# quokka-astro/quokka

Hardware: AMD Instinct MI355X
Metric: Mcell-updates/s on 3D Sedov unigrid (higher is better)
Workload: dtype f64; 1 GPU; 3D Sedov blast 256x256x256 unigrid (tests/blast_unigrid_256.in scaled to 256^3 cells per GPU), 128^3 boxes, PPM+HLLC RK2, gamma=1.4, CFL 0.3, reflecting octant; cells_per_gpu=16777216, boxes_per_gpu=8, parallelism=box-decomposition x1, rk2_mode=carry, fofc_stages=0, retries=0, x_sweep_in_y_march=True

## Files before the change

### include/quokka_amd.h

```cpp
#ifndef QUOKKA_AMD_H_
#define QUOKKA_AMD_H_

#include <stdint.h>

#ifdef __cplusplus
extern "C" {
#endif

typedef struct qk_ctx qk_ctx;
typedef struct qk_level qk_level;
typedef void *qk_stream;

typedef enum qk_status {
	QK_OK = 0,
	QK_ERR_INVALID = -1,
	QK_ERR_HIP = -2,
	QK_ERR_UNSUPPORTED = -3,
	QK_ERR_STATE = -4,
	QK_ERR_NOT_CONVERGED = -5
} qk_status;

typedef struct qk_array4 {
	double *p;
	int64_t jstride, kstride, nstride;
// ... 12 lines not shown

typedef struct qk_box {
	int lo[3];
	int hi[3];
} qk_box;

#define QK_MAX_SCALARS 8
#define QK_HOOK_COMPILED 100
typedef struct qk_hydro_traits {
	double gamma;
	double cs_isothermal;
	double mean_molecular_weight;
	double boltzmann_constant;
	int reconstruct_eint;
	int nscalars;
	int nmscalars;
	int ndim;
	int eos_temperature_model;
	double eos_alpha;
} qk_hydro_traits;

enum { QK_DIR_X1 = 0, QK_DIR_X2 = 1, QK_DIR_X3 = 2 };
enum { QK_RIEMANN_HLLC = 0, QK_RIEMANN_LLF = 1, QK_RIEMANN_HLLD = 2  };
enum { QK_LIMITER_MINMOD = 0, QK_LIMITER_MC = 1 };
enum { QK_BC_REFLECT_ODD = -1, QK_BC_INT_DIR = 0, QK_BC_REFLECT_EVEN = 1, QK_BC_FOEXTRAP = 2, QK_BC_EXT_DIR = 3 };

#define QK_DEVICE_HOST_PLANNING (-1)
int qk_ctx_create(qk_ctx **ctx, int device);
int qk_ctx_destroy(qk_ctx *ctx);
const char *qk_last_error(qk_ctx *ctx);
const char *qk_version(void);

int qk_profile_enable(qk_ctx *ctx, int on);
int qk_profile_only(qk_ctx *ctx, const char *kernel_name);
int qk_profile_reset(qk_ctx *ctx);
int qk_profile_num_kernels(qk_ctx *ctx);
int qk_profile_get(qk_ctx *ctx, int k, const char **name, long *count, double *total_ms);

int qk_clear_bytes(qk_ctx *ctx, qk_stream s, void *device_ptr, int64_t nbytes);

int qk_level_create(qk_ctx *ctx, qk_level **lev, int ndim, int nboxes, const qk_box *valid_boxes);
int qk_level_destroy(qk_level *lev);

int qk_upload_array4_table(qk_ctx *ctx, int n, const qk_array4 *host_table, qk_array4 **device_table);
int qk_upload_iarray4_table(qk_ctx *ctx, int n, const qk_iarray4 *host_table, qk_iarray4 **device_table);

int qk_ReconstructStatesConstant(qk_level *lev, qk_stream s, int dir, const qk_array4 *q, qk_array4 *leftState, qk_array4 *rightState, int nghost,
				 int nvars);
int qk_ReconstructStatesPLM(qk_level *lev, qk_stream s, int dir, int limiter, const qk_array4 *q, qk_array4 *leftState, qk_array4 *rightState,
			    int nghost, int nvars);
int qk_ReconstructStatesPPM(qk_level *lev, qk_stream s, int dir, const qk_array4 *q, qk_array4 *leftState, qk_array4 *rightState, int nghost,
			    int nvars, int iReadFrom, int iWriteFrom);

int qk_hydro_ConservedToPrimitive(qk_level *lev, qk_stream s, const qk_hydro_traits *t, const qk_array4 *cons, qk_array4 *primVar, int nghost);
int qk_hydro_ComputeFlatteningCoefficients(qk_level *lev, qk_stream s, const qk_hydro_traits *t, int dir, const qk_array4 *primVar, qk_array4 *x1Chi,
					   int nghost);
int qk_hydro_FlattenShocks(qk_level *lev, qk_stream s, const qk_hydro_traits *t, int dir, const qk_array4 *q, const qk_array4 *x1Chi,
			   const qk_array4 *x2Chi, const qk_array4 *x3Chi, qk_array4 *x1LeftState, qk_array4 *x1RightState, int nghost, int nvars);
int qk_hydro_ComputeFluxes(qk_level *lev, qk_stream s, const qk_hydro_traits *t, int riemann, int dir, qk_array4 *x1Flux, qk_array4 *x1FaceVel,
			   const qk_array4 *x1LeftState, const qk_array4 *x1RightState, const qk_array4 *primVar, double K_visc);
int qk_hydro_ComputeRhsFromFluxes(qk_level *lev, qk_stream s, const qk_hydro_traits *t, qk_array4 *rhs, const qk_array4 *const fluxArray[3],
				  const double dx[3], int nvars);
int qk_hydro_AddInternalEnergyPdV(qk_level *lev, qk_stream s, const qk_hydro_traits *t, qk_array4 *rhs, const qk_array4 *consVar, const double dx[3],
				  const qk_array4 *const faceVelArray[3], const qk_iarray4 *redoFlag);
int qk_hydro_PredictStep(qk_level *lev, qk_stream s, const qk_hydro_traits *t, const qk_array4 *consVarOld, qk_array4 *consVarNew,
			 const qk_array4 *rhs, double dt, int nvars, qk_iarray4 *redoFlag, int64_t *d_redo_count);
int qk_hydro_EnforceLimits(qk_level *lev, qk_stream s, const qk_hydro_traits *t, double densityFloor, double tempFloor, qk_array4 *state);
int qk_hydro_SyncDualEnergy(qk_level *lev, qk_stream s, const qk_hydro_traits *t, qk_array4 *consVar, int *d_error_flag);
int qk_hydro_ComputeMaxSignalSpeed(qk_level *lev, qk_stream s, const qk_hydro_traits *t, const qk_array4 *cons, qk_array4 *maxSignal);
int qk_hydro_maxSignalSpeedLocal(qk_level *lev, qk_stream s, const qk_hydro_traits *t, int which, const qk_array4 *cons, double *d_result);

int qk_replaceFluxes(qk_level *lev, qk_stream s, int dir, qk_array4 *flux, const qk_array4 *FOflux, const qk_iarray4 *redoFlag, int face_ncomp);
int qk_Saxpy(qk_level *lev, qk_stream s, int dir, qk_array4 *dst, double a, const qk_array4 *src, int ncomp);
int qk_hydro_FixupState(qk_level *lev, qk_stream s, const qk_hydro_traits *t, double densityFloor, double tempFloor, int use_dual_energy, qk_array4 *state,
			int *d_error_flag, double *d_max_signal);


int qk_advect_ComputeFluxes(qk_level *lev, qk_stream s, int dir, qk_array4 *flux, const qk_array4 *left, const qk_array4 *right, double advectionVx, int nvars);
int qk_advect_PredictStep(qk_level *lev, qk_stream s, const qk_array4 *consVarOld, qk_array4 *consVarNew, const qk_array4 *const fluxArray[3], double dt,
			  const double dx[3], int nvars);
int qk_advect_AddFluxesRK2(qk_level *lev, qk_stream s, qk_array4 *U_new, const qk_array4 *U0, const qk_array4 *U1, const qk_array4 *const fluxArray[3], double dt,
			   const double dx[3], int nvars);

typedef struct qk_hydro_stage_args {
	const qk_array4 *U_in;
	const qk_array4 *U_old;
	qk_array4 *U_out;
	qk_array4 *halfFlux[3];
	qk_array4 *halfVel[3];
	qk_iarray4 *redoFlag;
	int64_t *d_redo_count;
	int *d_error_flag;
	double *d_max_signal;
	void *scratch;
	int64_t scratch_bytes;
	double dx[3];
	double dt;
	int stage;
	int reconstruction_order;
	double densityFloor, tempFloor;
	int use_dual_energy;
	double K_visc;
	int store_flux_rk2;
	qk_array4 *fluxRk2[3];
	int rk2_carry_rhs;
	qk_array4 *rhs1;
	const struct qk_carray4 *flux_mask;
	int fofc_pass;
	int prim_out;
	int prim_in;
	int store_vel_rk2;
	qk_array4 *velRk2[3];
} qk_hydro_stage_args;

int64_t qk_hydro_stage_scratch_bytes(qk_level *lev, const qk_hydro_traits *t);
int qk_hydro_stage_fused(qk_level *lev, qk_stream s, const qk_hydro_traits *t, const qk_hydro_stage_args *a);

#define QK_MAX_GROUPS 8
typedef struct qk_rad_traits {
	double c_light, c_hat, radiation_constant, Erad_floor;
	int beta_order;
	int opacity_model;
	double kappaP, kappaE, kappaF;
	int pow_mode;
	int eddington_model;
	double opacity_T_ref, opacity_T_exponent, opacity_pow_floor;
	int ngroups;
	int mg_opacity_model;
	double energy_unit;
	double rad_boundaries[QK_MAX_GROUPS + 1];
	double mg_kappa_exponent[QK_MAX_GROUPS + 1], mg_kappa_lower[QK_MAX_GROUPS + 1];
	double mg_kappa_rho_exponent, mg_kappa_T_ref, mg_kappa_T_exponent;
	int enable_dust_gas_thermal_coupling_model;
	double dust_gas_interaction_coeff;
	int thermal_model;
	double gas_dust_coupling_threshold;
	double cooling_linear_coeff[QK_MAX_GROUPS];
	double cr_heating_rate;
	int enable_photoelectric_heating;
	double pe_heating_E1_derivative;
} qk_rad_traits;

int qk_rad_ConservedToPrimitive(qk_level *lev, qk_stream s, const qk_rad_traits *rt, const qk_array4 *cons, qk_array4 *primVar, int nghost);
int qk_rad_ComputeWavespeedCorrection(qk_level *lev, qk_stream s, const qk_rad_traits *rt, const qk_hydro_traits *t, int ndim, const qk_array4 *consVar,
				      const double dx[3], qk_array4 *const eps[3]);
int qk_rad_ComputeFluxes(qk_level *lev, qk_stream s, const qk_rad_traits *rt, int dir, qk_array4 *x1Flux, const qk_array4 *x1LeftState,
			 const qk_array4 *x1RightState, const qk_array4 *consVar, const qk_array4 *wavespeed_eps);
int qk_rad_computeRadiationFluxes(qk_level *lev, qk_stream s, const qk_rad_traits *rt, int ndim, int reconstruction_order, const qk_array4 *consVar,
				  qk_array4 *const flux[3], const qk_array4 *const wavespeed_eps[3] );
int qk_rad_stage_fused(qk_level *lev, qk_stream s, const qk_rad_traits *rt, int reconstruction_order, int stage, const qk_array4 *U_in, const qk_array4 *U0,
		       qk_array4 *U_new, qk_array4 *acc, qk_array4 *const flux_out[3], double dt, const double dx[3],
		       const qk_array4 *const wavespeed_eps[3] );
int qk_rad_PredictStep(qk_level *lev, qk_stream s, const qk_rad_traits *rt, int ndim, const qk_array4 *consVarOld, qk_array4 *consVarNew,
		       const qk_array4 *const fluxArray[3], double dt, const double dx[3]);
int qk_rad_AddFluxesRK2(qk_level *lev, qk_stream s, const qk_rad_traits *rt, int ndim, qk_array4 *U_new, const qk_array4 *U0, const qk_array4 *U1,
			const qk_array4 *const fluxArrayOld[3], const qk_array4 *const fluxArray[3], double dt, const double dx[3]);
int qk_rad_AddSourceTermsSingleGroup(qk_level *lev, qk_stream s, const qk_rad_traits *rt, const qk_hydro_traits *t, qk_array4 *consVar,
				     const qk_array4 *radEnergySource, double dt, int stage, int *d_iteration_counter, int *d_failure_counter);
int qk_rad_AddSourceTermsSingleGroupMirror(qk_level *lev, qk_stream s, const qk_rad_traits *rt, const qk_hydro_traits *t, qk_array4 *consVar,
					   const qk_array4 *radEnergySource, double dt, int stage, int *d_iteration_counter, int *d_failure_counter,
					   qk_array4 *mirror);
int qk_rad_AddSourceTermsMultiGroup(qk_level *lev, qk_stream s, const qk_rad_traits *rt, const qk_hydro_traits *t, qk_array4 *consVar,
				    const qk_array4 *radEnergySource, double dt, int stage, int *d_iteration_counter, int *d_failure_counter);
int qk_rad_mg_planck_fractions(qk_ctx *ctx, const qk_rad_traits *rt, double kB, int n, const double *T, double *fractions, double *Erad_g);

typedef struct qk_geometry {
	qk_box domain;
	int periodic[3];
	int ndim;
} qk_geometry;

typedef struct qk_bcrec {
	int lo[3];
	int hi[3];
} qk_bcrec;

#define QK_MAX_STATE_COMPS 48
typedef struct qk_dirichlet_face {
	int enabled;
	double values[QK_MAX_STATE_COMPS];
	int marshak;
	int marshak_energy_comp;
	int marshak_flux_comp;
	double marshak_c;
	uint64_t interior_mask;
	int kinetic_from_interior;
} qk_dirichlet_face;

typedef struct qk_ghost_plan qk_ghost_plan;
int qk_ghost_plan_create(qk_level *lev, qk_ghost_plan **plan, const qk_geometry *geom, int nghost, int ncomp, int n_all_boxes,
			 const qk_box *all_boxes, const int *owner_rank, int my_rank);
int qk_ghost_plan_destroy(qk_ghost_plan *plan);
int qk_ghost_plan_num_peers(qk_ghost_plan *plan);
int qk_ghost_plan_peer(qk_ghost_plan *plan, int k, int *rank, int64_t *send_count, int64_t *recv_count);
int qk_ghost_plan_num_items(qk_ghost_plan *plan, int kind, int k);
int qk_ghost_plan_item(qk_ghost_plan *plan, int kind, int k, int idx, int *dst_box, int *src_box, int lo[3], int hi[3], int shift[3], int64_t *offset);
int qk_FillBoundary_local(qk_ghost_plan *plan, qk_stream s, qk_array4 *state);
int qk_FillBoundary_local_int(qk_ghost_plan *plan, qk_stream s, qk_iarray4 *state);
int qk_FillBoundary_pack(qk_ghost_plan *plan, qk_stream s, int k, const qk_array4 *state, double *sendbuf);
int qk_FillBoundary_unpack(qk_ghost_plan *plan, qk_stream s, int k, qk_array4 *state, const double *recvbuf);
int qk_FillBoundary_pack_int(qk_ghost_plan *plan, qk_stream s, int k, const qk_iarray4 *state, int *sendbuf);
int qk_FillBoundary_unpack_int(qk_ghost_plan *plan, qk_stream s, int k, qk_iarray4 *state, const int *recvbuf);
int qk_SumBoundary_local(qk_ghost_plan *plan, qk_stream s, qk_array4 *state);
int qk_SumBoundary_pack(qk_ghost_plan *plan, qk_stream s, int k, const qk_array4 *state, double *buf);
int qk_SumBoundary_unpack(qk_ghost_plan *plan, qk_stream s, int k, qk_array4 *state, const double *buf);
int qk_FillPhysicalBoundary(qk_ghost_plan *plan, qk_stream s, qk_array4 *state, const qk_bcrec *bcs, const qk_dirichlet_face *dirichlet);
int qk_ghost_plan_set_components(qk_ghost_plan *plan, int scomp, int ncomp);
#define QK_BOXES_ALL 0
#define QK_BOXES_LOCAL_ONLY 1
#define QK_BOXES_REMOTE_DEPENDENT 2
int qk_ghost_plan_box_is_remote(qk_ghost_plan *plan, int local_box);
int qk_ghost_plan_set_box_remote(qk_ghost_plan *plan, int local_box, int flag);
int qk_FillPhysicalBoundary_subset(qk_ghost_plan *plan, qk_stream s, qk_array4 *state, const qk_bcrec *bcs, const qk_dirichlet_face *dirichlet,
				   int which);

typedef struct qk_carray4 {
	char *p;
	int64_t jstride, kstride, nstride;
	int begin[3];
	int end[3];
	int ncomp;
} qk_carray4;
enum { QK_TAG_CLEAR = 0, QK_TAG_BUF = 1, QK_TAG_SET = 2 };
#define QK_TAGFIELD_PRESSURE (-1)
int qk_tag_relative_gradient(qk_level *lev, qk_stream s, const qk_hydro_traits *t, const qk_array4 *state, qk_carray4 *tags, int field,
			     double eta_threshold, double q_min, int min_inclusive);
int qk_tag_centered_gradient(qk_level *lev, qk_stream s, const qk_array4 *state, qk_carray4 *tags, int comp, int dir, double dx, double eta_threshold,
			     double q_min, int min_inclusive);
int qk_PreInterpState(qk_level *lev, qk_stream s, qk_array4 *mf);
int qk_PostInterpState(qk_level *lev, qk_stream s, qk_array4 *mf);
typedef struct qk_avgdown_plan qk_avgdown_plan;
int qk_avgdown_plan_create(qk_level *crse, qk_level *fine, const int ratio[3], qk_avgdown_plan **plan);
int qk_avgdown_plan_destroy(qk_avgdown_plan *plan);
int qk_avgdown_plan_num_items(qk_avgdown_plan *plan);
int qk_average_down(qk_avgdown_plan *plan, qk_stream s, const qk_array4 *fine, qk_array4 *crse, int scomp, int ncomp);

typedef struct qk_interp_plan qk_interp_plan;
int qk_interp_plan_create(qk_level *crse, qk_level *fine, const qk_geometry *fine_geom, int nghost, const int ratio[3], int whole_fab, int n_all_fine,
			  const qk_box *all_fine, qk_interp_plan **plan);
int qk_interp_plan_destroy(qk_interp_plan *plan);
int qk_interp_plan_num_items(qk_interp_plan *plan);
int qk_interp_plan_item(qk_interp_plan *plan, int idx, int *fine_box, int *crse_box, int lo[3], int hi[3]);
int qk_InterpFromCoarse(qk_interp_plan *plan, qk_stream s, qk_array4 *fine, const qk_array4 *crse_old, const qk_array4 *crse_new, double w_old,
			double w_new, int ncomp, int method, int energy_hooks);

typedef struct qk_fluxreg qk_fluxreg;
int qk_fluxreg_create(qk_level *crse, qk_level *fine, const qk_geometry *crse_geom, const int ratio[3], int ncomp, int n_all_fine, const qk_box *all_fine,
		      int reg_nghost, qk_fluxreg **fr);
int qk_fluxreg_destroy(qk_fluxreg *fr);
int qk_fluxreg_num_items(qk_fluxreg *fr);
int qk_fluxreg_item(qk_fluxreg *fr, int idx, int *dir, int *side, int *fine_box, int *crse_box, int lo[3], int hi[3], int shift[3]);
int qk_fluxreg_reset(qk_fluxreg *fr, qk_stream s);
int qk_fluxreg_save(qk_fluxreg *fr, qk_stream s);
int qk_fluxreg_restore(qk_fluxreg *fr, qk_stream s);
int qk_fluxreg_CrseAdd(qk_fluxreg *fr, qk_stream s, const qk_array4 *const flux[3], const double dx[3], double dt);
int qk_fluxreg_FineAdd(qk_fluxreg *fr, qk_stream s, const qk_array4 *const flux[3], const double dx_fine[3], double dt);
int qk_fluxreg_Reflux(qk_fluxreg *fr, qk_stream s, qk_array4 *crse_state);
int qk_fluxreg_set_state_component(qk_fluxreg *fr, int comp0);

int qk_fluxreg_create_crse_part(qk_level *crse, qk_level *all_fine_level, const qk_geometry *crse_geom, const int ratio[3], int ncomp, qk_fluxreg **fr);

typedef struct qk_pcopy_plan qk_pcopy_plan;
int qk_pcopy_plan_create(qk_ctx *ctx, const qk_geometry *geom, int n_src, const qk_box *src_boxes, const int *src_owner, int src_nghost, int src_ring_only,
			 int n_dst, const qk_box *dst_boxes, const int *dst_owner, int dst_nghost, const qk_box *dst_holes, int ncomp, int my_rank,
			 qk_pcopy_plan **plan);
int qk_pcopy_plan_destroy(qk_pcopy_plan *plan);
int qk_pcopy_plan_num_peers(qk_pcopy_plan *plan);
int qk_pcopy_plan_peer(qk_pcopy_plan *plan, int k, int *rank, int64_t *send_count, int64_t *recv_count);
int qk_pcopy_plan_num_items(qk_pcopy_plan *plan, int kind, int k);
int qk_pcopy_plan_item(qk_pcopy_plan *plan, int kind, int k, int idx, int *dst_box, int *src_box, int lo[3], int hi[3], int shift[3], int64_t *offset);
int qk_ParallelCopy_local(qk_pcopy_plan *plan, qk_stream s, const qk_array4 *src, qk_array4 *dst, int scomp_src, int scomp_dst, int add);
int qk_ParallelCopy_pack(qk_pcopy_plan *plan, qk_stream s, int k, const qk_array4 *src, int scomp_src, double *sendbuf);
int qk_ParallelCopy_unpack(qk_pcopy_plan *plan, qk_stream s, int k, qk_array4 *dst, int scomp_dst, const double *recvbuf, int add);

int qk_copy_box(qk_ctx *ctx, qk_stream s, const qk_array4 *src, const qk_array4 *dst, const int lo[3], const int hi[3], int scomp, int dcomp, int ncomp);
int qk_amr_tile_flags(qk_level *lev, qk_stream s, const qk_carray4 *tags, const qk_box *domain, int n_error_buf, int tile, int *tile_flags_host);
int qk_amr_tile_flags_periodic(qk_level *lev, qk_stream s, const qk_carray4 *tags, const qk_box *domain, const int periodic[3], int n_error_buf, int tile,
			       int *tile_flags_host);
int qk_amr_cluster_tiles(const int *tiles, const int ntiles[3], int ndim, int blocking_factor, int max_grid_size, int parent_align, qk_box *boxes,
			 int max_boxes);
int qk_amr_cluster_berger_rigoutsos(const int *tiles, const int *allowed, const int ntiles[3], int ndim, int blocking_factor, int max_grid_size, double grid_eff,
				    qk_box *boxes, int max_boxes);

typedef struct qk_cloudy_tables {
	const double *log_nH;
	const double *log_Tgas;
	const double *cooling;
	const double *heating;
	const double *mean_mol_weight;
	int n_nH, n_Tgas;
	double T_min, T_max;
	double mmw_min, mmw_max;
} qk_cloudy_tables;
int qk_cloudy_tables_read(qk_ctx *ctx, const char *path, qk_cloudy_tables *host_tables);
int qk_cloudy_tables_free(qk_cloudy_tables *host_tables);
int qk_cooling_tabulated(qk_level *lev, qk_stream s, const qk_hydro_traits *t, qk_array4 *state, const qk_cloudy_tables *device_tables, double dt, double T_floor,
			 long long *d_counters);
// ... 52 lines not shown
```

### quokka_amd/capi.py

```python
from __future__ import annotations

import ctypes as C
import os

_HERE = os.path.dirname(os.path.abspath(__file__))
LIB_PATH = os.environ.get("QK_LIB_PATH", os.path.join(_HERE, "lib", "libquokka_amd.so"))

QK_OK, QK_ERR_INVALID, QK_ERR_HIP, QK_ERR_UNSUPPORTED, QK_ERR_STATE, QK_ERR_NOT_CONVERGED = 0, -1, -2, -3, -4, -5
ERR_UNSUPPORTED = QK_ERR_UNSUPPORTED
QK_TRACER_PREV, QK_TRACER_CUR, QK_TRACER_MAX_DEPTH = 0, 1, 3
HOOK_COMPILED = 100
DIR_X1, DIR_X2, DIR_X3 = 0, 1, 2
ARITH_DIVBY_RECIPOF, ARITH_DIVN, ARITH_RECIPEXACT, ARITH_SQRTN = 0, 1, 2, 3
COOLING_LIBM_DEVICE, COOLING_LIBM_PORTABLE = 0, 1
RIEMANN_HLLC, RIEMANN_LLF, RIEMANN_HLLD = 0, 1, 2
LIMITER_MINMOD, LIMITER_MC = 0, 1
BC_REFLECT_ODD, BC_INT_DIR, BC_REFLECT_EVEN, BC_FOEXTRAP, BC_EXT_DIR = -1, 0, 1, 2, 3

K_B = 1.380649e-16
M_U = 1.6605390666e-24


class Array4(C.Structure):
    _fields_ = [("p", C.c_void_p), ("jstride", C.c_int64), ("kstride", C.c_int64), ("nstride", C.c_int64),
                ("begin", C.c_int * 3), ("end", C.c_int * 3), ("ncomp", C.c_int)]


class Box(C.Structure):
    _fields_ = [("lo", C.c_int * 3), ("hi", C.c_int * 3)]


class HydroTraits(C.Structure):
    _fields_ = [("gamma", C.c_double), ("cs_isothermal", C.c_double), ("mean_molecular_weight", C.c_double),
                ("boltzmann_constant", C.c_double), ("reconstruct_eint", C.c_int), ("nscalars", C.c_int),
                ("nmscalars", C.c_int), ("ndim", C.c_int), ("eos_temperature_model", C.c_int), ("eos_alpha", C.c_double)]


class Geometry(C.Structure):
    _fields_ = [("domain", Box), ("periodic", C.c_int * 3), ("ndim", C.c_int)]


class BCRec(C.Structure):
    _fields_ = [("lo", C.c_int * 3), ("hi", C.c_int * 3)]


MAX_GROUPS = 8
MAX_STATE_COMPS = 48


class DirichletFace(C.Structure):
    _fields_ = [("enabled", C.c_int), ("values", C.c_double * MAX_STATE_COMPS),
                ("marshak", C.c_int), ("marshak_energy_comp", C.c_int), ("marshak_flux_comp", C.c_int), ("marshak_c", C.c_double),
                ("interior_mask", C.c_uint64), ("kinetic_from_interior", C.c_int)]


class RadTraits(C.Structure):
    _fields_ = [("c_light", C.c_double), ("c_hat", C.c_double), ("radiation_constant", C.c_double), ("Erad_floor", C.c_double),
                ("beta_order", C.c_int), ("opacity_model", C.c_int), ("kappaP", C.c_double), ("kappaE", C.c_double), ("kappaF", C.c_double),
                ("pow_mode", C.c_int), ("eddington_model", C.c_int),
                ("opacity_T_ref", C.c_double), ("opacity_T_exponent", C.c_double), ("opacity_pow_floor", C.c_double),
                ("ngroups", C.c_int), ("mg_opacity_model", C.c_int), ("energy_unit", C.c_double), ("rad_boundaries", C.c_double * (MAX_GROUPS + 1)),
                ("mg_kappa_exponent", C.c_double * (MAX_GROUPS + 1)), ("mg_kappa_lower", C.c_double * (MAX_GROUPS + 1)),
                ("mg_kappa_rho_exponent", C.c_double), ("mg_kappa_T_ref", C.c_double), ("mg_kappa_T_exponent", C.c_double),
                ("enable_dust_gas_thermal_coupling_model", C.c_int), ("dust_gas_interaction_coeff", C.c_double), ("thermal_model", C.c_int),
                ("gas_dust_coupling_threshold", C.c_double),
                ("cooling_linear_coeff", C.c_double * MAX_GROUPS), ("cr_heating_rate", C.c_double), ("enable_photoelectric_heating", C.c_int),
                ("pe_heating_E1_derivative", C.c_double)]

    def set_groups(self, boundaries, energy_unit, opacity_model, kappa_exponent, kappa_lower, rho_exponent=0.0, T_ref=0.0, T_exponent=0.0):
        ng = len(boundaries) - 1
        assert 2 <= ng <= MAX_GROUPS and len(kappa_exponent) == len(kappa_lower) == ng + 1
        self.ngroups, self.mg_opacity_model, self.energy_unit = ng, int(opacity_model), float(energy_unit)
        for g in range(ng + 1):
            self.rad_boundaries[g] = float(boundaries[g])
            self.mg_kappa_exponent[g] = float(kappa_exponent[g])
            self.mg_kappa_lower[g] = float(kappa_lower[g])
        self.mg_kappa_rho_exponent, self.mg_kappa_T_ref, self.mg_kappa_T_exponent = float(rho_exponent), float(T_ref), float(T_exponent)
        return self


class CloudyTables(C.Structure):
    _fields_ = [("log_nH", C.c_void_p), ("log_Tgas", C.c_void_p), ("cooling", C.c_void_p), ("heating", C.c_void_p), ("mean_mol_weight", C.c_void_p),
                ("n_nH", C.c_int), ("n_Tgas", C.c_int), ("T_min", C.c_double), ("T_max", C.c_double), ("mmw_min", C.c_double), ("mmw_max", C.c_double)]


class StageArgs(C.Structure):
    _fields_ = [("U_in", C.c_void_p), ("U_old", C.c_void_p), ("U_out", C.c_void_p),
                ("halfFlux", C.c_void_p * 3), ("halfVel", C.c_void_p * 3),
                ("redoFlag", C.c_void_p), ("d_redo_count", C.c_void_p), ("d_error_flag", C.c_void_p), ("d_max_signal", C.c_void_p),
                ("scratch", C.c_void_p), ("scratch_bytes", C.c_int64),
                ("dx", C.c_double * 3), ("dt", C.c_double), ("stage", C.c_int), ("reconstruction_order", C.c_int),
                ("densityFloor", C.c_double), ("tempFloor", C.c_double), ("use_dual_energy", C.c_int), ("K_visc", C.c_double),
                ("store_flux_rk2", C.c_int), ("fluxRk2", C.c_void_p * 3), ("rk2_carry_rhs", C.c_int), ("rhs1", C.c_void_p), ("flux_mask", C.c_void_p), ("fofc_pass", C.c_int),
                ("prim_out", C.c_int), ("prim_in", C.c_int),
                ("store_vel_rk2", C.c_int), ("velRk2", C.c_void_p * 3)]


def traits(gamma=1.4, reconstruct_eint=True, ndim=3, mean_molecular_weight=M_U, boltzmann_constant=K_B,
           cs_isothermal=float("nan"), nscalars=0, nmscalars=0, eos_temperature_model=0, eos_alpha=0.0) -> HydroTraits:
    return HydroTraits(gamma, cs_isothermal, mean_molecular_weight, boltzmann_constant, int(reconstruct_eint), nscalars, nmscalars, ndim,
                       int(eos_temperature_model), float(eos_alpha))


class QkError(RuntimeError):
    pass


_lib = None


def lib() -> C.CDLL:
    global _lib
    if _lib is not None:
        return _lib
    if not os.path.exists(LIB_PATH):
        raise QkError(f"{LIB_PATH} is missing: run `python -c 'import __graft_entry__ as g; g.build()'` "
                      "(hipcc --offload-arch=gfx950). The hot path has no CPU fallback.")
    L = C.CDLL(LIB_PATH)
    vp, ci, cd = C.c_void_p, C.c_int, C.c_double
    P = C.POINTER
    L.qk_version.restype = C.c_char_p
    L.qk_last_error.restype = C.c_char_p
    L.qk_last_error.argtypes = [vp]
    L.qk_ctx_create.argtypes = [P(vp), ci]
    L.qk_ctx_destroy.argtypes = [vp]
    L.qk_level_create.argtypes = [vp, P(vp), ci, ci, P(Box)]
    L.qk_level_destroy.argtypes = [vp]
    L.qk_upload_array4_table.argtypes = [vp, ci, P(Array4), P(vp)]
    L.qk_upload_iarray4_table.argtypes = [vp, ci, P(Array4), P(vp)]
    L.qk_profile_enable.argtypes = [vp, ci]
    L.qk_profile_only.argtypes = [vp, C.c_char_p]
    L.qk_clear_bytes.argtypes = [vp, vp, vp, C.c_int64]
    L.qk_profile_reset.argtypes = [vp]
    L.qk_cloudy_tables_read.argtypes = [vp, C.c_char_p, P(CloudyTables)]
    L.qk_cloudy_tables_free.argtypes = [P(CloudyTables)]
    L.qk_cooling_tabulated.argtypes = [vp, vp, P(HydroTraits), vp, P(CloudyTables), cd, cd, vp]
    L.qk_cooling_evaluate.argtypes = [vp, vp, P(CloudyTables), cd, ci, C.c_int64, vp, vp, vp]
    L.qk_cooling_set_libm.argtypes = [vp, ci]
    L.qk_arith_evaluate.argtypes = [vp, vp, ci, C.c_int64, vp, vp, vp]
    L.qk_profile_num_kernels.argtypes = [vp]
    L.qk_profile_get.argtypes = [vp, ci, P(C.c_char_p), P(C.c_long), P(cd)]
    T = P(HydroTraits)
    L.qk_ReconstructStatesConstant.argtypes = [vp, vp, ci, vp, vp, vp, ci, ci]
    L.qk_ReconstructStatesPLM.argtypes = [vp, vp, ci, ci, vp, vp, vp, ci, ci]
    L.qk_ReconstructStatesPPM.argtypes = [vp, vp, ci, vp, vp, vp, ci, ci, ci, ci]
    L.qk_hydro_ConservedToPrimitive.argtypes = [vp, vp, T, vp, vp, ci]
    L.qk_hydro_ComputeFlatteningCoefficients.argtypes = [vp, vp, T, ci, vp, vp, ci]
    L.qk_hydro_FlattenShocks.argtypes = [vp, vp, T, ci, vp, vp, vp, vp, vp, vp, ci, ci]
    L.qk_hydro_ComputeFluxes.argtypes = [vp, vp, T, ci, ci, vp, vp, vp, vp, vp, cd]
    L.qk_hydro_ComputeRhsFromFluxes.argtypes = [vp, vp, T, vp, P(vp), P(cd), ci]
    L.qk_hydro_AddInternalEnergyPdV.argtypes = [vp, vp, T, vp, vp, P(cd), P(vp), vp]
    L.qk_hydro_PredictStep.argtypes = [vp, vp, T, vp, vp, vp, cd, ci, vp, vp]
    L.qk_hydro_EnforceLimits.argtypes = [vp, vp, T, cd, cd, vp]
    L.qk_hydro_SyncDualEnergy.argtypes = [vp, vp, T, vp, vp]
    L.qk_hydro_ComputeMaxSignalSpeed.argtypes = [vp, vp, T, vp, vp]
    L.qk_hydro_maxSignalSpeedLocal.argtypes = [vp, vp, T, ci, vp, vp]
    L.qk_replaceFluxes.argtypes = [vp, vp, ci, vp, vp, vp, ci]
    L.qk_Saxpy.argtypes = [vp, vp, ci, vp, cd, vp, ci]
    R = P(RadTraits)
    L.qk_rad_ConservedToPrimitive.argtypes = [vp, vp, R, vp, vp, ci]
    L.qk_rad_ComputeFluxes.argtypes = [vp, vp, R, ci, vp, vp, vp, vp, vp]
    L.qk_rad_computeRadiationFluxes.argtypes = [vp, vp, R, ci, ci, vp, P(vp), P(vp)]
    L.qk_rad_ComputeWavespeedCorrection.argtypes = [vp, vp, R, T, ci, vp, P(cd), P(vp)]
    L.qk_rad_PredictStep.argtypes = [vp, vp, R, ci, vp, vp, P(vp), cd, P(cd)]
    L.qk_rad_AddFluxesRK2.argtypes = [vp, vp, R, ci, vp, vp, vp, P(vp), P(vp), cd, P(cd)]
    L.qk_hydro_FixupState.argtypes = [vp, vp, T, cd, cd, ci, vp, vp, vp]
    L.qk_rad_stage_fused.argtypes = [vp, vp, R, ci, ci, vp, vp, vp, vp, P(vp), cd, P(cd), P(vp)]
    L.qk_rad_AddSourceTermsSingleGroup.argtypes = [vp, vp, R, T, vp, vp, cd, ci, vp, vp]
    L.qk_rad_AddSourceTermsSingleGroupMirror.argtypes = [vp, vp, R, T, vp, vp, cd, ci, vp, vp, vp]
    L.qk_rad_AddSourceTermsMultiGroup.argtypes = [vp, vp, R, T, vp, vp, cd, ci, vp, vp]
    L.qk_rad_mg_planck_fractions.argtypes = [vp, R, cd, ci, P(cd), P(cd), P(cd)]
    if hasattr(L, "qk_hydro_stage_fused"):
        L.qk_hydro_stage_scratch_bytes.argtypes = [vp, T]
        L.qk_hydro_stage_scratch_bytes.restype = C.c_int64
        L.qk_hydro_stage_fused.argtypes = [vp, vp, T, P(StageArgs)]
    if hasattr(L, "qk_ghost_plan_create"):
        L.qk_ghost_plan_create.argtypes = [vp, P(vp), P(Geometry), ci, ci, ci, P(Box), P(ci), ci]
        L.qk_ghost_plan_destroy.argtypes = [vp]
        L.qk_ghost_plan_num_peers.argtypes = [vp]
        L.qk_ghost_plan_peer.argtypes = [vp, ci, P(ci), P(C.c_int64), P(C.c_int64)]
        L.qk_ghost_plan_num_items.argtypes = [vp, ci, ci]
        L.qk_ghost_plan_item.argtypes = [vp, ci, ci, ci, P(ci), P(ci), ci * 3, ci * 3, ci * 3, P(C.c_int64)]
        L.qk_FillBoundary_local.argtypes = [vp, vp, vp]
        L.qk_FillBoundary_local_int.argtypes = [vp, vp, vp]
        L.qk_FillBoundary_pack.argtypes = [vp, vp, ci, vp, vp]
        L.qk_FillBoundary_unpack.argtypes = [vp, vp, ci, vp, vp]
        L.qk_SumBoundary_local.argtypes = [vp, vp, vp]
        L.qk_SumBoundary_pack.argtypes = [vp, vp, ci, vp, vp]
        L.qk_SumBoundary_unpack.argtypes = [vp, vp, ci, vp, vp]
        L.qk_FillBoundary_pack_int.argtypes = [vp, vp, ci, vp, vp]
        L.qk_FillBoundary_unpack_int.argtypes = [vp, vp, ci, vp, vp]
        L.qk_FillPhysicalBoundary.argtypes = [vp, vp, vp, P(BCRec), P(DirichletFace)]
        L.qk_FillPhysicalBoundary_subset.argtypes = [vp, vp, vp, P(BCRec), P(DirichletFace), C.c_int]
        L.qk_ghost_plan_set_components.argtypes = [vp, C.c_int, C.c_int]
        L.qk_ghost_plan_box_is_remote.argtypes = [vp, C.c_int]
        L.qk_ghost_plan_set_box_remote.argtypes = [vp, C.c_int, C.c_int]
    if hasattr(L, "qk_tag_relative_gradient"):
        L.qk_tag_relative_gradient.argtypes = [vp, vp, T, vp, vp, ci, C.c_double, C.c_double, ci]
        L.qk_tag_centered_gradient.argtypes = [vp, vp, vp, vp, ci, ci, C.c_double, C.c_double, C.c_double, ci]
        L.qk_avgdown_plan_create.argtypes = [vp, vp, ci * 3, P(vp)]
        L.qk_avgdown_plan_destroy.argtypes = [vp]
        L.qk_avgdown_plan_num_items.argtypes = [vp]
        L.qk_average_down.argtypes = [vp, vp, vp, vp, ci, ci]
        L.qk_interp_plan_create.argtypes = [vp, vp, P(Geometry), ci, ci * 3, ci, ci, vp, P(vp)]
        L.qk_interp_plan_destroy.argtypes = [vp]
        L.qk_interp_plan_num_items.argtypes = [vp]
        L.qk_interp_plan_item.argtypes = [vp, ci, P(ci), P(ci), ci * 3, ci * 3]
        L.qk_InterpFromCoarse.argtypes = [vp, vp, vp, vp, vp, C.c_double, C.c_double, ci, ci, ci]
        L.qk_fluxreg_create.argtypes = [vp, vp, P(Geometry), ci * 3, ci, ci, vp, ci, P(vp)]
        L.qk_fluxreg_destroy.argtypes = [vp]
        L.qk_fluxreg_num_items.argtypes = [vp]
        L.qk_fluxreg_item.argtypes = [vp, ci, P(ci), P(ci), P(ci), P(ci), ci * 3, ci * 3, ci * 3]
        L.qk_fluxreg_reset.argtypes = [vp, vp]
        L.qk_fluxreg_save.argtypes = [vp, vp]
        L.qk_fluxreg_restore.argtypes = [vp, vp]
        L.qk_fluxreg_CrseAdd.argtypes = [vp, vp, vp * 3, C.c_double * 3, C.c_double]
        L.qk_fluxreg_FineAdd.argtypes = [vp, vp, vp * 3, C.c_double * 3, C.c_double]
        L.qk_fluxreg_Reflux.argtypes = [vp, vp, vp]
        L.qk_fluxreg_set_state_component.argtypes = [vp, C.c_int]
        L.qk_copy_box.argtypes = [vp, vp, vp, vp, ci * 3, ci * 3, ci, ci, ci]
        L.qk_amr_tile_flags.argtypes = [vp, vp, vp, P(Box), ci, ci, vp]
        L.qk_amr_tile_flags_periodic.argtypes = [vp, vp, vp, P(Box), P(ci), ci, ci, vp]
        L.qk_amr_cluster_tiles.argtypes = [vp, ci * 3, ci, ci, ci, ci, P(Box), ci]
        L.qk_amr_cluster_berger_rigoutsos.argtypes = [vp, vp, ci * 3, ci, ci, ci, C.c_double, P(Box), ci]
        L.qk_PreInterpState.argtypes = [vp, vp, vp]
        L.qk_PostInterpState.argtypes = [vp, vp, vp]
        L.qk_fluxreg_create_crse_part.argtypes = [vp, vp, P(Geometry), ci * 3, ci, P(vp)]
        L.qk_pcopy_plan_create.argtypes = [vp, P(Geometry), ci, P(Box), P(ci), ci, ci, ci, P(Box), P(ci), ci, vp, ci, ci, P(vp)]
        L.qk_pcopy_plan_destroy.argtypes = [vp]
        L.qk_pcopy_plan_num_peers.argtypes = [vp]
        L.qk_pcopy_plan_peer.argtypes = [vp, ci, P(ci), P(C.c_int64), P(C.c_int64)]
        L.qk_pcopy_plan_num_items.argtypes = [vp, ci, ci]
        L.qk_pcopy_plan_item.argtypes = [vp, ci, ci, ci, P(ci), P(ci), ci * 3, ci * 3, ci * 3, P(C.c_int64)]
        L.qk_ParallelCopy_local.argtypes = [vp, vp, vp, vp, ci, ci, ci]
        L.qk_ParallelCopy_pack.argtypes = [vp, vp, ci, vp, ci, vp]
        L.qk_ParallelCopy_unpack.argtypes = [vp, vp, ci, vp, ci, vp, ci]
    L.qk_tracer_plan_create.argtypes = [vp, P(vp), P(Geometry), cd * 3, cd * 3, cd * 3]
    L.qk_tracer_plan_destroy.argtypes = [vp]
    L.qk_tracer_plan_lattice.argtypes = [vp, ci * 3, P(C.c_int64)]
    L.qk_tracer_InitOnePerCell.argtypes = [vp, vp, cd * 3, vp * 3, vp * 3, vp, vp, C.c_int64, ci]
    L.qk_tracer_AdvectWithUmac.argtypes = [vp, vp, vp * 3, cd, C.c_int64, vp * 3, vp * 3]
    L.qk_tracer_Redistribute.argtypes = [vp, vp, C.c_int64, vp * 3, vp]
    L.qk_tracer_plan_create_refined.argtypes = [vp, P(vp), P(Geometry), cd * 3, cd * 3, cd * 3]
    L.qk_tracer_plan_set_parent.argtypes = [vp, ci, vp, vp * 3]
    L.qk_tracer_plan_set_time_weights.argtypes = [vp, cd, cd]
    L.qk_tracer_plan_clear_parent.argtypes = [vp]
    L.qk_tracer_Where.argtypes = [P(vp), ci, vp, ci, ci, C.c_int64, vp * 3, vp, vp, vp]
    i3 = ci * 3
    L.qk_gravity_scratch_bytes.argtypes = [i3]
    L.qk_gravity_scratch_bytes.restype = C.c_int64
    L.qk_gravity_num_ghosts.argtypes = [i3]
    L.qk_gravity_num_ghosts.restype = C.c_int64
    L.qk_gravity_fill_rhs.argtypes = [vp, vp, cd, vp, ci, i3, vp]
    L.qk_gravity_dirichlet_solve.argtypes = [vp, vp, i3, cd, vp, vp, cd, cd, ci, vp, C.c_int64, P(ci), P(cd)]
    L.qk_gravity_surface_gather.argtypes = [vp, vp, i3, vp, vp]
    L.qk_gravity_surface_potential.argtypes = [vp, vp, i3, vp, vp, vp, C.c_int64]
    L.qk_gravity_surface_scatter.argtypes = [vp, vp, i3, vp, vp]
    L.qk_gravity_kick.argtypes = [vp, vp, i3, vp, cd * 3, cd, vp]
    _lib = L
    return L


BOXES_ALL, BOXES_LOCAL_ONLY, BOXES_REMOTE_DEPENDENT = 0, 1, 2
TAG_CLEAR, TAG_BUF, TAG_SET = 0, 1, 2
TAGFIELD_PRESSURE = -1

DECLARED_SYMBOLS = [
    "qk_ctx_create", "qk_ctx_destroy", "qk_last_error", "qk_version", "qk_level_create", "qk_level_destroy",
    "qk_upload_array4_table", "qk_upload_iarray4_table", "qk_clear_bytes", "qk_profile_enable", "qk_profile_only", "qk_profile_reset", "qk_profile_num_kernels", "qk_profile_get",
    "qk_ReconstructStatesConstant", "qk_ReconstructStatesPLM", "qk_ReconstructStatesPPM",
    "qk_hydro_ConservedToPrimitive", "qk_hydro_ComputeFlatteningCoefficients", "qk_hydro_FlattenShocks",
    "qk_hydro_ComputeFluxes", "qk_hydro_ComputeRhsFromFluxes", "qk_hydro_AddInternalEnergyPdV", "qk_hydro_PredictStep",
    "qk_hydro_EnforceLimits", "qk_hydro_SyncDualEnergy", "qk_hydro_ComputeMaxSignalSpeed", "qk_hydro_maxSignalSpeedLocal",
    "qk_replaceFluxes", "qk_Saxpy", "qk_hydro_FixupState", "qk_hydro_stage_scratch_bytes", "qk_hydro_stage_fused",
    "qk_rad_ConservedToPrimitive", "qk_rad_ComputeWavespeedCorrection", "qk_rad_ComputeFluxes", "qk_rad_computeRadiationFluxes", "qk_rad_PredictStep", "qk_rad_AddFluxesRK2", "qk_rad_stage_fused",
    "qk_rad_AddSourceTermsSingleGroup", "qk_rad_AddSourceTermsSingleGroupMirror", "qk_rad_AddSourceTermsMultiGroup", "qk_rad_mg_planck_fractions",
    "qk_ghost_plan_create", "qk_ghost_plan_destroy", "qk_ghost_plan_num_peers", "qk_ghost_plan_peer", "qk_ghost_plan_num_items", "qk_ghost_plan_item",
    "qk_FillBoundary_local", "qk_FillBoundary_local_int", "qk_FillBoundary_pack", "qk_FillBoundary_unpack", "qk_FillBoundary_pack_int", "qk_FillBoundary_unpack_int", "qk_SumBoundary_local", "qk_SumBoundary_pack", "qk_SumBoundary_unpack", "qk_FillPhysicalBoundary",
    "qk_FillPhysicalBoundary_subset", "qk_ghost_plan_set_components", "qk_ghost_plan_box_is_remote", "qk_ghost_plan_set_box_remote",
    "qk_tag_relative_gradient", "qk_tag_centered_gradient", "qk_avgdown_plan_create", "qk_avgdown_plan_destroy", "qk_avgdown_plan_num_items", "qk_average_down", "qk_PreInterpState", "qk_PostInterpState",
    "qk_interp_plan_create", "qk_interp_plan_destroy", "qk_interp_plan_num_items", "qk_interp_plan_item", "qk_InterpFromCoarse",
    "qk_fluxreg_create", "qk_fluxreg_destroy", "qk_fluxreg_num_items", "qk_fluxreg_item", "qk_fluxreg_reset", "qk_fluxreg_save", "qk_fluxreg_restore", "qk_fluxreg_CrseAdd", "qk_fluxreg_FineAdd",
    "qk_fluxreg_Reflux", "qk_fluxreg_set_state_component", "qk_amr_tile_flags", "qk_amr_tile_flags_periodic", "qk_amr_cluster_tiles", "qk_amr_cluster_berger_rigoutsos", "qk_copy_box",
    "qk_cloudy_tables_read", "qk_cloudy_tables_free", "qk_cooling_tabulated", "qk_cooling_evaluate", "qk_cooling_set_libm", "qk_arith_evaluate",
    "qk_fluxreg_create_crse_part", "qk_pcopy_plan_create", "qk_pcopy_plan_destroy", "qk_pcopy_plan_num_peers", "qk_pcopy_plan_peer", "qk_pcopy_plan_num_items",
    "qk_pcopy_plan_item", "qk_ParallelCopy_local", "qk_ParallelCopy_pack", "qk_ParallelCopy_unpack",
    "qk_tracer_plan_create", "qk_tracer_plan_destroy", "qk_tracer_plan_lattice", "qk_tracer_InitOnePerCell", "qk_tracer_AdvectWithUmac", "qk_tracer_Redistribute",
    "qk_tracer_plan_create_refined", "qk_tracer_plan_set_parent", "qk_tracer_plan_set_time_weights", "qk_tracer_plan_clear_parent", "qk_tracer_Where",
    "qk_gravity_scratch_bytes", "qk_gravity_num_ghosts", "qk_gravity_fill_rhs", "qk_gravity_dirichlet_solve", "qk_gravity_surface_gather",
    "qk_gravity_surface_potential", "qk_gravity_surface_scatter", "qk_gravity_kick",
]


def check(ctx, rc: int, what: str = "") -> None:
    if rc != QK_OK:
        msg = lib().qk_last_error(ctx).decode() if ctx else ""
        raise QkError(f"{what} failed with status {rc}: {msg}")
```

### quokka_amd/csrc/qk_boundary.hip

```cpp
#include <algorithm>
#include <cstdlib>
#include <array>
#include <map>
#include <cstring>
#include <vector>

#include "qk_device.hpp"
#include "qk_internal.hpp"

using namespace qk;

namespace
{

struct CopyItem {
	int dst_box;
	int src_box;
	int lo[3], hi[3];
	int shift[3];
	int64_t offset;
};

struct PeerPlan {
	int rank = -1;
// ... 333 lines not shown
					it.offset = pp.recv_count;
					pp.recv_count += regionCells(it) * ncomp;
					pp.max_recv_cells = std::max<int64_t>(pp.max_recv_cells, regionCells(it));
					pp.recv.push_back(it);
				} else {
					PeerPlan &pp = peers[owner[gd]];
					pp.rank = owner[gd];
					it.offset = pp.send_count;
					pp.send_count += regionCells(it) * ncomp;
					pp.max_send_cells = std::max<int64_t>(pp.max_send_cells, regionCells(it));
					pp.send.push_back(it);
				}
			}
		}
	}
	for (int b = 0; b < lev->nboxes; ++b) {
		qk_box grown = lev->boxes[b];
		for (int d = 0; d < geom->ndim; ++d) {
			grown.lo[d] -= nghost;
			grown.hi[d] += nghost;
		}
		for (int d = 0; d < geom->ndim; ++d) {
			if (geom->periodic[d] != 0) {
				continue;
			}
			for (int side = 0; side < 2; ++side) {
				CopyItem it{};
				it.dst_box = b;
				it.src_box = b;
				for (int e = 0; e < 3; ++e) {
					it.lo[e] = grown.lo[e];
					it.hi[e] = grown.hi[e];
				}
				if (side == 0) {
					it.hi[d] = std::min(grown.hi[d], geom->domain.lo[d] - 1);
				} else {
					it.lo[d] = std::max(grown.lo[d], geom->domain.hi[d] + 1);
				}
				if (it.hi[d] >= it.lo[d]) {
					P->shells.push_back(it);
					P->max_shell_cells = std::max<int64_t>(P->max_shell_cells, regionCells(it));
				}
			}
		}
	}
	P->box_remote.assign(lev->nboxes, 0);
	for (auto &kv : peers) {
		for (auto const &it : kv.second.recv) {
			P->box_remote[it.dst_box] = 1;
		}
	}
	partitionShells(P);
	{
		int64_t biggest = std::max<int64_t>(P->max_local_cells, P->max_shell_cells);
		for (auto &kv : peers) {
			biggest = std::max<int64_t>(biggest, std::max<int64_t>(kv.second.max_recv_cells, kv.second.max_send_cells));
		}
		if (biggest * ncomp >= (int64_t{1} << 31)) {
			delete P;
			return setError(ctx, QK_ERR_UNSUPPORTED, "qk_ghost_plan_create: a ghost region holds 2^31 or more values");
		}
	}
	int rc = uploadItems(ctx, P->local, &P->d_local);
	if (rc == QK_OK) {
		rc = uploadItems(ctx, P->shells, &P->d_shells);
	}
	for (auto &kv : peers) {
		if (rc == QK_OK) {
			rc = uploadItems(ctx, kv.second.send, &kv.second.d_send);
		}
		if (rc == QK_OK) {
			rc = uploadItems(ctx, kv.second.recv, &kv.second.d_recv);
		}
		P->peers.push_back(kv.second);
	}
	if (rc != QK_OK) {
		qk_ghost_plan_destroy(P);
		return rc;
	}
	*plan_out = P;
	return QK_OK;
}

int qk_ghost_plan_destroy(qk_ghost_plan *plan)
{
	if (plan == nullptr) {
		return QK_ERR_INVALID;
	}
	(void)hipFree(plan->d_local);
	(void)hipFree(plan->d_shells);
	for (auto &p : plan->peers) {
		(void)hipFree(p.d_send);
		(void)hipFree(p.d_recv);
	}
	(void)hipFree(plan->d_bcs);
	(void)hipFree(plan->d_dir);
	(void)hipFree(plan->d_physbc);
	delete plan;
	return QK_OK;
}

int qk_ghost_plan_num_peers(qk_ghost_plan *plan) { return plan == nullptr ? QK_ERR_INVALID : static_cast<int>(plan->peers.size()); }

int qk_ghost_plan_peer(qk_ghost_plan *plan, int k, int *rank, int64_t *send_count, int64_t *recv_count)
{
	if (plan == nullptr) {
		return QK_ERR_INVALID;
	}
	QK_REQUIRE(plan->lev->ctx, k >= 0 && k < static_cast<int>(plan->peers.size()) && rank && send_count && recv_count, "qk_ghost_plan_peer: bad index");
	*rank = plan->peers[k].rank;
	*send_count = plan->peers[k].send_count;
	*recv_count = plan->peers[k].recv_count;
	return QK_OK;
}

static auto planItems(qk_ghost_plan *plan, int kind, int k) -> std::vector<CopyItem> const *
{
	if (kind == 0) {
		return &plan->local;
	}
	if (kind == 3) {
		return &plan->shells;
	}
	if (k < 0 || k >= static_cast<int>(plan->peers.size())) {
		return nullptr;
	}
	return (kind == 1) ? &plan->peers[k].send : (kind == 2) ? &plan->peers[k].recv : nullptr;
}

int qk_ghost_plan_num_items(qk_ghost_plan *plan, int kind, int k)
{
	if (plan == nullptr) {
		return QK_ERR_INVALID;
	}
	auto const *v = planItems(plan, kind, k);
	return v == nullptr ? QK_ERR_INVALID : static_cast<int>(v->size());
}

int qk_ghost_plan_item(qk_ghost_plan *plan, int kind, int k, int idx, int *dst_box, int *src_box, int lo[3], int hi[3], int shift[3], int64_t *offset)
{
	if (plan == nullptr) {
		return QK_ERR_INVALID;
	}
	auto const *v = planItems(plan, kind, k);
	QK_REQUIRE(plan->lev->ctx, v != nullptr && idx >= 0 && idx < static_cast<int>(v->size()) && dst_box && src_box && lo && hi && shift && offset,
		   "qk_ghost_plan_item: bad argument");
	CopyItem const &it = (*v)[idx];
	*dst_box = it.dst_box;
	*src_box = it.src_box;
	for (int d = 0; d < 3; ++d) {
		lo[d] = it.lo[d];
		hi[d] = it.hi[d];
		shift[d] = it.shift[d];
	}
	*offset = it.offset;
	return QK_OK;
}

int qk_FillBoundary_local(qk_ghost_plan *plan, qk_stream s, qk_array4 *state_t)
{
	if (plan == nullptr) {
		return QK_ERR_INVALID;
	}
	qk_ctx *ctx = plan->lev->ctx;
	QK_REQUIRE(ctx, state_t, "FillBoundary_local: NULL state");
	if (plan->local.empty()) {
// ... 268 lines not shown
```

### quokka_amd/csrc/qk_core.hip

```cpp
#include <algorithm>
#include <cstring>

#include "qk_device.hpp"
#include "qk_internal.hpp"

namespace
{

__global__ void __launch_bounds__(256) k_arith_evaluate(int what, int64_t n, const double *a, const double *b, double *out)
{
	const int64_t i = static_cast<int64_t>(blockIdx.x) * blockDim.x + threadIdx.x;
	if (i >= n) {
		return;
	}
	double r;
	switch (what) {
	case QK_ARITH_DIVBY_RECIPOF:
		r = qk::divBy(a[i], qk::recipOf(b[i]));
		break;
	case QK_ARITH_DIVN:
		r = qk::divN(a[i], b[i]);
		break;
	case QK_ARITH_RECIPEXACT:
		r = qk::recipExact(b[i]);
// ... 20 lines not shown
		auto *c = new qk_ctx;
		c->device = -1;
		*ctx = c;
		return QK_OK;
	}
	int ndev = 0;
	if (hipGetDeviceCount(&ndev) != hipSuccess || ndev == 0) {
		std::fprintf(stderr, "quokka_amd: no HIP device visible; the hot path has no CPU fallback\n");
		return QK_ERR_HIP;
	}
	if (device < 0 || device >= ndev) {
		return QK_ERR_INVALID;
	}
	if (hipSetDevice(device) != hipSuccess) {
		return QK_ERR_HIP;
	}
	auto *c = new qk_ctx;
	c->device = device;
	*ctx = c;
	return QK_OK;
}

int qk_ctx_destroy(qk_ctx *ctx)
{
	if (ctx == nullptr) {
		return QK_ERR_INVALID;
	}
	for (void *p : ctx->owned) {
		(void)hipFree(p);
	}
	delete ctx;
	return QK_OK;
}

const char *qk_last_error(qk_ctx *ctx)
{
	if (ctx == nullptr) {
		return "null context";
	}
	return ctx->last_error.c_str();
}

int qk_level_create(qk_ctx *ctx, qk_level **lev, int ndim, int nboxes, const qk_box *valid_boxes)
{
	if (ctx == nullptr || lev == nullptr) {
		return QK_ERR_INVALID;
	}
	QK_REQUIRE(ctx, nboxes >= 0 && (valid_boxes != nullptr || nboxes == 0), "qk_level_create: bad box list");
	QK_REQUIRE(ctx, ndim >= 1 && ndim <= 3, "qk_level_create: ndim must be 1, 2 or 3");
	auto *L = new qk_level;
	L->ctx = ctx;
	L->ndim = ndim;
	L->nboxes = nboxes;
	L->boxes.assign(valid_boxes, valid_boxes + nboxes);
	for (int b = 0; b < nboxes; ++b) {
		for (int d = 0; d < 3; ++d) {
			L->maxlen[d] = std::max(L->maxlen[d], valid_boxes[b].hi[d] - valid_boxes[b].lo[d] + 1);
		}
	}
	if (ctx->device < 0) {
		*lev = L;
		return QK_OK;
	}
	hipError_t e = hipMalloc(reinterpret_cast<void **>(&L->d_boxes), sizeof(qk_box) * (nboxes > 0 ? nboxes : 1));
	if (e == hipSuccess) {
		e = (nboxes > 0) ? hipMemcpy(L->d_boxes, valid_boxes, sizeof(qk_box) * nboxes, hipMemcpyHostToDevice) : hipSuccess;
	}
	if (e != hipSuccess) {
		delete L;
		return qk::setError(ctx, QK_ERR_HIP, "qk_level_create", hipGetErrorString(e));
	}
	*lev = L;
	return QK_OK;
}

int qk_level_destroy(qk_level *lev)
{
	if (lev == nullptr) {
		return QK_ERR_INVALID;
	}
	(void)hipFree(lev->d_boxes);
	(void)hipFree(lev->d_sgeom);
	(void)hipFree(lev->d_tile_flags);
	(void)hipFree(lev->d_cooling_queue);
	delete lev;
	return QK_OK;
}

int qk_clear_bytes(qk_ctx *ctx, qk_stream s, void *device_ptr, int64_t nbytes)
{
	if (ctx == nullptr) {
		return QK_ERR_INVALID;
	}
	QK_REQUIRE(ctx, device_ptr != nullptr && nbytes >= 0, "qk_clear_bytes: NULL pointer or negative size");
	QK_HIP_CHECK(ctx, hipMemsetAsync(device_ptr, 0, static_cast<size_t>(nbytes), static_cast<hipStream_t>(s)));
	return QK_OK;
}

int qk_profile_enable(qk_ctx *ctx, int on)
{
	if (ctx == nullptr) {
		return QK_ERR_INVALID;
	}
	ctx->profiling = (on != 0);
	return QK_OK;
}

int qk_profile_only(qk_ctx *ctx, const char *kernel_name)
{
	if (ctx == nullptr) {
		return QK_ERR_INVALID;
	}
	ctx->prof_only = (kernel_name != nullptr) ? kernel_name : "";
	return QK_OK;
}

static void profCollect(qk_ctx *ctx)
{
	for (auto &p : ctx->prof_pending) {
		float ms = 0.f;
		if (hipEventSynchronize(p.stop) == hipSuccess && hipEventElapsedTime(&ms, p.start, p.stop) == hipSuccess) {
			ctx->prof_slots[p.slot].count += 1;
			ctx->prof_slots[p.slot].total_ms += ms;
		}
		ctx->prof_free_events.push_back(p.start);
		ctx->prof_free_events.push_back(p.stop);
	}
	ctx->prof_pending.clear();
}

int qk_profile_reset(qk_ctx *ctx)
{
	if (ctx == nullptr) {
		return QK_ERR_INVALID;
	}
	profCollect(ctx);
	ctx->prof_slots.clear();
	return QK_OK;
}

int qk_profile_num_kernels(qk_ctx *ctx)
{
	if (ctx == nullptr) {
		return QK_ERR_INVALID;
	}
	profCollect(ctx);
	return static_cast<int>(ctx->prof_slots.size());
}

int qk_profile_get(qk_ctx *ctx, int k, const char **name, long *count, double *total_ms)
{
	if (ctx == nullptr) {
		return QK_ERR_INVALID;
	}
	QK_REQUIRE(ctx, k >= 0 && k < static_cast<int>(ctx->prof_slots.size()) && name && count && total_ms, "qk_profile_get: bad index");
	*name = ctx->prof_slots[k].name.c_str();
	*count = ctx->prof_slots[k].count;
	*total_ms = ctx->prof_slots[k].total_ms;
	return QK_OK;
}

static int uploadTable(qk_ctx *ctx, int n, const void *host, size_t elem, void **dev)
{
	if (ctx == nullptr) {
		return QK_ERR_INVALID;
	}
// ... 40 lines not shown
```

### quokka_amd/csrc/qk_hydro_fused.hip

```cpp
#include "qk_device.hpp"
#include <algorithm>
#include <cmath>
#include <cstdlib>
#include <type_traits>
#include <vector>

#include "qk_internal.hpp"

using namespace qk;

namespace
{

constexpr int NG = 4;

template <class P> QK_DEV void streamStore(P *p, double v) { __builtin_nontemporal_store(v, p); }
template <class P> QK_DEV auto streamLoad(P *p) -> double { return __builtin_nontemporal_load(p); }

struct SGeom {
	int64_t off;
	int glo[3];
	int n[3];
	int pitch;
	int64_t ncell;
};

enum { S_AUX = 0, S_RHS = 4 };
constexpr auto scratchComps(int nscalars) -> int { return S_RHS + NVAR + nscalars + 1; }
constexpr int QK_FUSED_MAX_SCALARS = 3;

struct SweepArgs {
	const qk_box *boxes;
	const SGeom *geom;
	double *scratch;
	int64_t total_cells;
	const qk_array4 *U_in;
	const qk_array4 *U_old;
	qk_array4 *U_out;
	qk_array4 *halfFlux;
	qk_array4 *halfVel;
	qk_iarray4 *redoFlag;
	unsigned long long *redo_count;
	int *error_flag;
	double *max_signal;
	double inv_dx;
	double dx;
	double inv_dx0, dx0;
	double dx3[3];
	double dt;
	double densityFloor, tempFloor;
	double K_visc;
	int use_dual_energy;
	bool reconstruct_eint;
	bool same_old;
	bool store_rk2;
	qk_array4 *rk2Flux;
	qk_array4 *rhs1;
	const qk_carray4 *fluxMask;
	int nseg;
	bool prim_in, prim_out;
	bool store_vel;
	qk_array4 *rk2Vel;
};

QK_DEV auto sarr(SweepArgs const &a, int comp) -> double * { return a.scratch + static_cast<int64_t>(comp) * a.total_cells; }

#ifndef QK_PT_Y
#define QK_PT_Y 7
#define QK_PT_THREADS 512
#endif
constexpr int PT_X = 66, PT_Y = QK_PT_Y, PT_THREADS = QK_PT_THREADS;
constexpr int PT_OWN = PT_X * PT_Y;
constexpr int PT_HALO_Y = 6 * PT_X;
constexpr int PT_HALO = PT_HALO_Y + 6 * PT_Y;
static_assert(PT_HALO <= PT_THREADS && PT_OWN <= PT_THREADS, "one halo cell per thread");

struct PlaneCell {
	double rho, vx, vy, vz, P;
};

struct PlaneRaw {
	double rho, mx, my, mz, E;
};
QK_DEV auto planeLoad(RA4 const &U, int64_t u) -> PlaneRaw
{
	PlaneRaw r;
	r.rho = U.p[u + U.ns * RHO];
	r.mx = U.p[u + U.ns * MX];
	r.my = U.p[u + U.ns * MY];
	r.mz = U.p[u + U.ns * MZ];
	r.E = U.p[u + U.ns * ENE];
	return r;
}
QK_DEV auto planeCell(Eos const &eos, bool re, PlaneRaw const &r) -> PlaneCell
{
	PlaneCell c;
	c.rho = r.rho;
	const Recip R = recipOf(c.rho);
	c.vx = divBy(r.mx, R);
	c.vy = divBy(r.my, R);
	c.vz = divBy(r.mz, R);
	if (eos.isothermal) {
		c.P = c.rho * (eos.cs_iso * eos.cs_iso);
		return c;
	}
	const double kinetic_energy = 0.5 * c.rho * (c.vx * c.vx + c.vy * c.vy + c.vz * c.vz);
	const double Eint_cons = r.E - kinetic_energy;
	if (re) {
		const double e = divBy(Eint_cons, R);
		const double e2 = (c.rho == 0.0) ? 0.0 : divBy(c.rho * e, R);
		c.P = eos.gm1 * c.rho * e2;
	} else {
		const double e = (c.rho == 0.0) ? 0.0 : divBy(Eint_cons, R);
		c.P = eos.gm1 * c.rho * e;
	}
	return c;
}

QK_DEV auto chiCompressive(double Pm2, double Pm1, double Pp1, double Pp2, Recip const &RKS, Recip const &Rbeta) -> double
{
	constexpr double beta_max = 0.85;
	constexpr double Zmax = 0.75;
	constexpr double Zmin = 0.25;
	const double dP1 = fabs(Pp1 - Pm1);
	const double beta_denom = fabs(Pp2 - Pm2);
	const double beta = (beta_denom != 0) ? divBy(dP1, recipOf(beta_denom)) : 0;
	const double chi_min = smax0(smin1(divBy(beta_max - beta, Rbeta)));
	const double Z = divBy(dP1, RKS);
	return smax(chi_min, smin1((Zmax - Z) / (Zmax - Zmin)));
}

template <bool PRIM>
__global__ void __launch_bounds__(PT_THREADS, 4) k_pre3(const qk_box *boxes, const SGeom *geom, const qk_array4 *U_t, double *scratch, int64_t T, Eos eos, bool re, int nseg,
							    int xt, int yt, int ndim)
{
	constexpr bool prim_in = PRIM;
	const unsigned nblk = gridDim.x, lin = blockIdx.x;
	const unsigned q8 = nblk / 8, r8 = nblk % 8, xcd = lin % 8, slot = lin / 8;
	const unsigned logical = (xcd < r8) ? xcd * (q8 + 1) + slot : r8 * (q8 + 1) + (xcd - r8) * q8 + slot;
	const int bix = static_cast<int>(logical % xt), biy = static_cast<int>((logical / xt) % yt), biz = static_cast<int>(logical / (xt * yt));
	__shared__ double s_P[PT_Y + 6][PT_X + 6];
	__shared__ double s_vx[PT_Y][PT_X + 4], s_vy[PT_Y + 4][PT_X];
	__shared__ double s_cx[PT_Y][PT_X + 2], s_cy[PT_Y + 2][PT_X];

	const int b = biz / nseg;
	const int seg = biz - b * nseg;
	const qk_box bx = boxes[b];
	const SGeom g = geom[b];
	RA4 U(U_t[b]);
	const int t = threadIdx.x;
	const int x0 = bx.lo[0] - 1 + bix * PT_X;
	const int y0 = bx.lo[1] - 1 + biy * PT_Y;
	if (x0 > bx.hi[0] + 1 || y0 > bx.hi[1] + 1) {
		return;
	}
	const int nall = bx.hi[2] - bx.lo[2] + 3;
	const int seglen = (nall + nseg - 1) / nseg;
	const int zfirst = bx.lo[2] - 1 + seg * seglen;
	const int zlast = min(zfirst + seglen - 1, bx.hi[2] + 1);
	if (zlast < zfirst) {
		return;
	}
	const int ngy = (ndim >= 2) ? NG : 0, ngz = (ndim == 3) ? NG : 0;
	const int flo[2] = {bx.lo[0] - NG, bx.lo[1] - ngy}, fhi[2] = {bx.hi[0] + NG, bx.hi[1] + ngy};
	const int fzlo = bx.lo[2] - ngz, fzhi = bx.hi[2] + ngz;

	const bool own = t < PT_OWN;
	const int ty = own ? t / PT_X : 0;
	const int tx = own ? t - ty * PT_X : 0;
	const int oi = x0 + tx, oj = y0 + ty;
	const bool ownIn = own && oi <= fhi[0] && oj >= flo[1] && oj <= fhi[1];
	const bool ownOut = own && oi <= bx.hi[0] + 1 && oj <= bx.hi[1] + 1;
	const int h = t - (PT_THREADS - PT_HALO);
	int hx = 0, hy = 0;
	if (h >= 0) {
		if (h < PT_HALO_Y) {
			const int r = h / PT_X;
			hx = h - r * PT_X;
			hy = (r < 3) ? r - 3 : PT_Y + r - 3;
		} else {
			const int r = (h - PT_HALO_Y) / 6, c = (h - PT_HALO_Y) - r * 6;
			hy = r;
			hx = (c < 3) ? c - 3 : PT_X + c - 3;
		}
	}
	const int hi_ = x0 + hx, hj = y0 + hy;
	const bool haloIn = (h >= 0) && hi_ >= flo[0] && hi_ <= fhi[0] && hj >= flo[1] && hj <= fhi[1];
	const bool rimX = (h >= 0) && (hx == -1 || hx == PT_X);
	const bool rimY = (h >= 0) && (hy == -1 || hy == PT_Y);
	const int rx = hx, ry = hy;

	double Pz[5] = {1., 1., 1., 1., 1.}, vzw[5] = {0., 0., 0., 0., 0.}, rhoz[3] = {1., 1., 1.}, chz[3] = {1., 1., 1.};
	const Recip Rbeta = recipOf(0.85 - 0.75);
	double fm[4] = {1., 1., 1., 1.}, fdx[4] = {0., 0., 0., 0.}, fdy[4] = {0., 0., 0., 0.};
	double *Sout = scratch + g.off;
	const PlaneRaw neutral{1., 0., 0., 0., prim_in ? 1. : 1. / eos.gm1};
	auto cellOf = [&](PlaneRaw const &r) -> PlaneCell { return prim_in ? PlaneCell{r.rho, r.mx, r.my, r.mz, r.E} : planeCell(eos, re, r); };
	int64_t uo = ownIn ? U.idx(oi, oj, zfirst - 3) : 0;
	int64_t uh = haloIn ? U.idx(hi_, hj, zfirst - 3) : 0;

	for (int k = zfirst - 3; k <= zlast + 3; ++k, uo += U.ks, uh += U.ks) {
		const bool inPlane = (k >= zfirst) && (k <= zlast);
		const bool kIn = (k >= fzlo) && (k <= fzhi);
		const PlaneCell c = cellOf((ownIn && kIn) ? planeLoad(U, uo) : neutral);
#pragma unroll
		for (int m = 0; m < 4; ++m) {
			Pz[m] = Pz[m + 1];
			vzw[m] = vzw[m + 1];
		}
		Pz[4] = c.P;
		vzw[4] = c.vz;
		rhoz[0] = rhoz[1];
		rhoz[1] = rhoz[2];
		rhoz[2] = c.rho;
#pragma unroll
		for (int m = 0; m < 3; ++m) {
			fm[m] = fm[m + 1];
			fdx[m] = fdx[m + 1];
			fdy[m] = fdy[m + 1];
		}
		if (inPlane) {
			PlaneCell hc{1., 0., 0., 0., 1.};
			if (own) {
				s_P[ty + 3][tx + 3] = c.P;
				s_vx[ty][tx + 2] = c.vx;
				s_vy[ty + 2][tx] = c.vy;
			}
			if (h >= 0) {
				if constexpr (PRIM) {
					if (haloIn && kIn) {
						hc.P = U.p[uh + U.ns * ENE];
						if (hy >= 0 && hy < PT_Y && hx >= -2 && hx < PT_X + 2) {
							hc.vx = U.p[uh + U.ns * MX];
						}
						if (hx >= 0 && hx < PT_X && hy >= -2 && hy < PT_Y + 2) {
							hc.vy = U.p[uh + U.ns * MY];
						}
						if (rimX || rimY) {
							hc.rho = U.p[uh + U.ns * RHO];
						}
					}
				} else {
					hc = cellOf((haloIn && kIn) ? planeLoad(U, uh) : neutral);
				}
				s_P[hy + 3][hx + 3] = hc.P;
				if (hy >= 0 && hy < PT_Y && hx >= -2 && hx < PT_X + 2) {
					s_vx[hy][hx + 2] = hc.vx;
				}
				if (hx >= 0 && hx < PT_X && hy >= -2 && hy < PT_Y + 2) {
					s_vy[hy + 2][hx] = hc.vy;
				}
			}
			__syncthreads();
			if (own) {
				const bool cx = s_vx[ty][tx + 3] < s_vx[ty][tx + 1];
				const bool cy = (ndim >= 2) && (s_vy[ty + 3][tx] < s_vy[ty + 1][tx]);
				double chx = 1.0, chy = 1.0;
				if (cx || cy) {
					const Recip RKS = recipOf(flatteningKS(eos, c.rho, c.P));
					if (cx) {
						const double *Pr = &s_P[ty + 3][tx + 3];
						chx = chiCompressive(Pr[-2], Pr[-1], Pr[1], Pr[2], RKS, Rbeta);
					}
					if (cy) {
						chy = chiCompressive(s_P[ty + 1][tx + 3], s_P[ty + 2][tx + 3], s_P[ty + 4][tx + 3], s_P[ty + 5][tx + 3], RKS, Rbeta);
					}
				}
				s_cx[ty][tx + 1] = chx;
				s_cy[ty + 1][tx] = chy;
			}
			if (rimX) {
				double chx = 1.0;
				if (s_vx[ry][rx + 3] < s_vx[ry][rx + 1]) {
					const double *Pr = &s_P[ry + 3][rx + 3];
					chx = chiCompressive(Pr[-2], Pr[-1], Pr[1], Pr[2], recipOf(flatteningKS(eos, hc.rho, hc.P)), Rbeta);
				}
				s_cx[ry][rx + 1] = chx;
			} else if (rimY) {
				double chy = 1.0;
				if ((ndim >= 2) && (s_vy[ry + 3][rx] < s_vy[ry + 1][rx])) {
					chy = chiCompressive(s_P[ry + 1][rx + 3], s_P[ry + 2][rx + 3], s_P[ry + 4][rx + 3], s_P[ry + 5][rx + 3],
							     recipOf(flatteningKS(eos, hc.rho, hc.P)), Rbeta);
				}
				s_cy[ry + 1][rx] = chy;
			}
			__syncthreads();
			if (own) {
				const double mx = smin(smin(s_cx[ty][tx], s_cx[ty][tx + 1]), s_cx[ty][tx + 2]);
				const double my = smin(smin(s_cy[ty][tx], s_cy[ty + 1][tx]), s_cy[ty + 2][tx]);
				fm[3] = smin(mx, my);
				fdx[3] = smin(s_vx[ty][tx + 3] - c.vx, c.vx - s_vx[ty][tx + 1]);
				fdy[3] = smin(s_vy[ty + 3][tx] - c.vy, c.vy - s_vy[ty + 1][tx]);
			}
			__syncthreads();
		}
		chz[0] = chz[1];
		chz[1] = chz[2];
		chz[2] = 1.0;
		if ((ndim == 3) && (vzw[3] < vzw[1])) {
			chz[2] = chiCompressive(Pz[0], Pz[1], Pz[3], Pz[4], recipOf(flatteningKS(eos, rhoz[0], Pz[2])), Rbeta);
		}
		const int ko = k - 3;
		if (ko >= zfirst && ko <= zlast && ownOut) {
			const int64_t cc = (oi - g.glo[0]) + static_cast<int64_t>(g.pitch) * ((oj - g.glo[1]) + static_cast<int64_t>(g.n[1]) * (ko - g.glo[2]));
			Sout[(S_AUX + 0) * T + cc] = smin(fm[0], smin(smin(chz[0], chz[1]), chz[2]));
			Sout[(S_AUX + 1) * T + cc] = fdx[0];
			Sout[(S_AUX + 2) * T + cc] = fdy[0];
			Sout[(S_AUX + 3) * T + cc] = smin(vzw[2] - vzw[1], vzw[1] - vzw[0]);
		}
	}
}

template <int ORDER> QK_DEV void cellEdges(const double qm2, const double qm1, const double q0, const double qp1, const double qp2, double &am, double &ap)
{
	if (ORDER == 3) {
		ppmEdges(qm2, qm1, q0, qp1, qp2, am, ap);
	} else if (ORDER == 2) {
		plmEdges<QK_LIMITER_MINMOD>(qm1, q0, qp1, am, ap);
	} else {
		am = q0;
		ap = q0;
	}
}

// ... 446 lines not shown
			marked = (maskByte(md, i - 1, j, k) | maskByte(md, i, j, k)) != 0;
		}
		double qLo[NV];
		if (FOFC && STAGE == 1) {
			getColumn(s_q, tm1, qLo);
		}
		settleFace<STAGE, CARRY, FOFC, 0, NS, false>(a, eos, NDIM, b, fi, true, marked, F1, qLo, q0, F, vf);
	}
	__syncthreads();
	putColumn(s_q, t, F);
	s_d[2][t] = vf;
	__syncthreads();

	const bool isCell = validRow && (i >= bx.lo[0]) && (i <= bx.hi[0]) && (t >= 3) && (t < 3 + XOUT);
	if constexpr (NDIM == 1) {
		double sig0 = 0., sig1 = 0.;
		if (isCell) {
			double rhs[NV], r1[NV + 1];
#pragma unroll
			for (int n = 0; n < NV; ++n) {
				rhs[n] = a.inv_dx * (F[n] - s_q[n][tp1]);
				r1[n] = 0.;
			}
			r1[NV] = 0.;
			const double div_v = (s_d[2][tp1] - vf) / a.dx;
			RA4 Uold(a.U_old[b]);
			const int64_t co = Uold.idx(i, j, k);
			double Uo[NV];
#pragma unroll
			for (int n = 0; n < NV; ++n) {
				Uo[n] = Uold.p[co + Uold.ns * n];
			}
			if (CARRY && STAGE == 2) {
				RA4 R1(a.rhs1[b]);
				const int64_t c1 = R1.idx(i, j, k);
#pragma unroll
				for (int n = 0; n < NV + 1; ++n) {
					r1[n] = R1.p[c1 + R1.ns * n];
				}
			}
			const EpiConst ec = epiConst(eos);
			updateCellFrom<NS, CARRY ? STAGE : 0, FOFC, 1>(a, eos, ec, b, i, j, k, Uo, rhs, div_v, r1, sig0, sig1);
		}
		if (a.max_signal != nullptr) {
			reduceSignal(a.max_signal, sig0, sig1);
		}
	} else if (isCell) {
		double *R = a.scratch + g.off + c;
#pragma unroll
		for (int n = 0; n < NV; ++n) {
			streamStore(&R[(S_RHS + n) * T], a.inv_dx * (F[n] - s_q[n][tp1]));
		}
		R[RHS_DIVV * T] = (s_d[2][tp1] - vf) / a.dx;
	}
}

#ifndef QK_MARCH_BY
#define QK_MARCH_BY 4
#endif
constexpr int MARCH_BY = QK_MARCH_BY;
constexpr int XW = 64 + 8;
#ifndef QK_XROWS
#define QK_XROWS 16
#endif
constexpr int XROWS = QK_XROWS;
static_assert(XROWS == 8 || XROWS == 16 || XROWS == 32, "the batch maps rows and sides onto the lanes of one wave");
QK_DEV void waveFence()
{
	__builtin_amdgcn_fence(__ATOMIC_SEQ_CST, "wavefront");
	__builtin_amdgcn_wave_barrier();
}
template <int NV> using EdgeRow = double[6][NV + 1];
template <int NV> QK_DEV void stageEdgeRow(double (*sx)[XW], const EdgeRow<NV> &row)
{
	const int t6 = static_cast<int>(threadIdx.x);
	if (t6 < 6) {
		const int slot = (t6 < 2) ? t6 : 64 + t6;
#pragma unroll
		for (int n = 0; n < NV + 1; ++n) {
			sx[n][slot] = row[t6][n];
		}
	}
}
template <int ORDER, int NS>
QK_DEV void fusexEdgeBatch(SweepArgs const &a, Eos const &eos, RA4 const &Uin, SGeom const &g, const int64_t (&st)[3], const double *S, int x0, int row0, int hi, int ot, EdgeRow<NVAR + NS> *edge)
{
	constexpr int NV = NVAR + NS;
	const int64_t T = a.total_cells;
	const int tx = static_cast<int>(threadIdx.x);
	const int side = (tx / XROWS) & 1;
	const int brow = tx & (XROWS - 1);
	const int mrow = min(row0 + brow, hi);
	const int f = x0 + 64 * side;
	int64_t ub = Uin.idx(f - 3, mrow, ot);
	double qb[6][NV], Uc[NVAR];
#pragma unroll
	for (int m = 0; m < 6; ++m, ++ub) {
		loadPrims<NS>(Uin, ub, eos, a.reconstruct_eint, a.prim_in, qb[m], Uc);
	}
	const int64_t cb = (f - 1 - g.glo[0]) + (mrow - g.glo[1]) * st[1] + (ot - g.glo[2]) * st[2];
	const double chiL = S[cb], chiR = S[cb + 1];
	const double DyL = S[(S_AUX + 2) * T + cb], DyR = S[(S_AUX + 2) * T + cb + 1];
	const double DzL = S[(S_AUX + 3) * T + cb], DzR = S[(S_AUX + 3) * T + cb + 1];
	double qLb[NV], qRb[NV], Fb[NV], vfb;
#pragma unroll
	for (int n = 0; n < NV; ++n) {
		double unused;
		reconstructVar<ORDER>(chiL, qb[0][n], qb[1][n], qb[2][n], qb[3][n], qb[4][n], unused, qLb[n]);
		reconstructVar<ORDER>(chiR, qb[1][n], qb[2][n], qb[3][n], qb[4][n], qb[5][n], qRb[n], unused);
	}
	faceFluxAll<0, QK_RIEMANN_HLLC, false, NS>(eos, a.reconstruct_eint, 3, qLb, qRb, qb[3][PVX] - qb[2][PVX], DyL, DyR, DzL, DzR, a.K_visc, Fb, vfb);
	double(*ed)[NV + 1] = edge[brow];
	double *ef = ed[5 - side];
#pragma unroll
	for (int n = 0; n < NV; ++n) {
		ef[n] = Fb[n];
	}
	ef[NV] = vfb;
#pragma unroll
	for (int n = 0; n < NV; ++n) {
		ed[2 * side][n] = (side != 0) ? qb[3][n] : qb[1][n];
		ed[2 * side + 1][n] = (side != 0) ? qb[4][n] : qb[2][n];
	}
}
template <int DIR, int ORDER, int STAGE, bool LAST, int NS, bool CARRY, bool TWOD = false, bool FOFC = false, bool FUSEX = false>
__global__ void __launch_bounds__(64 * MARCH_BY) k_sweep_march(SweepArgs a, Eos eos)
{
	static_assert(!FUSEX || (DIR == 1 && !LAST && !TWOD && !FOFC && CARRY), "the X sweep rides on the Y sweep of a 3-D level in the carried form");
	static_assert(!(FOFC && CARRY), "the first-order flux correction pass exists for the reference's form of the RK2 average");
	static_assert(!TWOD || (DIR == 1 && LAST), "the 2-D build has one marching sweep: y, carrying the epilogue");
	constexpr int NV = NVAR + NS;
	constexpr int RHS_DIVV = S_RHS + NV;
	static_assert(DIR == 1 || DIR == 2, "marching sweeps are the strided directions");
	const BlockId blk = xcdContiguousBlock();
	const int bix = blk.x, biy = blk.y, biz = blk.z;
	const int b = biz / a.nseg;
	const int seg = biz - b * a.nseg;
	const qk_box bx = a.boxes[b];
	const SGeom g = a.geom[b];
	constexpr int OT = (DIR == 1) ? 2 : 1;
	const int i_raw = bx.lo[0] + bix * 64 + threadIdx.x;
	const int ot_raw = bx.lo[OT] + biy * MARCH_BY + threadIdx.y;
	const bool live = (i_raw <= bx.hi[0]) && (ot_raw <= bx.hi[OT]);
	const int i = min(i_raw, bx.hi[0]);
	const int ot = min(ot_raw, bx.hi[OT]);
	double sig0 = 0., sig1 = 0.;
	const int64_t T = a.total_cells;
	const int64_t st[3] = {1, g.pitch, static_cast<int64_t>(g.pitch) * g.n[1]};
	const int64_t ms = st[DIR];
	const int seglen = (bx.hi[DIR] - bx.lo[DIR] + 1 + a.nseg - 1) / a.nseg;
	const int lo = bx.lo[DIR] + seg * seglen, hi = min(lo + seglen - 1, bx.hi[DIR]);
	const int nvalid = hi - lo + 1;
	if (nvalid <= 0) {
		return;
	}
	if constexpr (FUSEX) {
		if (bx.lo[0] + bix * 64 > bx.hi[0]) {
			return;
		}
	}
	int pos[3];
	pos[0] = i;
	pos[OT] = ot;
	pos[DIR] = lo - 3;
	int64_t c = (pos[0] - g.glo[0]) * st[0] + (pos[1] - g.glo[1]) * st[1] + (pos[2] - g.glo[2]) * st[2];
	const double *S = a.scratch + g.off;
	double *Sw = a.scratch + g.off;
	RA4 Uin(a.U_in[b]);
	RA4 Uold(a.U_old[b]);
	const EpiConst ec = epiConst(eos);
	int64_t u = Uin.idx(pos[0], pos[1], pos[2]);
	const int64_t ums = (DIR == 1) ? Uin.js : Uin.ks;

	constexpr int AV = Axes<DIR, TWOD>::v, AW = Axes<DIR, TWOD>::w;
	double q[5][NV];
	double apPrev[NV], Fprev[NV];
	double vfPrev = 0., dVprev = 0., dWprev = 0.;
	bool maskCol = false;
	int maskLo = 0, maskHi = -1;
	if (CARRY && a.fluxMask != nullptr) {
		const qk_carray4 md = a.fluxMask[b];
		maskCol = live && i >= md.begin[0] && i < md.end[0] && ot >= md.begin[OT] && ot < md.end[OT];
		maskLo = md.begin[DIR];
		maskHi = md.end[DIR] - 1;
	}
	constexpr bool RING = LAST && (STAGE == 1);
	__shared__ double s_ring[RING ? 3 : 1][RING ? NV : 1][RING ? 64 * MARCH_BY : 1];
	__shared__ double s_fx[FUSEX ? MARCH_BY : 1][FUSEX ? NV + 2 : 1][FUSEX ? XW : 1];
	__shared__ double s_edge[FUSEX ? MARCH_BY : 1][FUSEX ? XROWS : 1][6][FUSEX ? NV + 1 : 1];
	double chiPrev = 1.;
	const int lself = (FUSEX && threadIdx.x == 0) ? 69 : static_cast<int>(threadIdx.x) + 2;
	const int lnext = (FUSEX && threadIdx.x == 63) ? 68 : static_cast<int>(threadIdx.x) + 3;
	const int tid = threadIdx.y * 64 + threadIdx.x;
	const bool ring = RING && a.same_old;
	int slot = 0;
	double Uo[NV];
#pragma unroll
	for (int n = 0; n < NV; ++n) {
		apPrev[n] = 0.;
		Fprev[n] = 0.;
#pragma unroll
		for (int m = 0; m < 5; ++m) {
			q[m][n] = 0.;
		}
	}

	constexpr bool PFQ = !FUSEX && NS == 0;
	double Un[NVAR];
	if constexpr (PFQ) {
#pragma unroll
		for (int n = 0; n < NVAR; ++n) {
			Un[n] = Uin.p[u + Uin.ns * n];
		}
	}
	for (int step = 0; step < nvalid + 6; ++step, c += ms, u += ums) {
#pragma unroll
		for (int n = 0; n < NV; ++n) {
			q[0][n] = q[1][n];
			q[1][n] = q[2][n];
			q[2][n] = q[3][n];
			q[3][n] = q[4][n];
		}
		{
			double Uc[NVAR];
			if constexpr (PFQ) {
#pragma unroll
				for (int n = 0; n < NVAR; ++n) {
					Uc[n] = Un[n];
					Un[n] = Uin.p[u + ums + Uin.ns * n];
				}
				primsOf<NS>(Uin, u, eos, a.reconstruct_eint, a.prim_in, Uc, q[4]);
			} else {
				loadPrims<NS>(Uin, u, eos, a.reconstruct_eint, a.prim_in, q[4], Uc);
			}
			if constexpr (RING) {
				if (ring) {
#pragma unroll
					for (int n = 0; n < NV; ++n) {
						Uo[n] = s_ring[slot][n][tid];
						s_ring[slot][n][tid] = (n < NVAR) ? Uc[n] : q[4][n];
					}
					slot = (slot == 2) ? 0 : slot + 1;
				}
			}
		}
		if (step < 4) {
			continue;
		}
		const int64_t cc = c - 2 * ms;
		const double chi = S[(S_AUX + 0) * T + cc];
		const double dV = S[(S_AUX + 1 + AV) * T + cc];
		const double dW = S[(S_AUX + 1 + AW) * T + cc];
		int fidx[3], cidx[3];
		fidx[0] = cidx[0] = i;
		fidx[OT] = cidx[OT] = ot;
		fidx[DIR] = lo + (step - 5);
		cidx[DIR] = lo + (step - 6);
		const int64_t cu = cc - ms;
		double rhs_in[NV + 1], F1[NV + 1];
		if (step >= 6) {
			if constexpr (FUSEX) {
				double(*sx)[XW] = s_fx[threadIdx.y];
				EdgeRow<NV> *edge = s_edge[threadIdx.y];
				const int rr = (step - 6) & (XROWS - 1);
				if (rr == 0) {
					fusexEdgeBatch<ORDER, NS>(a, eos, Uin, g, st, S, bx.lo[0] + bix * 64, cidx[DIR], hi, ot, edge);
					waveFence();
					stageEdgeRow<NV>(sx, edge[0]);
				}
				const double Dy = S[(S_AUX + 2) * T + cu];
				const int l = static_cast<int>(threadIdx.x) + 2;
				putColumn(sx, l, q[1]);
				waveFence();
				double amx[NV], apx[NV];
				reconstructCell<ORDER>(chiPrev, q[1], [&](int m, int n) { return sx[n][l + m]; }, amx, apx);
				const double uLeft = sx[PVX][l - 1];
				waveFence();
				putColumn(sx, l, apx);
				sx[NV][l] = Dy;
				sx[NV + 1][l] = dVprev;
				waveFence();
				double qLx[NV], Fx[NV], vfx;
				getColumn(sx, l - 1, qLx);
				const double dvl = sx[NV][l - 1], dwl = sx[NV + 1][l - 1];
				faceFluxAll<0, QK_RIEMANN_HLLC, false, NS>(eos, a.reconstruct_eint, 3, qLx, amx, q[1][PVX] - uLeft, dvl, Dy, dwl, dVprev, a.K_visc, Fx, vfx);
				waveFence();
				putColumn(sx, l, Fx);
				sx[NV][l] = vfx;
				waveFence();
#pragma unroll
				for (int n = 0; n < NV; ++n) {
					rhs_in[n] = a.inv_dx0 * (sx[n][lself] - sx[n][lnext]);
				}
				rhs_in[NV] = (sx[NV][lnext] - sx[NV][lself]) / a.dx0;
				waveFence();
				if (rr + 1 < XROWS) {
					stageEdgeRow<NV>(sx, edge[rr + 1]);
				}
			} else {
#pragma unroll
				for (int n = 0; n < NV + 1; ++n) {
					rhs_in[n] = streamLoad(&S[(S_RHS + n) * T + cu]);
				}
			}
			if (LAST && !ring && !(CARRY && STAGE == 2)) {
				const int64_t co = Uold.idx(cidx[0], cidx[1], cidx[2]);
#pragma unroll
				for (int n = 0; n < NV; ++n) {
					Uo[n] = Uold.p[co + Uold.ns * n];
				}
			}
			if (CARRY && LAST && STAGE == 2) {
				RA4 R1(a.rhs1[b]);
				const int64_t c1 = R1.idx(cidx[0], cidx[1], cidx[2]);
#pragma unroll
				for (int n = 0; n < NV + 1; ++n) {
					F1[n] = R1.p[c1 + R1.ns * n];
				}
			}
		}
		if (!CARRY && STAGE == 2 && step >= 5) {
			loadF1<NV>(a, b, fidx, F1);
		}
		double am[NV], ap[NV];
		reconstructCell<ORDER>(chi, q[2], [&](int m, int n) { return q[2 + m][n]; }, am, ap);
		if (step >= 5) {
			const double du = q[2][PVX + DIR] - q[1][PVX + DIR];
			double F[NV], vf;
			faceFluxAll<DIR, QK_RIEMANN_HLLC, TWOD, NS>(eos, a.reconstruct_eint, TWOD ? 2 : 3, apPrev, am, du, dVprev, dV, dWprev, dW, a.K_visc, F, vf);
			bool marked = false;
			if (maskCol && fidx[DIR] >= maskLo && cidx[DIR] <= maskHi) {
				CA4 M(a.fluxMask[b]);
				const int m0 = (cidx[DIR] >= maskLo) ? M(cidx[0], cidx[1], cidx[2]) : 0;
				const int m1 = (fidx[DIR] <= maskHi) ? M(fidx[0], fidx[1], fidx[2]) : 0;
				marked = (m0 | m1) != 0;
			}
			settleFace<STAGE, CARRY, FOFC, DIR, NS, TWOD>(a, eos, TWOD ? 2 : 3, b, fidx, live, marked, F1, q[1], q[2], F, vf);
			if (step >= 6) {
				double rhs[NV];
#pragma unroll
				for (int n = 0; n < NV; ++n) {
					rhs[n] = rhs_in[n] + a.inv_dx * (Fprev[n] - F[n]);
				}
				const double div_v = rhs_in[NV] + (vf - vfPrev) / a.dx;
				if (LAST) {
					if (live) {
						updateCellFrom<NS, CARRY ? STAGE : 0, FOFC, TWOD ? 2 : 3>(a, eos, ec, b, cidx[0], cidx[1], cidx[2], Uo, rhs, div_v, F1, sig0, sig1,
													    (STAGE == 1) && a.same_old && !a.reconstruct_eint && !a.prim_in, q[1][PPRES]);
					}
// ... 109 lines not shown
	const int nplanes = lev->maxlen[2] + 2;
	if (small) {
		return static_cast<int>(std::min<int64_t>((1024 + tiles - 1) / tiles, std::max(1, nplanes / smallMinLen())));
	}
	const int base = std::max(1, std::min(8, (nplanes + 15) / 30));
	int nseg = base;
	const double slots = 512.0;
	if (static_cast<double>(tiles) * base / slots < 6.0) {
		double best = 1e300;
		for (int c = std::max(1, base - 1); c <= base + 1; ++c) {
			const double rounds = static_cast<double>(tiles) * c / slots;
			const int seglen = (nplanes + c - 1) / c;
			const double cost = (std::ceil(rounds) / rounds) * (static_cast<double>(seglen + 6) / seglen);
			if (cost < best) {
				best = cost;
				nseg = c;
			}
		}
	}
	return nseg;
}

auto sweepArgsFor(SweepArgs a, const qk_hydro_stage_args *args, int d) -> SweepArgs
{
	a.halfFlux = args->halfFlux[d];
	a.halfVel = args->halfVel[d];
	a.rk2Flux = args->fluxRk2[d];
	a.rk2Vel = args->velRk2[d];
	a.inv_dx = 1.0 / args->dx[d];
	a.dx = args->dx[d];
	return a;
}

auto fusexApplies(const qk_level *lev, SweepArgs const &a, bool carry, int nscalars) -> bool
{
	const char *e = std::getenv("QK_FUSEX");
	if (!carry || nscalars != 0 || lev->ndim != 3 || a.fluxMask != nullptr || (e != nullptr && std::atoi(e) == 0)) {
		return false;
	}
	for (int b = 0; b < lev->nboxes; ++b) {
		if ((lev->boxes[b].hi[0] - lev->boxes[b].lo[0] + 1) % 64 != 0) {
			return false;
		}
	}
	return true;
}

template <int ORDER, int STAGE, int NS, bool CARRY, bool FOFC = false> void launchSweeps(qk_level *lev, hipStream_t s, SweepArgs a, Eos eos, const qk_hydro_stage_args *args)
{
	const bool fusex = fusexApplies(lev, a, CARRY, NS);
	if (!fusex) {
		const SweepArgs ax = sweepArgsFor(a, args, 0);
		const int64_t slab = static_cast<int64_t>(lev->maxlen[0] + 2 * NG) * lev->maxlen[1];
		const dim3 grid(static_cast<unsigned>((slab + XOUT - 1) / XOUT), static_cast<unsigned>(lev->maxlen[2]), static_cast<unsigned>(lev->nboxes));
		ProfScope ps(lev->ctx, s, "k_sweep_x");
		if (lev->ndim == 3) {
			hipLaunchKernelGGL((k_sweep_x<ORDER, STAGE, NS, CARRY, 3, FOFC>), grid, dim3(XB), 0, s, ax, eos);
		} else if constexpr (!CARRY) {
			if (lev->ndim == 2) {
				hipLaunchKernelGGL((k_sweep_x<ORDER, STAGE, NS, false, 2, FOFC>), grid, dim3(XB), 0, s, ax, eos);
			} else {
				hipLaunchKernelGGL((k_sweep_x<ORDER, STAGE, NS, false, 1, FOFC>), grid, dim3(XB), 0, s, ax, eos);
			}
		}
	}
	if (lev->ndim == 1) {
		return;
	}
	{
		SweepArgs ay = sweepArgsFor(a, args, 1);
		ay.same_old = (lev->ndim == 2) && (args->U_in == args->U_old);
		ay.nseg = marchSegments(lev, 1, 2);
		ay.inv_dx0 = 1.0 / args->dx[0];
		ay.dx0 = args->dx[0];
		const dim3 grid((lev->maxlen[0] + 63) / 64, (lev->maxlen[2] + MARCH_BY - 1) / MARCH_BY, lev->nboxes * ay.nseg);
		ProfScope ps(lev->ctx, s, fusex ? "k_sweep_xy" : "k_sweep_y");
		if (lev->ndim == 2) {
			if constexpr (!CARRY) {
				hipLaunchKernelGGL((k_sweep_march<1, ORDER, STAGE, true, NS, false, true, FOFC>), grid, dim3(64, MARCH_BY), 0, s, ay, eos);
			}
			return;
		}
		if constexpr (CARRY && !FOFC && NS == 0) {
			if (fusex) {
				hipLaunchKernelGGL((k_sweep_march<1, ORDER, STAGE, false, NS, CARRY, false, FOFC, true>), grid, dim3(64, MARCH_BY), 0, s, ay, eos);
			}
		}
		if (!fusex) {
			hipLaunchKernelGGL((k_sweep_march<1, ORDER, STAGE, false, NS, CARRY, false, FOFC>), grid, dim3(64, MARCH_BY), 0, s, ay, eos);
		}
	}
	{
		SweepArgs az = sweepArgsFor(a, args, 2);
		az.same_old = (args->U_in == args->U_old);
		az.nseg = marchSegments(lev, 2, 1);
		const dim3 grid((lev->maxlen[0] + 63) / 64, (lev->maxlen[1] + MARCH_BY - 1) / MARCH_BY, lev->nboxes * az.nseg);
		ProfScope ps(lev->ctx, s, "k_sweep_z");
		hipLaunchKernelGGL((k_sweep_march<2, ORDER, STAGE, true, NS, CARRY, false, FOFC>), grid, dim3(64, MARCH_BY), 0, s, az, eos);
	}
}

template <int ORDER, int NS> void launchStage(qk_level *lev, hipStream_t s, SweepArgs const &a, Eos const &eos, const qk_hydro_stage_args *args)
{
	auto form = [&](auto stage) {
		constexpr int STAGE = decltype(stage)::value;
		if (args->fofc_pass != 0) {
			launchSweeps<ORDER, STAGE, NS, false, true>(lev, s, a, eos, args);
		} else if (args->rk2_carry_rhs != 0) {
			launchSweeps<ORDER, STAGE, NS, true>(lev, s, a, eos, args);
		} else {
			launchSweeps<ORDER, STAGE, NS, false>(lev, s, a, eos, args);
		}
	};
	if (args->stage == 1) {
		form(std::integral_constant<int, 1>{});
	} else {
		form(std::integral_constant<int, 2>{});
	}
}
template <int ORDER> void launchOrder(int nscalars, qk_level *lev, hipStream_t s, SweepArgs const &a, Eos const &eos, const qk_hydro_stage_args *args)
{
	switch (nscalars) {
	case 0: return launchStage<ORDER, 0>(lev, s, a, eos, args);
	case 1: return launchStage<ORDER, 1>(lev, s, a, eos, args);
	case 2: return launchStage<ORDER, 2>(lev, s, a, eos, args);
	default: return launchStage<ORDER, 3>(lev, s, a, eos, args);
	}
}

}

extern "C" {

int64_t qk_hydro_stage_scratch_bytes(qk_level *lev, const qk_hydro_traits *t)
{
	if (lev == nullptr) {
		return QK_ERR_INVALID;
	}
	if (int rc = checkTraits(lev->ctx, t); rc != QK_OK) {
		return rc;
	}
	std::vector<SGeom> g;
	const int64_t cells = scratchGeom(lev, g);
	return cells * scratchComps(t->nscalars) * static_cast<int64_t>(sizeof(double));
}

int qk_hydro_stage_fused(qk_level *lev, qk_stream stream, const qk_hydro_traits *t, const qk_hydro_stage_args *args)
{
	if (lev == nullptr) {
		return QK_ERR_INVALID;
	}
	qk_ctx *ctx = lev->ctx;
	if (int rc = checkTraits(ctx, t); rc != QK_OK) {
		return rc;
	}
	if (int rc = needsLibraryEos(ctx, t, "qk_hydro_stage_fused (EnforceLimits)"); rc != QK_OK) {
		return rc;
	}
	QK_REQUIRE(ctx, args != nullptr, "qk_hydro_stage_fused: NULL args");
	if (lev->nboxes == 0) {
		return QK_OK;
	}
	if (t->nscalars > QK_FUSED_MAX_SCALARS || t->nmscalars != 0) {
		return setError(ctx, QK_ERR_UNSUPPORTED, "qk_hydro_stage_fused: up to 3 passive scalars, no mass scalars (use the reference-shaped operators)");
	}
	if (t->ndim != lev->ndim) {
		return setError(ctx, QK_ERR_INVALID, "qk_hydro_stage_fused: traits.ndim differs from the level's dimension");
	}
	if (t->ndim != 3 && args->rk2_carry_rhs != 0) {
		return setError(ctx, QK_ERR_UNSUPPORTED, "qk_hydro_stage_fused: rk2_carry_rhs is instantiated for 3-D builds");
	}
	QK_REQUIRE(ctx, args->K_visc >= 0.0, "qk_hydro_stage_fused: negative artificial-viscosity coefficient");
	QK_REQUIRE(ctx, args->stage == 1 || args->stage == 2, "qk_hydro_stage_fused: stage must be 1 or 2");
	QK_REQUIRE(ctx, args->reconstruction_order >= 1 && args->reconstruction_order <= 3, "qk_hydro_stage_fused: reconstruction_order must be 1..3");
	QK_REQUIRE(ctx, args->U_in && args->U_old && args->U_out && args->redoFlag && args->d_redo_count && args->d_error_flag && args->scratch,
		   "qk_hydro_stage_fused: NULL array");
	QK_REQUIRE(ctx, args->fofc_pass == 0 || (args->K_visc == 0.0 && (args->rk2_carry_rhs == 0 || args->stage == 1)),
		   "qk_hydro_stage_fused: the fused first-order flux correction pass needs K_visc == 0 and, in the carried-rhs form, stage 1 (use the reference-shaped operators otherwise)");
	QK_REQUIRE(ctx, args->rk2_carry_rhs == 0 || (args->rhs1 != nullptr && args->store_flux_rk2 == 0),
		   "qk_hydro_stage_fused: rk2_carry_rhs needs rhs1 and excludes store_flux_rk2 (flux_rk2 is formed on the faces flux_mask marks, nowhere else)");
	if (args->rk2_carry_rhs != 0 && args->flux_mask != nullptr) {
		for (int d = 0; d < t->ndim; ++d) {
			QK_REQUIRE(ctx, args->halfFlux[d] != nullptr && args->fluxRk2[d] != nullptr && args->fluxRk2[d] != args->halfFlux[d],
				   "qk_hydro_stage_fused: flux_mask needs halfFlux[d] and a distinct fluxRk2[d]");
		}
	}
	for (int d = 0; d < t->ndim; ++d) {
		QK_REQUIRE(ctx, args->rk2_carry_rhs != 0 || (args->halfFlux[d] && args->halfVel[d]), "qk_hydro_stage_fused: NULL halfFlux/halfVel");
		QK_REQUIRE(ctx, args->store_flux_rk2 == 0 || args->stage != 2 || (args->fluxRk2[d] != nullptr && args->fluxRk2[d] != args->halfFlux[d]),
			   "qk_hydro_stage_fused: store_flux_rk2 needs fluxRk2[d], distinct from halfFlux[d]");
		QK_REQUIRE(ctx, lev->maxlen[d] >= 1, "qk_hydro_stage_fused: empty box");
	}
	if (args->store_vel_rk2 != 0) {
		QK_REQUIRE(ctx, args->rk2_carry_rhs == 0, "qk_hydro_stage_fused: store_vel_rk2 excludes rk2_carry_rhs (the carried form has no halfVel to average with)");
		QK_REQUIRE(ctx, args->stage == 2, "qk_hydro_stage_fused: store_vel_rk2 belongs to stage 2 (stage 1 leaves its face velocity in halfVel)");
		for (int d = 0; d < t->ndim; ++d) {
			QK_REQUIRE(ctx, args->velRk2[d] != nullptr, "qk_hydro_stage_fused: store_vel_rk2 needs velRk2[d]");
			QK_REQUIRE(ctx, args->velRk2[d] != args->halfVel[d],
				   "qk_hydro_stage_fused: store_vel_rk2 needs velRk2[d] distinct from halfVel[d] (the x sweep evaluates a tile-boundary face in both tiles, and both need v1 intact)");
		}
	}
	QK_REQUIRE(ctx, args->scratch_bytes >= qk_hydro_stage_scratch_bytes(lev, t), "qk_hydro_stage_fused: scratch too small");
	if (args->prim_in != 0 || args->prim_out != 0) {
		QK_REQUIRE(ctx, t->reconstruct_eint == 0 && !Eos(*t).isothermal && t->eos_temperature_model == 0,
			   "qk_hydro_stage_fused: the primitive hand-off is the gamma-law, reconstruct_eint = 0 form");
		QK_REQUIRE(ctx, args->fofc_pass == 0, "qk_hydro_stage_fused: the primitive hand-off has no correction pass (redo the step without it)");
		QK_REQUIRE(ctx, (args->prim_out == 0 || args->stage == 1) && (args->prim_in == 0 || (args->stage == 2 && args->U_in != args->U_old)),
			   "qk_hydro_stage_fused: prim_out belongs to stage 1, prim_in to stage 2 (whose old state is a different array)");
	}

	if (int rc = buildGeom(lev); rc != QK_OK) {
		return rc;
	}
	auto s = static_cast<hipStream_t>(stream);
	const Eos eos(*t);
	const bool re = (t->reconstruct_eint != 0);
	auto *scratch = static_cast<double *>(args->scratch);
	const int64_t T = lev->sgeom_total_cells;
	const SGeom *geom = static_cast<const SGeom *>(lev->d_sgeom);
	const qk_box *boxes = lev->d_boxes;

	{
		ProfScope ps(ctx, s, "k_pre");
		const int xt = (lev->maxlen[0] + 2 + PT_X - 1) / PT_X, yt = (lev->maxlen[1] + 2 + PT_Y - 1) / PT_Y;
		const int nseg = prePassSegments(lev, xt, yt);
		const dim3 grid(static_cast<unsigned>(xt) * yt * lev->nboxes * nseg);
		if (args->prim_in != 0) {
			hipLaunchKernelGGL(k_pre3<true>, grid, dim3(PT_THREADS), 0, s, boxes, geom, args->U_in, scratch, T, eos, re, nseg, xt, yt, t->ndim);
		} else {
			hipLaunchKernelGGL(k_pre3<false>, grid, dim3(PT_THREADS), 0, s, boxes, geom, args->U_in, scratch, T, eos, re, nseg, xt, yt, t->ndim);
		}
	}

	SweepArgs a{};
	a.boxes = boxes;
	a.geom = geom;
	a.scratch = scratch;
	a.total_cells = T;
	a.U_in = args->U_in;
	a.U_old = args->U_old;
	a.U_out = args->U_out;
	a.redoFlag = args->redoFlag;
	a.redo_count = reinterpret_cast<unsigned long long *>(args->d_redo_count);
	a.error_flag = args->d_error_flag;
	a.max_signal = args->d_max_signal;
	a.dt = args->dt;
	a.densityFloor = args->densityFloor;
	a.tempFloor = args->tempFloor;
	a.K_visc = args->K_visc;
	a.use_dual_energy = args->use_dual_energy;
	a.reconstruct_eint = re;
	a.store_rk2 = (args->store_flux_rk2 != 0);
	a.store_vel = (args->store_vel_rk2 != 0);
	a.rhs1 = args->rhs1;
	a.fluxMask = (args->rk2_carry_rhs != 0) ? args->flux_mask : nullptr;
	a.prim_in = (args->prim_in != 0);
	a.prim_out = (args->prim_out != 0);
	for (int d = 0; d < 3; ++d) {
		a.dx3[d] = args->dx[d];
	}

	if (args->reconstruction_order == 3) {
		launchOrder<3>(t->nscalars, lev, s, a, eos, args);
	} else if (args->reconstruction_order == 2) {
		launchOrder<2>(t->nscalars, lev, s, a, eos, args);
	} else {
		launchOrder<1>(t->nscalars, lev, s, a, eos, args);
	}
	QK_HIP_CHECK(ctx, hipGetLastError());
	return QK_OK;
}

}
```

### quokka_amd/csrc/qk_internal.hpp

```cpp
#ifndef QK_INTERNAL_HPP_
#define QK_INTERNAL_HPP_

#include <hip/hip_runtime.h>

#include <cstdio>
#include <mutex>
#include <string>
#include <vector>

#include "quokka_amd.h"

struct qk_prof_pending {
	int slot;
	hipEvent_t start, stop;
};
struct qk_prof_slot {
	std::string name;
	long count = 0;
	double total_ms = 0.0;
};

struct qk_ctx {
	int device = 0;
	std::string last_error;
	std::vector<void *> owned;
	std::mutex mtx;
	bool profiling = false;
	std::string prof_only;
	std::vector<qk_prof_slot> prof_slots;
	std::vector<qk_prof_pending> prof_pending;
	std::vector<hipEvent_t> prof_free_events;
	int *counter_slots = nullptr;
	int cooling_libm = 0;
};

struct qk_level {
	qk_ctx *ctx = nullptr;
	int ndim = 3;
	int nboxes = 0;
	std::vector<qk_box> boxes;
	qk_box *d_boxes = nullptr;
	int maxlen[3] = {0, 0, 0};
	void *d_sgeom = nullptr;
	int64_t sgeom_total_cells = 0;
	int *d_tile_flags = nullptr;
	size_t tile_flags_bytes = 0;
	unsigned long long *d_cooling_queue = nullptr;
};

namespace qk
{

inline auto setError(qk_ctx *ctx, int code, const char *what, const char *detail = "") -> int
{
	if (ctx != nullptr) {
		std::lock_guard<std::mutex> lock(ctx->mtx);
		ctx->last_error = std::string(what) + (detail[0] != 0 ? ": " : "") + detail;
	}
	return code;
}

#define QK_HIP_CHECK(ctx, expr)                                                                                                                      \
	do {                                                                                                                                         \
		hipError_t qk_e_ = (expr);                                                                                                           \
		if (qk_e_ != hipSuccess) {                                                                                                           \
			return qk::setError((ctx), QK_ERR_HIP, #expr, hipGetErrorString(qk_e_));                                                     \
		}                                                                                                                                    \
	} while (0)

#define QK_REQUIRE(ctx, cond, msg)                                                                                                                   \
	do {                                                                                                                                         \
		if (!(cond)) {                                                                                                                       \
			return qk::setError((ctx), QK_ERR_INVALID, msg);                                                                             \
		}                                                                                                                                    \
	} while (0)

inline auto checkTraits(qk_ctx *ctx, const qk_hydro_traits *t) -> int
{
	if (t == nullptr) {
		return setError(ctx, QK_ERR_INVALID, "traits is NULL");
	}
	if (t->nscalars < 0 || t->nscalars > QK_MAX_SCALARS || t->nmscalars < 0 || t->nmscalars > t->nscalars) {
		return setError(ctx, QK_ERR_UNSUPPORTED, "0..QK_MAX_SCALARS passive scalars, of which the first nmscalars (0..nscalars) are mass scalars");
	}
	if (t->eos_temperature_model != QK_HOOK_COMPILED &&
	    (t->eos_temperature_model < 0 || t->eos_temperature_model > 1 || (t->eos_temperature_model == 1 && !(t->eos_alpha > 0.0)))) {
		return setError(ctx, QK_ERR_UNSUPPORTED, "eos_temperature_model must be 0 (gamma law), 1 (E = alpha / 4 T^4, alpha > 0) or QK_HOOK_COMPILED");
	}
	if (t->ndim < 1 || t->ndim > 3) {
		return setError(ctx, QK_ERR_UNSUPPORTED, "ndim must be 1, 2 or 3");
	}
	return QK_OK;
}

inline auto needsLibraryEos(qk_ctx *ctx, const qk_hydro_traits *t, const char *who) -> int
{
	if (t->eos_temperature_model == QK_HOOK_COMPILED) {
		return setError(ctx, QK_ERR_UNSUPPORTED, who,
				"the quokka::EOS temperature hooks of this problem are compiled device code: instantiate the kernel in the problem's translation unit "
				"(quokka_amd/host/qk_problem_kernels.hpp)");
	}
	return QK_OK;
}

struct CellLaunch {
	dim3 grid;
	dim3 block;
};

inline auto cellLaunch(const qk_level *lev, int ng, int facedir) -> CellLaunch
{
	int64_t n = 1;
	for (int d = 0; d < 3; ++d) {
		int len = lev->maxlen[d];
		if (d < lev->ndim) {
			len += 2 * ng;
		}
		if (d == facedir) {
			len += 1;
		}
		n *= len;
	}
	CellLaunch L;
	L.block = dim3(256, 1, 1);
	L.grid = dim3(static_cast<unsigned>((n + 255) / 256), static_cast<unsigned>(lev->nboxes), 1);
	return L;
}

struct ProfScope {
	qk_ctx *ctx;
// ... 44 lines not shown
```

### quokka_amd/host/quokka_host.hpp

```cpp
#ifndef QK_HOST_QUOKKA_HOST_HPP_
#define QK_HOST_QUOKKA_HOST_HPP_

#include "quokka_amr_simulation.hpp"
#include "compat/grackle_like_cooling.hpp"
#include "compat/tabulated_cooling.hpp"

template <typename problem_t> class QuokkaSimulation : public AMRSimulation<problem_t>
{
      public:
	using B = AMRSimulation<problem_t>;
	using B::BCs_cc_;
	using B::cflNumber_;
	using B::densityFloor_;
	using B::dt_;
	using B::geom;
	using B::grids_;
	using B::istep;
	using B::maxTimesteps_;
	using B::nghost_cc_;
	using B::state_new_cc_;
	using B::state_old_cc_;
	using B::stopTime_;
	using B::tempFloor_;
	using B::tNew_;
// ... 364 lines not shown
		} else {
			amrex::MultiFab::Copy(state_new_cc_[0], state_old_cc_[0], 0, 0, ncompHydro_, 0);
		}
		if constexpr (is_radiation_enabled_) {
			subcycleRadiationAtLevel(time, dt_lev);
		}
		callAfterLevelAdvance(time, dt_lev);
		return true;
	}

      private:
	void construct()
	{
		amrex::ParmParse hpp("hydro");
		hpp.query("rk_integrator_order", integratorOrder_);
		hpp.query("reconstruction_order", reconstructionOrder_);
		hpp.query("use_dual_energy", useDualEnergy_);
		hpp.query("abort_on_fofc_failure", abortOnFofcFailure_);
		hpp.query("artificial_viscosity_coefficient", artificialViscosityK_);
		{
			amrex::ParmParse qpp("qk");
			qpp.query("fused_fofc", fusedFofc_);
		}
		hpp.query("rk2_carry_rhs", rk2CarryRhs_);
		{
			amrex::ParmParse cpp("cooling");
			int alwaysReadTables = 0;
			cpp.query("enabled", enableCooling_);
			cpp.query("read_tables_even_if_disabled", alwaysReadTables);
			cpp.query("cooling_table_type", coolingTableType_);
			cpp.query("hdf5_data_file", coolingTableFilename_);
			if ((enableCooling_ == 1) || (alwaysReadTables == 1)) {
				if (coolingTableType_ == "cloudy_cooling_tools") {
					amrex::Print() << "Reading cloudy-cooling-tools tables...\n";
					quokka::TabulatedCooling::readCloudyData(coolingTableFilename_, cloudyTables_);
				} else if (coolingTableType_ == "grackle") {
					amrex::Print() << "Reading Grackle tables...\n";
					quokka::GrackleLikeCooling::readGrackleData(coolingTableFilename_, grackleTables_);
				} else {
					amrex::Abort("Invalid cooling table type!");
				}
			}
		}
		amrex::ParmParse rpp("radiation");
		rpp.query("reconstruction_order", radiationReconstructionOrder_);
		rpp.query("cfl", radiationCflNumber_);
		rpp.query("dust_gas_interaction_coeff", dustGasInteractionCoeff_);
		rpp.query("max_substeps", maxSubsteps_);
		{
			int ti = 0;
			rpp.query("source_is_time_independent", ti);
			radSourceTimeIndependent_ = (ti != 0);
		}
		std::string walltime;
		if (amrex::ParmParse().query("max_walltime", walltime)) {
			int h = 0, m = 0, sec = 0;
			if (std::sscanf(walltime.c_str(), "%d:%d:%d", &h, &m, &sec) == 3) {
				maxWalltime_ = 3600L * h + 60L * m + sec;
			}
		}
		defineComponentNames();
		allocate();
	}

      public:
	void defineComponentNames()
	{
		this->componentNames_cc_ = {"gasDensity", "x-GasMomentum", "y-GasMomentum", "z-GasMomentum", "gasEnergy", "gasInternalEnergy"};
		if constexpr (is_radiation_enabled_) {
			for (int i = 0; i < Physics_Traits<problem_t>::nGroups; ++i) {
				for (auto const *name : {"radEnergy-Group", "x-RadFlux-Group", "y-RadFlux-Group", "z-RadFlux-Group"}) {
					this->componentNames_cc_.push_back(name + std::to_string(i));
				}
			}
		}
	}

	void WritePlotFile();
	void WriteCheckpointFile();
	long maxWalltime_ = 0;
	int lastPlotFileStep_ = 0, lastChkFileStep_ = 0;
	void outputAfterInitialConditions()
	{
		if (this->restart_chkfile.empty() && this->checkpointInterval_ > 0) {
			WriteCheckpointFile();
		}
		if (this->plotfileInterval_ > 0) {
			WritePlotFile();
		}
		lastPlotFileStep_ = lastChkFileStep_ = istep[0];
	}
	void outputAfterStep(int step)
	{
		if (this->plotfileInterval_ > 0 && (step + 1) % this->plotfileInterval_ == 0) {
			lastPlotFileStep_ = step + 1;
			WritePlotFile();
		}
		if (this->checkpointInterval_ > 0 && (step + 1) % this->checkpointInterval_ == 0) {
			lastChkFileStep_ = step + 1;
			WriteCheckpointFile();
		}
	}
	void outputAfterEvolve()
	{
		if (this->plotfileInterval_ > 0 && istep[0] > lastPlotFileStep_) {
			WritePlotFile();
		}
		if (this->checkpointInterval_ > 0 && istep[0] > lastChkFileStep_) {
			WriteCheckpointFile();
		}
	}
	[[nodiscard]] auto walltimeExceeded(std::chrono::steady_clock::time_point t0) const -> bool
	{
		return maxWalltime_ > 0 && std::chrono::duration<double>(std::chrono::steady_clock::now() - t0).count() > 0.9 * static_cast<double>(maxWalltime_);
	}

	void setInitialConditionsOnGrid(quokka::grid const &grid_elem) override;
	void setInitialConditionsOnGridFaceVars(quokka::grid const &grid_elem) override;
	using AMRSimulation<problem_t>::componentNames_fc;
	void preCalculateInitialConditions() override;
	void computeAfterEvolve(amrex::Vector<amrex::Real> &initSumCons) override;
	void computeAfterTimestep();
	void ComputeDerivedVar(int lev, std::string const &dname, amrex::MultiFab &mf, int ncomp) const;
	[[nodiscard]] auto ComputeProjections(int dir) const -> std::unordered_map<std::string, amrex::BaseFab<amrex::Real>>;
	auto ComputeStatistics() -> std::map<std::string, amrex::Real>;
	template <typename F> auto computeAxisAlignedProfile(int axis, F const &user_f) -> amrex::Gpu::HostVector<amrex::Real>;
	void addStrangSplitSources(amrex::MultiFab &state, int lev, amrex::Real time, amrex::Real dt_lev);
	void createInitialParticles();
	void computeBeforeTimestep();
	void dropCachedSignal() { invalidateSignal(); }
	void callAfterTimestep()
	{
		computeAfterTimestep();
		if (!afterTimestepIsDefault_) {
			invalidateSignal();
		}
	}
	void computeAfterLevelAdvance(int lev, amrex::Real time, amrex::Real dt_lev, int ncycle);
	void callAfterLevelAdvance(double time, double dt_lev)
	{
		computeAfterLevelAdvance(this->amrLevel_, time, dt_lev, 1);
		if (!afterLevelAdvanceIsDefault_) {
			invalidateSignal();
		}
	}
	void callBeforeTimestep()
	{
		computeBeforeTimestep();
		if (!beforeTimestepIsDefault_) {
			invalidateSignal();
		}
	}
	void computeReferenceSolution(amrex::MultiFab & , amrex::GpuArray<amrex::Real, AMREX_SPACEDIM> const & ,
				      amrex::GpuArray<amrex::Real, AMREX_SPACEDIM> const & )
	{
	}

	void computeTimestep()
	{
		double m = 0.0;
		if constexpr (!Physics_Traits<problem_t>::is_hydro_enabled) {
			static_assert(is_radiation_enabled_, "At least one of hydro or radiation must be enabled! Cannot compute a time step.");
			m = RadSystem<problem_t>::c_hat_;
		} else {
			resolveSignal();
			m = (haveSignal_ ? signal_[1] : HydroSystem<problem_t>::maxSignalSpeedLocal(state_new_cc_[0], 1));
		}
		if constexpr (is_radiation_enabled_ && Physics_Traits<problem_t>::is_hydro_enabled) {
			m = std::max(RadSystem<problem_t>::c_hat_ / static_cast<double>(maxSubsteps_), m);
		}
		double dt_tmp = cflNumber_ * (minDx() / m);
		dt_tmp = std::min(dt_tmp, 1.1 * dt_[0]);
		double dt_0 = std::min(dt_tmp, 1.0 * dt_tmp);
		dt_0 = std::min(dt_0, this->maxDt_);
		if (tNew_[0] == 0.0) {
			dt_0 = std::min(dt_0, this->initDt_);
		}
		if (this->constantDt_ > 0.0) {
			dt_0 = this->constantDt_;
		}
		double const eps = 1.e-3 * dt_0;
		if (tNew_[0] + dt_0 > stopTime_ - eps) {
			dt_0 = stopTime_ - tNew_[0];
		}
		dt_[0] = dt_0;
	}

// ... 538 lines not shown
		QK_HOST_HIP(hipMemsetAsync(d_count_, 0, sizeof(int64_t), nullptr));
		HydroSystem<problem_t>::ComputeRhsFromFluxes(rhs_, fl, geom[0].CellSizeArray(), ncompHydro_);
		HydroSystem<problem_t>::AddInternalEnergyPdV(rhs_, stateOld, geom[0].CellSizeArray(), vl, redoFlag_);
		HydroSystem<problem_t>::PredictStep(stateOld, stateNew, rhs_, dt, ncompHydro_, redoFlag_, d_count_);
		return readCount();
	}

	void fillFlagGhosts()
	{
		for (size_t k = 0; k < flagPeers_.peer.size(); ++k) {
			qkhost::check(qk_FillBoundary_pack_int(flagPlan_, nullptr, static_cast<int>(k), qkhost::itab(redoFlag_), static_cast<int *>(flagPeers_.send[k])),
				      "redoFlag pack");
		}
		qkhost::Comm::get().exchangeBegin(flagPeers_.peer, flagPeers_.send, flagPeers_.nsend, flagPeers_.recv, flagPeers_.nrecv, sizeof(int), nullptr);
		qkhost::check(qk_FillBoundary_local_int(flagPlan_, nullptr, qkhost::itab(redoFlag_)), "redoFlag.FillBoundary");
		qkhost::Comm::get().exchangeEnd(nullptr);
		for (size_t k = 0; k < flagPeers_.peer.size(); ++k) {
			qkhost::check(qk_FillBoundary_unpack_int(flagPlan_, nullptr, static_cast<int>(k), qkhost::itab(redoFlag_), static_cast<const int *>(flagPeers_.recv[k])),
				      "redoFlag unpack");
		}
	}

	bool unfusedRan_ = false;
	auto stageUnfused(int stageNo, amrex::MultiFab const &U_in, amrex::MultiFab const &U_old, amrex::MultiFab &U_out, double dt) -> bool
	{
		unfusedRan_ = true;
		auto *lev = qkhost::Runtime::get().lev;
		computeHydroFluxes(U_in);
		auto *fl = &flux_;
		auto *vl = &vel_;
		if (stageNo == 1) {
			for (int d = 0; d < AMREX_SPACEDIM; ++d) {
				amrex::MultiFab::Copy(halfFlux_[d], flux_[d]);
				amrex::MultiFab::Copy(halfVel_[d], vel_[d]);
			}
		} else {
			for (int d = 0; d < AMREX_SPACEDIM; ++d) {
				rk2flux_[d].setVal(0);
				rk2vel_[d].setVal(0);
				qkhost::check(qk_Saxpy(lev, nullptr, d, qkhost::tab(rk2flux_[d]), 0.5, qkhost::tab(halfFlux_[d]), ncompHydro_), "Saxpy");
				qkhost::check(qk_Saxpy(lev, nullptr, d, qkhost::tab(rk2vel_[d]), 0.5, qkhost::tab(halfVel_[d]), 1), "Saxpy");
				qkhost::check(qk_Saxpy(lev, nullptr, d, qkhost::tab(rk2flux_[d]), 0.5, qkhost::tab(flux_[d]), ncompHydro_), "Saxpy");
				qkhost::check(qk_Saxpy(lev, nullptr, d, qkhost::tab(rk2vel_[d]), 0.5, qkhost::tab(vel_[d]), 1), "Saxpy");
			}
			fl = &rk2flux_;
			vl = &rk2vel_;
		}
		redoFlag_.setVal(0);
		int64_t nbad = rhsPdvPredict(*fl, *vl, U_old, U_out, dt);
		if (nbad > 0) {
			++fofcStages_;
			computeFOHydroFluxes(U_old);
			fillFlagGhosts();
			for (int d = 0; d < AMREX_SPACEDIM; ++d) {
				qkhost::check(qk_replaceFluxes(lev, nullptr, d, qkhost::tab((*fl)[d]), qkhost::tab(FOflux_[d]), qkhost::itab(redoFlag_), ncompHydro_),
					      "replaceFluxes");
				qkhost::check(qk_replaceFluxes(lev, nullptr, d, qkhost::tab((*vl)[d]), qkhost::tab(FOvel_[d]), qkhost::itab(redoFlag_), 1), "replaceFluxes");
			}
			nbad = rhsPdvPredict(*fl, *vl, U_old, U_out, dt);
			if (stageNo == 1 && integratorOrder_ == 1) {
				for (int d = 0; d < AMREX_SPACEDIM; ++d) {
					amrex::MultiFab::Copy(halfFlux_[d], flux_[d]);
				}
			}
			if (nbad > 0 && abortOnFofcFailure_ != 0) {
				return false;
			}
		}
		HydroSystem<problem_t>::EnforceLimits(densityFloor_, tempFloor_, U_out);
		if (useDualEnergy_ == 1) {
			HydroSystem<problem_t>::SyncDualEnergy(U_out, d_error_);
		}
		return true;
	}

	[[nodiscard]] static constexpr auto fusedEligible() -> bool
	{
		return HydroSystem<problem_t>::nscalars_ <= 3 && Physics_Traits<problem_t>::numMassScalars == 0;
	}
	[[nodiscard]] auto isFinalStage(int stageNo) const -> bool { return (stageNo == 2) || (integratorOrder_ == 1); }
	[[nodiscard]] auto carryActive() const -> bool { return AMREX_SPACEDIM == 3 && rk2CarryRhs_ != 0 && integratorOrder_ == 2 && !storeFluxRk2_ && !forceExactForm_; }
	bool forceExactForm_ = false;

	struct OverlapGroup {
		std::vector<int> idx;
		qk_level *lev = nullptr;
		std::map<const void *, void *> tables;
	};
	OverlapGroup groups_[2];
	OverlapGroup specNear_, specFar_;
	std::vector<OverlapGroup> specFarParts_;
	hipStream_t farStream_ = nullptr;
	hipEvent_t evInterReady_ = nullptr, evFarDone_ = nullptr;
	void *farScratch_ = nullptr;
	int64_t farScratchBytes_ = 0;
	double *d_fixFar_ = nullptr;
	bool fixFarPending_ = false;
	static void releaseGroup(OverlapGroup &G)
	{
		for (auto &kv : G.tables) {
			(void)hipFree(kv.second);
		}
		G.tables.clear();
		if (G.lev != nullptr) {
			qk_level_destroy(G.lev);
			G.lev = nullptr;
		}
		G.idx.clear();
	}
	int overlapState_ = 0;
	amrex::Long minOverlapCells_ = 8L * 128 * 128 * 128;

	auto overlapActive() -> bool
	{
		if (overlapState_ == 0) {
			overlapState_ = 2;
			amrex::ParmParse pq("qk");
			pq.query("min_overlap_cells", minOverlapCells_);
			if (!this->beforePhysBC_ && fusedEligible()) {
				amrex::Long cells[2] = {0, 0};
				for (int b = 0; b < static_cast<int>(grids_.size()); ++b) {
					int const g = (qk_ghost_plan_box_is_remote(this->plan_, b) == 1) ? 1 : 0;
					groups_[g].idx.push_back(b);
					cells[g] += grids_[b].numPts();
				}
				if (!groups_[0].idx.empty() && !groups_[1].idx.empty() && std::min(cells[0], cells[1]) >= minOverlapCells_) {
					for (auto &g : groups_) {
						std::vector<qk_box> qb;
						for (int b : g.idx) {
							qb.push_back({{grids_[b].lo[0], grids_[b].lo[1], grids_[b].lo[2]}, {grids_[b].hi[0], grids_[b].hi[1], grids_[b].hi[2]}});
						}
						qkhost::check(qk_level_create(qkhost::Runtime::get().ctx, &g.lev, AMREX_SPACEDIM, static_cast<int>(qb.size()), qb.data()), "qk_level_create");
					}
					overlapState_ = 1;
					std::cout << "rank " << qkhost::Comm::get().rank << ": overlapped ghost fill: " << groups_[0].idx.size() << " early / " << groups_[1].idx.size()
						  << " late boxes\n";
				}
			}
		}
		return overlapState_ == 1;
	}
	template <typename D> auto groupTable(int g, D *full) -> D * { return groupTableOf(groups_[g], full); }
	template <typename D> static auto groupTableOf(OverlapGroup &G, D *full) -> D *
	{
		if (full == nullptr) {
			return nullptr;
		}
		auto &m = G.tables;
		auto it = m.find(full);
		if (it == m.end()) {
			void *p = nullptr;
			QK_HOST_HIP(hipMalloc(&p, sizeof(D) * G.idx.size()));
			for (size_t n = 0; n < G.idx.size(); ++n) {
				QK_HOST_HIP(hipMemcpy(static_cast<D *>(p) + n, full + G.idx[n], sizeof(D), hipMemcpyDeviceToDevice));
			}
			it = m.emplace(full, p).first;
		}
		return static_cast<D *>(it->second);
	}

	void fusedBegin(int stageNo, bool bothSlots = false)
	{
		hipStream_t const cs = qkhost::Runtime::get().computeStream();
		(void)stageNo;
		QK_HOST_HIP(hipMemsetAsync(d_words_, 0, 3 * sizeof(int64_t), cs));
		if (bothSlots) {
			QK_HOST_HIP(hipMemsetAsync(d_words_ + 4, 0, 3 * sizeof(int64_t), cs));
		}
	}
	void readWords(StageWords w[2])
	{
		int64_t h[8];
		QK_HOST_HIP(hipMemcpy(h, d_words_, sizeof(h), hipMemcpyDeviceToHost));
		double v[8];
		for (int sl = 0; sl < 2; ++sl) {
			std::memcpy(&v[4 * sl], &h[4 * sl], 2 * sizeof(double));
			v[4 * sl + 2] = static_cast<double>(h[4 * sl + 2]);
			v[4 * sl + 3] = static_cast<double>(h[4 * sl + 3] & 0xFFFFFFFFLL);
		}
		if (qkhost::Comm::get().size > 1) {
			qkhost::Comm::get().allReduce(v, 8, qkhost::Comm::Op::max);
		}
		for (int sl = 0; sl < 2; ++sl) {
			w[sl].sig[0] = v[4 * sl];
			w[sl].sig[1] = v[4 * sl + 1];
			w[sl].count = static_cast<int64_t>(v[4 * sl + 2]);
			w[sl].err = static_cast<int64_t>(v[4 * sl + 3]);
		}
	}
	void fusedLaunch(int stageNo, amrex::MultiFab const &U_in, amrex::MultiFab const &U_old, amrex::MultiFab &U_out, double dt, int group = -1, bool fofc = false,
			 int slot = 0, OverlapGroup *grp = nullptr, void *scratch = nullptr, int64_t scratchBytes = 0, hipStream_t stream = nullptr)
	{
		auto t = qkhost::traits<problem_t>();
		if (grp == nullptr && group >= 0) {
			grp = &groups_[group];
		}
		auto sel = [&](qk_array4 *full) { return grp == nullptr ? full : groupTableOf(*grp, full); };
		qk_hydro_stage_args a{};
		a.U_in = sel(qkhost::tab(U_in));
		a.U_old = sel(qkhost::tab(U_old));
		a.U_out = sel(qkhost::tab(U_out));
		for (int d = 0; d < 3; ++d) {
			a.halfFlux[d] = (d < AMREX_SPACEDIM) ? sel(qkhost::tab(halfFlux_[d])) : nullptr;
			a.halfVel[d] = (d < AMREX_SPACEDIM) ? sel(qkhost::tab(halfVel_[d])) : nullptr;
			a.dx[d] = (d < AMREX_SPACEDIM) ? geom[0].dx[d] : 1.0;
		}
		a.redoFlag = grp == nullptr ? qkhost::itab(redoFlag_) : groupTableOf(*grp, qkhost::itab(redoFlag_));
		a.d_redo_count = d_words_ + 4 * slot + 2;
		a.d_error_flag = reinterpret_cast<int *>(d_words_ + 4 * slot + 3);
		if (isFinalStage(stageNo)) {
			a.d_max_signal = reinterpret_cast<double *>(d_words_ + 4 * slot);
		}
		a.scratch = (scratch != nullptr) ? scratch : scratch_;
		a.scratch_bytes = (scratch != nullptr) ? scratchBytes : scratchBytes_;
		a.dt = dt;
		a.stage = stageNo;
		a.reconstruction_order = reconstructionOrder_;
		a.densityFloor = densityFloor_;
		a.tempFloor = tempFloor_;
		a.use_dual_energy = useDualEnergy_;
		a.K_visc = artificialViscosityK_;
		bool const masked = carryActive() && fluxMask_.size() > 0;
		a.store_flux_rk2 = (!carryActive() && needsFluxRk2()) ? 1 : 0;
		for (int d = 0; d < 3; ++d) {
			a.fluxRk2[d] = ((a.store_flux_rk2 != 0 || masked) && d < AMREX_SPACEDIM) ? sel(qkhost::tab(rk2flux_[d])) : nullptr;
		}
		if (masked) {
			auto *full = reinterpret_cast<qk_carray4 *>(fluxMask_.arrays());
			a.flux_mask = grp == nullptr ? full : groupTableOf(*grp, full);
		}
		if (carryActive()) {
			if (rhs1_.size() == 0) {
				rhs1_.define(grids_, ncompHydro_ + 1, 0);
			}
			a.rk2_carry_rhs = 1;
			a.rhs1 = sel(qkhost::tab(rhs1_));
		}
		a.fofc_pass = fofc ? 1 : 0;
		if (primNow_ && !fofc) {
			a.prim_out = (stageNo == 1) ? 1 : 0;
			a.prim_in = (stageNo == 2) ? 1 : 0;
		}
		qkhost::check(qk_hydro_stage_fused(grp == nullptr ? qkhost::Runtime::get().lev : grp->lev, stream != nullptr ? stream : qkhost::Runtime::get().computeStream(), &t, &a),
			      "qk_hydro_stage_fused");
	}
	auto fusedEnd(int stageNo, StageWords const *given = nullptr) -> int64_t
	{
		StageWords w[2];
		if (given == nullptr) {
			readWords(w);
			given = &w[0];
		}
		if (given->err != 0) {
			amrex::Abort("density is negative in SyncDualEnergy! abort!!");
		}
		int64_t const nbad = given->count;
		if (nbad == 0) {
			stage1LeftF1_ = (stageNo == 1) ? !carryActive() : stage1LeftF1_;
			if (isFinalStage(stageNo)) {
				signal_[0] = given->sig[0];
				signal_[1] = given->sig[1];
				haveSignal_ = true;
			}
		}
		return nbad;
	}
	auto redoStageUnfused(int stageNo, amrex::MultiFab const &U_in, amrex::MultiFab const &U_old, amrex::MultiFab &U_out, double dt) -> bool
	{
		if (stageNo == 2 && !stage1LeftF1_) {
			computeHydroFluxes(U_old);
			for (int d = 0; d < AMREX_SPACEDIM; ++d) {
				amrex::MultiFab::Copy(halfFlux_[d], flux_[d]);
				amrex::MultiFab::Copy(halfVel_[d], vel_[d]);
			}
		}
		if (stageNo == 1) {
			stage1LeftF1_ = true;
		}
		return stageUnfused(stageNo, U_in, U_old, U_out, dt);
	}

	auto correctStage(int stageNo, amrex::MultiFab const &U_in, amrex::MultiFab const &U_old, amrex::MultiFab &U_out, double dt) -> bool
	{
		if (stageNo == 1) {
			stage1LeftF1_ = !carryActive();
		}
		bool const applies = fusedFofc_ != 0 && artificialViscosityK_ == 0.0 && !(integratorOrder_ == 1 && storeFluxRk2_);
		if (!applies) {
			return redoStageUnfused(stageNo, U_in, U_old, U_out, dt);
		}
		if (carryActive() && stageNo == 2) {
			++fofcStages_;
			forceExactForm_ = true;
			fusedBegin(1);
			fusedLaunch(1, U_old, U_old, U_out, dt);
			stage1LeftF1_ = true;
			fusedBegin(2);
			fusedLaunch(2, U_in, U_old, U_out, dt);
			int64_t nbad = fusedEnd(2);
			if (nbad > 0) {
				fillFlagGhosts();
				fusedBegin(2);
				fusedLaunch(2, U_in, U_old, U_out, dt, -1, true);
				nbad = fusedEnd(2);
			}
			forceExactForm_ = false;
			return !(nbad > 0 && abortOnFofcFailure_ != 0);
		}
		++fofcStages_;
		fillFlagGhosts();
		fusedBegin(stageNo);
		fusedLaunch(stageNo, U_in, U_old, U_out, dt, -1, true);
		return !(fusedEnd(stageNo) > 0 && abortOnFofcFailure_ != 0);
	}

	auto stage(int stageNo, amrex::MultiFab const &U_in, amrex::MultiFab const &U_old, amrex::MultiFab &U_out, double dt) -> bool
	{
		if constexpr (fusedEligible()) {
			fusedBegin(stageNo);
			fusedLaunch(stageNo, U_in, U_old, U_out, dt);
			if (fusedEnd(stageNo) == 0) {
				return true;
			}
			return correctStage(stageNo, U_in, U_old, U_out, dt);
		}
		return redoStageUnfused(stageNo, U_in, U_old, U_out, dt);
	}

	auto fillAndStage(int stageNo, amrex::MultiFab &U_in, amrex::MultiFab const &U_old, amrex::MultiFab &U_out, double dt) -> bool
	{
		if constexpr (fusedEligible()) {
			if (overlapActive()) {
				fusedBegin(stageNo);
				launchStage(stageNo, U_in, U_old, U_out, dt, 0);
				if (fusedEnd(stageNo) == 0) {
					return true;
				}
				return correctStage(stageNo, U_in, U_old, U_out, dt);
			}
		}
		this->fillBoundaryConditions(U_in);
		return stage(stageNo, U_in, U_old, U_out, dt);
	}
	void launchStage(int stageNo, amrex::MultiFab &U_in, amrex::MultiFab const &U_old, amrex::MultiFab &U_out, double dt, int slot)
	{
		if (overlapActive()) {
			this->fillBoundaryConditions(U_in, [&]() { fusedLaunch(stageNo, U_in, U_old, U_out, dt, 0, false, slot); });
			fusedLaunch(stageNo, U_in, U_old, U_out, dt, 1, false, slot);
			return;
		}
		this->fillBoundaryConditions(U_in);
		fusedLaunch(stageNo, U_in, U_old, U_out, dt, -1, false, slot);
	}
	auto stagePairSpeculative(amrex::MultiFab &U_old, double time, double dt) -> int
	{
		if (primBackoff_ > 0) {
			--primBackoff_;
		} else if (primHandoffApplies()) {
			primNow_ = true;
			fusedBegin(1, true);
			fillTime_ = time;
			launchStage(1, U_old, U_old, state_inter_cc_, dt, 0);
			fillTime_ = time + dt;
			launchStage(2, state_inter_cc_, U_old, state_new_cc_[0], dt, 1);
			primNow_ = false;
			StageWords w[2];
			readWords(w);
			if (w[0].count == 0 && w[1].count == 0) {
				fusedEnd(1, &w[0]);
				fusedEnd(2, &w[1]);
				primBackoffLen_ = 0;
				return 1;
			}
			++primHandoffDropped_;
			primBackoffLen_ = std::min(64, std::max(4, 2 * primBackoffLen_));
			primBackoff_ = primBackoffLen_;
			invalidateSignal();
		}
		fusedBegin(1, true);
		fillTime_ = time;
		launchStage(1, U_old, U_old, state_inter_cc_, dt, 0);
		fillTime_ = time + dt;
		launchStage(2, state_inter_cc_, U_old, state_new_cc_[0], dt, 1);
		StageWords w[2];
		readWords(w);
		if (fusedEnd(1, &w[0]) != 0) {
			return -1;
		}
		if (fusedEnd(2, &w[1]) == 0) {
			return 1;
		}
		return correctStage(2, state_inter_cc_, U_old, state_new_cc_[0], dt) ? 1 : 0;
	}
	[[nodiscard]] auto primHandoffApplies() -> bool
	{
		if (primHandoffChecked_) {
			return primHandoffOk_;
		}
		if (this->customBcIsDefault_ < 0) {
			return false;
		}
		primHandoffChecked_ = true;
		int on = 1;
		amrex::ParmParse("qk").query("prim_handoff", on);
		auto const t = qkhost::traits<problem_t>();
		bool ok = on != 0 && this->customBcIsDefault_ == 1 && this->amrLevel_ == 0 && !is_radiation_enabled_ && t.reconstruct_eint == 0 &&
			  t.eos_temperature_model == 0 && !(t.cs_isothermal == t.cs_isothermal) && t.gamma != 1.0 &&
			  Physics_Indices<problem_t>::nvarTotal_cc == ncompHydro_;
		for (auto const &bc : this->BCs_cc_) {
			for (int d = 0; d < AMREX_SPACEDIM; ++d) {
				ok = ok && bc.lo(d) != amrex::BCType::ext_dir && bc.hi(d) != amrex::BCType::ext_dir && bc.lo(d) != amrex::BCType::hoextrap &&
				     bc.hi(d) != amrex::BCType::hoextrap;
			}
		}
		primHandoffOk_ = ok;
		return ok;
	}
	bool primHandoffChecked_ = false, primHandoffOk_ = false, primNow_ = false;
	long primHandoffDropped_ = 0;
	int primBackoff_ = 0, primBackoffLen_ = 0;
	int rk2CarryRhs_ = 0;
	int fusedFofc_ = 1;
	bool stage1LeftF1_ = true;
	amrex::MultiFab rhs1_;
};

template <typename problem_t> void QuokkaSimulation<problem_t>::preCalculateInitialConditions() {}
template <typename problem_t> void QuokkaSimulation<problem_t>::setInitialConditionsOnGridFaceVars(quokka::grid const & ) {}

template <typename problem_t> void QuokkaSimulation<problem_t>::computeAfterTimestep() { afterTimestepIsDefault_ = true; }
template <typename problem_t> void QuokkaSimulation<problem_t>::computeBeforeTimestep() { beforeTimestepIsDefault_ = true; }
// ... 94 lines not shown
```

### quokka_amd/simulation.py

```python
from __future__ import annotations

import ctypes as C
import math
import os
from dataclasses import dataclass
from typing import Callable, List, Optional, Sequence, Tuple

import numpy as np
import torch

from . import capi
from .hydro_system import HydroSystem, HyperbolicSystem, Saxpy, replaceFluxes
from .multifab import Context, Level, MultiFab

NGHOST_CC = 4


def chop_domain(n_cell: Sequence[int], max_grid_size: Sequence[int]) -> List[Tuple[List[int], List[int]]]:
    nb = [(n_cell[d] + max_grid_size[d] - 1) // max_grid_size[d] for d in range(3)]
    boxes = []
    for kb in range(nb[2]):
        for jb in range(nb[1]):
            for ib in range(nb[0]):
                lo, hi = [], []
# ... 168 lines not shown
        L = self.lev.ctx.L
        return [b for b in range(self.lev.nboxes) if L.qk_ghost_plan_box_is_remote(self.h, b) == 1]

    def set_box_remote(self, b: int, flag: bool):
        self.lev.ctx.check(self.lev.ctx.L.qk_ghost_plan_set_box_remote(self.h, b, int(flag)), "qk_ghost_plan_set_box_remote")

    def items(self, kind: int, k: int = 0):
        L = self.lev.ctx.L
        out = []
        for idx in range(L.qk_ghost_plan_num_items(self.h, kind, k)):
            db, sb, off = C.c_int(), C.c_int(), C.c_int64()
            lo, hi, sh = (C.c_int * 3)(), (C.c_int * 3)(), (C.c_int * 3)()
            self.lev.ctx.check(L.qk_ghost_plan_item(self.h, kind, k, idx, C.byref(db), C.byref(sb), lo, hi, sh, C.byref(off)), "qk_ghost_plan_item")
            out.append((db.value, sb.value, list(lo), list(hi), list(sh), off.value))
        return out

    def __del__(self):
        try:
            self.lev.ctx.L.qk_ghost_plan_destroy(self.h)
        except Exception:
            pass


class HydroSimulation:

    def __init__(self, ctx: Context, geom: Geometry, traits: capi.HydroTraits, bcs, max_grid_size=None, dirichlet=None,
                 rank: int = 0, nranks: int = 1, use_fused: bool = True, ncomp_cc: int = 6, boxes=None, owner=None):
        self.ctx, self.geom, self.traits = ctx, geom, traits
        self.rank, self.nranks = rank, nranks
        self.hydro = HydroSystem(traits)
        self.ncomp_cc = ncomp_cc
        mgs = list(max_grid_size) if max_grid_size is not None else list(geom.n_cell)
        mgs = (mgs + [1, 1, 1])[:3]
        for d in range(geom.ndim, 3):
            mgs[d] = 1
        self.all_boxes = [(list(lo), list(hi)) for lo, hi in boxes] if boxes is not None else chop_domain(geom.n_cell, mgs)
        if owner is not None:
            self.owner = list(owner)
        else:
            self.owner = distribute_boxes(self.all_boxes, nranks, geom.n_cell, mgs) if nranks > 1 else [0] * len(self.all_boxes)
        self.my_boxes = [b for b, o in zip(self.all_boxes, self.owner) if o == rank]
        assert self.my_boxes or owner is not None, "rank owns no boxes"
        self.lev = Level(ctx, geom.ndim, self.my_boxes)
        self.stopTime_ = 1.0
        self.cflNumber_ = 0.3
        self.maxTimesteps_ = 10000
        self.maxDt_ = float("inf")
        self.initDt_ = float("inf")
        self.constantDt_ = 0.0
        self.densityFloor_ = 0.0
        self.tempFloor_ = 0.0
        self.integratorOrder_ = 2
        self.reconstructionOrder_ = 3
        self.useDualEnergy_ = 1
        self.abortOnFofcFailure_ = 1
        self.artificialViscosityK_ = 0.0
        self.do_tracers = 0
        self.tracers = None
        self.tracers_on_fused_stages = 0
        self.doPoissonSolve_ = 0
        self.Gconst_ = 6.67430e-8
        self.reltolPoisson_ = 1.0e-5
        self.abstolPoisson_ = 1.0e-5
        self.do_cic_particles = 0
        self.phi = None
        self.poisson = None
        self.on_gravity = None
        self._avg_face_vel = None
        self.min_overlap_cells = 8 * 128 ** 3
        self.use_fused = use_fused and traits.nscalars <= 3 and traits.nmscalars == 0
        lev = self.lev
        self.state_old_cc_ = MultiFab(lev, self.ncomp_cc, NGHOST_CC, fill=0.0)
        self.state_new_cc_ = MultiFab(lev, self.ncomp_cc, NGHOST_CC, fill=0.0)
        self.state_old_tmp = MultiFab(lev, self.ncomp_cc, NGHOST_CC, fill=0.0)
        self.state_inter_cc_ = MultiFab(lev, self.ncomp_cc, NGHOST_CC, fill=0.0)
        self.tNew_ = 0.0
        self.dt_ = 1.0e100
        self.istep = 0
        self.cellUpdates_ = 0
        self.counters = {"fofc1_stages": 0, "fofc2_stages": 0, "retries": 0}
        self.strang_sources = []
        self.ghost = GhostExchange(lev, geom, self.ncomp_cc, NGHOST_CC, self.all_boxes, self.owner, rank, bcs, dirichlet)
        self.flag_ghost = None
        nd = geom.ndim
        self.halfFlux = [MultiFab(lev, self.hydro.nvar_, 0, facedir=d) for d in range(nd)]
        self.halfVel = [MultiFab(lev, 1, 0, facedir=d) for d in range(nd)]
        self.redoFlag = MultiFab(lev, 1, 1, dtype=torch.int32, fill=0)
        self._dev_words = torch.zeros(8, dtype=torch.int64, device=ctx.device)
        self.speculate_stage2 = True
        self.prim_handoff = os.environ.get("QK_PRIM_HANDOFF", "1") == "1"
        self._prim_now = False
        self._has_dirichlet = dirichlet is not None
        self.dev_counters = self._dev_words[2:3]
        self.dev_error = self._dev_words[3:4].view(torch.int32)[0:1]
        self._err_latched = False
        self._unfused_ran = False
        self.dev_max = torch.zeros(1, dtype=torch.float64, device=ctx.device)
        self.dev_signal = self._dev_words[0:2].view(torch.float64)
        self._dev_fix = torch.zeros(8, dtype=torch.int64, device=ctx.device)
        self._fix_far_words = False
        self._fix_words_pending = False
        self._signal_of_state_new = None
        self.scratch = None
        if self.use_fused:
            nbytes = ctx.L.qk_hydro_stage_scratch_bytes(lev.h, C.byref(traits))
            assert nbytes > 0 or not self.my_boxes
            self.scratch = torch.empty(max(nbytes // 8, 1), dtype=torch.float64, device=ctx.device)
        self._unfused_tmp = None

    def CountCells(self) -> int:
        return sum(int(np.prod([hi[d] - lo[d] + 1 for d in range(3)])) for lo, hi in self.all_boxes)

    def fillBoundaryConditions(self, state: MultiFab):
        self.ghost.fill(state)

    def set_initial_conditions(self, fn: Callable[[np.ndarray, np.ndarray, np.ndarray], np.ndarray]):
        for b, (lo, hi) in enumerate(self.my_boxes):
            k, j, i = np.meshgrid(np.arange(lo[2], hi[2] + 1), np.arange(lo[1], hi[1] + 1), np.arange(lo[0], hi[0] + 1), indexing="ij")
            vals = fn(i, j, k)
            self.state_new_cc_.valid(b).copy_(torch.from_numpy(np.ascontiguousarray(vals)))
        self.fillBoundaryConditions(self.state_new_cc_)
        self.state_old_cc_.copy_from(self.state_new_cc_)
        if self.do_tracers:
            self.InitTracerParticles()
        if self.doPoissonSolve_:
            self.calculateGpotAllLevels()

    def calculateGpotAllLevels(self):
        if not self.doPoissonSolve_:
            return
        from . import gravity
        gravity.check_supported(self)
        if self.poisson is None:
            self.poisson = gravity.PoissonSolver(self.ctx, self.geom.n_cell, self.geom.dx[0])
        ps = self.poisson
        ps.zero_rhs()
        ps.fill_rhs(self.lev, self.state_new_cc_, self.Gconst_, 0)
        ps.solve_open(self.reltolPoisson_, self.abstolPoisson_)
        self.phi = ps.phi

    def gravAccelAllLevels(self, dt: float):
        if not self.doPoissonSolve_:
            return
        if self.phi is None:
            raise capi.QkError("gravAccelAllLevels: no potential (calculateGpotAllLevels has not run)")
        self.poisson.kick(self.lev, self.state_new_cc_, self.geom.dx, dt)
        self._signal_of_state_new = None

    def ellipticSolveAllLevels(self, dt: float):
        if not self.doPoissonSolve_:
            return
        self.calculateGpotAllLevels()
        if self.on_gravity is not None:
            self.on_gravity(self, dt)
        self.gravAccelAllLevels(dt)

    def InitTracerParticles(self):
        if not self.do_tracers:
            raise capi.QkError("InitTracerParticles: do_tracers is 0")
        self._check_tracers()
        from .tracers import TracerParticles
        self.tracers = TracerParticles(self)
        self.tracers.init_one_per_cell()

    def _check_tracers(self):
        from .amr_simulation import AmrLevelSim
        if type(self) is not HydroSimulation and type(self) is not AmrLevelSim:
            raise capi.QkError(f"do_tracers: tracer particles are built for HydroSimulation and the hydro levels of AmrSimulation, not for "
                               f"{type(self).__name__} (radiation)")
        if self.nranks > 1:
            raise capi.QkError("do_tracers: tracer particles are built for one rank (nranks > 1: no particle exchange between ranks)")
        if self.integratorOrder_ != 2:
            raise capi.QkError("do_tracers: tracer particles need integratorOrder_ = 2 (the RK2 average of the face velocities)")

    def _allreduce_max(self, x: float) -> float:
        if self.nranks > 1:
            import torch.distributed as dist
            from . import comm
            t = torch.tensor([x], dtype=torch.float64, device=self.ctx.device)
            comm.all_reduce(t, dist.ReduceOp.MAX)
            return float(t.item())
        return x

    def _allreduce_sum(self, x: int) -> int:
        if self.nranks > 1:
            import torch.distributed as dist
            from . import comm
            t = torch.tensor([x], dtype=torch.int64, device=self.ctx.device)
            comm.all_reduce(t, dist.ReduceOp.SUM)
            return int(t.item())
        return x

    def min_dx(self) -> float:
        return min(self.geom.dx[: self.geom.ndim])

    @property
    def _signal_of_state_new(self):
# ... 132 lines not shown
        self._unfused_ran = True
        self.counters["operator_stages"] = self.counters.get("operator_stages", 0) + 1
        t, lev, nd = self._tmp(), self.lev, self.geom.ndim
        self.computeHydroFluxes(U_in, t["flux"], t["vel"])
        if stage == 1:
            for d in range(nd):
                self.halfFlux[d].copy_from(t["flux"][d])
                self.halfVel[d].copy_from(t["vel"][d])
            fl, vl = t["flux"], t["vel"]
        else:
            for d in range(nd):
                t["rk2flux"][d].storage.zero_()
                t["rk2vel"][d].storage.zero_()
                Saxpy(lev, d, t["rk2flux"][d], 0.5, self.halfFlux[d], self.hydro.nvar_)
                Saxpy(lev, d, t["rk2vel"][d], 0.5, self.halfVel[d], 1)
                Saxpy(lev, d, t["rk2flux"][d], 0.5, t["flux"][d], self.hydro.nvar_)
                Saxpy(lev, d, t["rk2vel"][d], 0.5, t["vel"][d], 1)
            fl, vl = t["rk2flux"], t["rk2vel"]
        self.redoFlag.storage.zero_()
        nbad = self._rhs_pdv_predict(fl, vl, U_old, U_out, dt)
        if nbad > 0 and with_fofc:
            self.counters["fofc1_stages" if stage == 1 else "fofc2_stages"] += 1
            self.computeFOHydroFluxes(U_old, t["FOflux"], t["FOvel"])
            self._fill_flag_ghosts()
            for d in range(nd):
                replaceFluxes(lev, d, fl[d], t["FOflux"][d], self.redoFlag, self.hydro.nvar_)
                replaceFluxes(lev, d, vl[d], t["FOvel"][d], self.redoFlag, 1)
            nbad = self._rhs_pdv_predict(fl, vl, U_old, U_out, dt)
            if nbad > 0 and self.abortOnFofcFailure_ != 0:
                return False
        self._limits_and_sync(U_out)
        if stage == 2:
            self._avg_face_vel = vl
        if stage == 2 and self._needs_flux_rk2():
            for d in range(nd):
                self.fluxRk2()[d].copy_from(fl[d])
        elif stage == 1 and self.integratorOrder_ == 1 and getattr(self, "store_flux_rk2", False):
            for d in range(nd):
                self.halfFlux[d].copy_from(fl[d])
        return True

    def fluxRk2(self):
        if getattr(self, "_fluxRk2", None) is None:
            self._fluxRk2 = [MultiFab(self.lev, self.hydro.nvar_, 0, facedir=d, fill=0.0) for d in range(self.geom.ndim)]
        return self._fluxRk2

    def _needs_flux_rk2(self) -> bool:
        return bool(getattr(self, "store_flux_rk2", False)) or getattr(self, "flux_mask", None) is not None

    def _carry_active(self) -> bool:
        return (bool(getattr(self, "rk2_carry_rhs", False)) and self.integratorOrder_ == 2 and not getattr(self, "store_flux_rk2", False)
                and self.geom.ndim == 3 and not getattr(self, "_force_exact_form", False) and not self._tracers_on_fused())

    def _tracers_on_fused(self) -> bool:
        return bool(self.tracers_on_fused_stages) and self.use_fused and bool(self.do_tracers) and self.tracers is not None

    def velRk2(self):
        if getattr(self, "_velRk2", None) is None:
            self._velRk2 = [MultiFab(self.lev, 1, 0, facedir=d, fill=0.0) for d in range(self.geom.ndim)]
        return self._velRk2

    def rhs1(self):
        if getattr(self, "_rhs1", None) is None:
            self._rhs1 = MultiFab(self.lev, self.hydro.nvar_ + 1, 0, fill=0.0)
        return self._rhs1

    def _prim_handoff_applies(self) -> bool:
        return type(self) is HydroSimulation and self._prim_handoff_state_ok()

    def _prim_handoff_state_ok(self) -> bool:
        t = self.traits
        return (self.prim_handoff and not self._has_dirichlet and self.ncomp_cc == self.hydro.nvar_
                and t.reconstruct_eint == 0 and t.cs_isothermal != t.cs_isothermal and t.eos_temperature_model == 0 and t.gamma != 1.0)

    def _is_final(self, stage: int) -> bool:
        return (stage == 2) or (self.integratorOrder_ == 1)

    def _fused_begin(self, stage: int, slot: int = 0, both: bool = False):
        if self._unfused_ran and not self._err_latched:
            self._err_latched = int(self.dev_error.item()) != 0
        c = self.ctx
        c.check(c.L.qk_clear_bytes(c.h, c.stream(), C.c_void_p(self._dev_words.data_ptr() + (0 if both else 32 * slot)), 64 if both else 32), "qk_clear_bytes")

    def _fused_launch(self, stage: int, U_in, U_old, U_out, dt, group=None, fofc: bool = False, slot: int = 0, scratch=None):
        lev, idx = (self.lev, None) if group is None else group
        tab = (lambda mf: mf.ptr) if idx is None else (lambda mf: mf.subset_ptr(idx))
        a = capi.StageArgs()
        a.U_in, a.U_old, a.U_out = tab(U_in), tab(U_old), tab(U_out)
        nd = self.geom.ndim
        for d in range(3):
            a.halfFlux[d] = tab(self.halfFlux[d]) if d < nd else None
            a.halfVel[d] = tab(self.halfVel[d]) if d < nd else None
            a.dx[d] = self.geom.dx[d] if d < nd else 1.0
        a.redoFlag = tab(self.redoFlag)
        w = self._dev_words.data_ptr() + 32 * slot
        a.d_redo_count = C.c_void_p(w + 16)
        a.d_error_flag = C.c_void_p(w + 24)
        if self._is_final(stage):
            a.d_max_signal = C.c_void_p(w)
        sc = self.scratch if scratch is None else scratch
        a.scratch = C.c_void_p(sc.data_ptr())
        a.scratch_bytes = sc.numel() * 8
        a.dt, a.stage, a.reconstruction_order = dt, stage, self.reconstructionOrder_
        a.densityFloor, a.tempFloor, a.use_dual_energy, a.K_visc = self.densityFloor_, self.tempFloor_, self.useDualEnergy_, float(self.artificialViscosityK_)
        mask = getattr(self, "flux_mask", None)
        if self._carry_active():
            a.rk2_carry_rhs = 1
            a.rhs1 = tab(self.rhs1())
            if mask is not None:
                a.flux_mask = tab(mask)
        else:
            a.store_flux_rk2 = int(self._needs_flux_rk2())
        if a.store_flux_rk2 or a.flux_mask:
            for d in range(nd):
                a.fluxRk2[d] = tab(self.fluxRk2()[d])
        if stage == 2 and self._tracers_on_fused():
            a.store_vel_rk2 = 1
            for d in range(nd):
                a.velRk2[d] = tab(self.velRk2()[d])
        a.fofc_pass = int(fofc)
        if self._prim_now and not fofc:
            a.prim_out, a.prim_in = int(stage == 1), int(stage == 2)
        c = self.ctx
        c.check(c.L.qk_hydro_stage_fused(lev.h, c.stream(), C.byref(self.traits), C.byref(a)), "qk_hydro_stage_fused")

    def _read_words(self):
        if self.nranks > 1:
            import torch.distributed as dist
            from . import comm
            w = self._dev_words.view(2, 4)
            v = torch.cat([w[:, 0:2].reshape(-1).view(torch.float64).view(2, 2), w[:, 2:3].to(torch.float64),
                           (w[:, 3:4] & 0xFFFFFFFF).to(torch.float64)], dim=1).reshape(-1)
            comm.all_reduce(v, dist.ReduceOp.MAX)
            vals = v.tolist()
            return [vals[0:4], vals[4:8]]
        hw = self.__dict__.get("_host_words")
        if hw is None:
            hw = self.__dict__["_host_words"] = torch.zeros(8, dtype=torch.int64).pin_memory()
            self.__dict__["_host_words_np"] = hw.numpy()
        hw.copy_(self._dev_words, non_blocking=True)
        torch.cuda.current_stream(self.ctx.device).synchronize()
        a = self.__dict__["_host_words_np"]
        f = a.view(np.float64)
        return [[float(f[4 * s]), float(f[4 * s + 1]), float(a[4 * s + 2]), float(int(a[4 * s + 3]) & 0xFFFFFFFF)] for s in (0, 1)]

    def _fused_end(self, stage: int, slot: int = 0, vals=None) -> int:
        final = self._is_final(stage)
        vals = (self._read_words() if vals is None else vals)[slot]
        self._err_latched = self._err_latched or vals[3] != 0.0
        nbad = int(vals[2])
        if final and nbad == 0:
            self._signal_of_state_new = (vals[0], vals[1])
        return nbad

    def overlap_groups(self):
        late = self.ghost.remote_boxes()
        key = tuple(late)
        if getattr(self, "_groups_key", None) != key:
            early = [b for b in range(self.lev.nboxes) if b not in set(late)]
            self._groups = None
            cells = lambda idx: sum(int(np.prod([self.my_boxes[b][1][d] - self.my_boxes[b][0][d] + 1 for d in range(3)])) for b in idx)
            if early and late and min(cells(early), cells(late)) >= self.min_overlap_cells:
                mk = lambda idx: (Level(self.ctx, self.geom.ndim, [self.my_boxes[b] for b in idx]), idx)
                self._groups = (mk(early), mk(late))
            self._groups_key = key
        return self._groups

    def _before_fill(self, stage: int, dt: float):
        """hook: a refined level sets the time its coarse-fine ghost cells are interpolated to"""

    def _launch_stage(self, stage, U_in, U_old, U_out, dt, slot: int = 0):
        self._before_fill(stage, dt)
        groups = self.overlap_groups()
        if groups is None:
            self.fillBoundaryConditions(U_in)
            self._fused_launch(stage, U_in, U_old, U_out, dt, slot=slot)
            return
        early, late = groups
        self.ghost.fill(U_in, between=lambda: self._fused_launch(stage, U_in, U_old, U_out, dt, early, slot=slot))
        self._fused_launch(stage, U_in, U_old, U_out, dt, late, slot=slot)

    def _finish_stage(self, stage, U_in, U_old, U_out, dt, nbad: int) -> bool:
        if nbad == 0:
            self._stage1_left_F1 = (stage == 1 and not self._carry_active())
            self._fused_stage_stood(stage)
            return True
        return self._correct_stage(stage, U_in, U_old, U_out, dt)

    def _fused_stage_stood(self, stage: int):
        if stage == 2 and self._tracers_on_fused():
            self._avg_face_vel = self.velRk2()

    def _fill_and_stage(self, stage, U_in, U_old, U_out, dt, fused: Optional[bool] = None) -> bool:
        if not (self.use_fused if fused is None else fused):
            self._before_fill(stage, dt)
            self.fillBoundaryConditions(U_in)
            return self._redo_stage_unfused(stage, U_in, U_old, U_out, dt)
        self._fused_begin(stage)
        self._launch_stage(stage, U_in, U_old, U_out, dt)
        return self._finish_stage(stage, U_in, U_old, U_out, dt, self._fused_end(stage))

    def _stage(self, stage, U_in, U_old, U_out, dt) -> bool:
        if self.use_fused:
            self._fused_begin(stage)
            self._fused_launch(stage, U_in, U_old, U_out, dt)
            return self._finish_stage(stage, U_in, U_old, U_out, dt, self._fused_end(stage))
        return self._redo_stage_unfused(stage, U_in, U_old, U_out, dt)

    def _correct_stage(self, stage, U_in, U_old, U_out, dt) -> bool:
        if stage == 1:
            self._stage1_left_F1 = not self._carry_active()
        ok = self._fofc_fused(stage, U_in, U_old, U_out, dt)
        if ok is not None:
            return ok
        return self._redo_stage_unfused(stage, U_in, U_old, U_out, dt)

    def _fofc_fused(self, stage, U_in, U_old, U_out, dt):
        if (not getattr(self, "fused_fofc", True) or float(self.artificialViscosityK_) != 0.0
                or (self.integratorOrder_ == 1 and getattr(self, "store_flux_rk2", False))):
            return None
        if self._carry_active() and stage == 2:
            return self._fofc_stage2_of_carried_form(U_in, U_old, U_out, dt)
        self.counters["fofc1_stages" if stage == 1 else "fofc2_stages"] += 1
        self._fill_flag_ghosts()
        self._fused_begin(stage)
        self._fused_launch(stage, U_in, U_old, U_out, dt, fofc=True)
        nbad = self._fused_end(stage)
        self._fused_stage_stood(stage)
        return not (nbad > 0 and self.abortOnFofcFailure_ != 0)

    def _fofc_stage2_of_carried_form(self, U_in, U_old, U_out, dt) -> bool:
        self.counters["fofc2_stages"] += 1
        self._force_exact_form = True
        try:
            self._fused_begin(1)
            self._fused_launch(1, U_old, U_old, U_out, dt)
            self._stage1_left_F1 = True
            self._fused_begin(2)
            self._fused_launch(2, U_in, U_old, U_out, dt)
            nbad = self._fused_end(2)
            if nbad > 0:
                self._fill_flag_ghosts()
                self._fused_begin(2)
                self._fused_launch(2, U_in, U_old, U_out, dt, fofc=True)
                nbad = self._fused_end(2)
        finally:
            self._force_exact_form = False
        return not (nbad > 0 and self.abortOnFofcFailure_ != 0)

    def _redo_stage_unfused(self, stage, U_in, U_old, U_out, dt) -> bool:
        if stage == 2 and self.use_fused and not getattr(self, "_stage1_left_F1", True):
            self.computeHydroFluxes(U_old, self.halfFlux, self.halfVel)
        if stage == 1:
            self._stage1_left_F1 = True
        return self._stage_unfused(stage, U_in, U_old, U_out, dt, with_fofc=True)

    def add_strang_source(self, source) -> None:
        self.strang_sources.append(source)

    def _strang_sources(self, state: MultiFab, time: float, dt: float) -> bool:
        ok = True
        for src in self.strang_sources:
            ok = src(state, time, dt) and ok
        return ok

    def advanceHydroAtLevel(self, state_old_tmp: MultiFab, dt_lev: float, time: Optional[float] = None) -> bool:
        time = (self.tNew_ - self.dt_) if time is None else time
        if self.strang_sources and not self._strang_sources(state_old_tmp, time, 0.5 * dt_lev):
            return False
        self._signal_of_state_new = None
        self._err_latched, self._unfused_ran = False, False
        with_tracers = bool(self.do_tracers) and self.tracers is not None
        if with_tracers:
            self._check_tracers()
        fused = self.use_fused and (not with_tracers or self._tracers_on_fused())
        self._avg_face_vel = None
        pair_done = False
        self._prim_now = False
        if getattr(self, "_prim_backoff", 0) > 0:
            self._prim_backoff -= 1
        elif fused and self.integratorOrder_ == 2 and self.speculate_stage2 and self._prim_handoff_applies():
            inter, new = self.state_inter_cc_, self.state_new_cc_
            self._prim_now = True
            try:
                self._fused_begin(1, both=True)
                self._launch_stage(1, state_old_tmp, state_old_tmp, inter, dt_lev, slot=0)
                self._launch_stage(2, inter, state_old_tmp, new, dt_lev, slot=1)
            finally:
                self._prim_now = False
            vals = self._read_words()
            latched = self._err_latched
            if self._fused_end(1, 0, vals) == 0 and self._fused_end(2, 1, vals) == 0:
# ... 345 lines not shown
```

Baseline: 3299 Mcell-updates/s.

## Read ghost cells directly from neighbour boxes instead of filling ghost zones

Adds a per-level face map that gives, for each box face, the source box, index transform and reflection sign. The fused hydro kernels then read halo cells straight from neighbouring boxes' interiors, flipping momentum signs at reflecting walls. The separate FillBoundary/physical-boundary pass before each RK stage is skipped, and ghosts are marked stale and filled lazily only before output or a correction stage. This removes the ghost-exchange kernels and their memory traffic. In exchange, the stage kernels do more complex, less coalesced address computation at box edges and take on extra correctness risk.

```diff
diff --git a/include/quokka_amd.h b/include/quokka_amd.h
--- a/include/quokka_amd.h
+++ b/include/quokka_amd.h
@@ -118,6 +118,7 @@
 int qk_advect_AddFluxesRK2(qk_level *lev, qk_stream s, qk_array4 *U_new, const qk_array4 *U0, const qk_array4 *U1, const qk_array4 *const fluxArray[3], double dt,
 			   const double dx[3], int nvars);
 
+#define QK_GHOST_FROM_SOURCE_ON 0x51475331
 typedef struct qk_hydro_stage_args {
 	const qk_array4 *U_in;
 	const qk_array4 *U_old;
@@ -147,6 +148,7 @@
 	int prim_in;
 	int store_vel_rk2;
 	qk_array4 *velRk2[3];
+	int ghost_from_source;
 } qk_hydro_stage_args;
 
 int64_t qk_hydro_stage_scratch_bytes(qk_level *lev, const qk_hydro_traits *t);
@@ -249,6 +251,9 @@
 int qk_ghost_plan_set_box_remote(qk_ghost_plan *plan, int local_box, int flag);
 int qk_FillPhysicalBoundary_subset(qk_ghost_plan *plan, qk_stream s, qk_array4 *state, const qk_bcrec *bcs, const qk_dirichlet_face *dirichlet,
 				   int which);
+
+int qk_ghost_source_plan(qk_level *lev, const qk_geometry *geom, int nghost, int ncomp, const qk_bcrec *bcs, int n_all, int *qualifies);
+int qk_ghost_source_lookup(qk_level *lev, int box, const int idx[3], int *src_box, int src_idx[3], int flip[3]);
 
 typedef struct qk_carray4 {
 	char *p;
diff --git a/quokka_amd/capi.py b/quokka_amd/capi.py
--- a/quokka_amd/capi.py
+++ b/quokka_amd/capi.py
@@ -15,6 +15,7 @@
 COOLING_LIBM_DEVICE, COOLING_LIBM_PORTABLE = 0, 1
 RIEMANN_HLLC, RIEMANN_LLF, RIEMANN_HLLD = 0, 1, 2
 LIMITER_MINMOD, LIMITER_MC = 0, 1
+GHOST_FROM_SOURCE_ON = 0x51475331
 BC_REFLECT_ODD, BC_INT_DIR, BC_REFLECT_EVEN, BC_FOEXTRAP, BC_EXT_DIR = -1, 0, 1, 2, 3
 
 K_B = 1.380649e-16
@@ -93,7 +94,8 @@
                 ("densityFloor", C.c_double), ("tempFloor", C.c_double), ("use_dual_energy", C.c_int), ("K_visc", C.c_double),
                 ("store_flux_rk2", C.c_int), ("fluxRk2", C.c_void_p * 3), ("rk2_carry_rhs", C.c_int), ("rhs1", C.c_void_p), ("flux_mask", C.c_void_p), ("fofc_pass", C.c_int),
                 ("prim_out", C.c_int), ("prim_in", C.c_int),
-                ("store_vel_rk2", C.c_int), ("velRk2", C.c_void_p * 3)]
+                ("store_vel_rk2", C.c_int), ("velRk2", C.c_void_p * 3),
+                ("ghost_from_source", C.c_int)]
 
 
 def traits(gamma=1.4, reconstruct_eint=True, ndim=3, mean_molecular_weight=M_U, boltzmann_constant=K_B,
@@ -195,6 +197,9 @@
         L.qk_ghost_plan_set_components.argtypes = [vp, C.c_int, C.c_int]
         L.qk_ghost_plan_box_is_remote.argtypes = [vp, C.c_int]
         L.qk_ghost_plan_set_box_remote.argtypes = [vp, C.c_int, C.c_int]
+    if hasattr(L, "qk_ghost_source_plan"):
+        L.qk_ghost_source_plan.argtypes = [vp, P(Geometry), ci, ci, P(BCRec), ci, P(ci)]
+        L.qk_ghost_source_lookup.argtypes = [vp, ci, ci * 3, P(ci), ci * 3, ci * 3]
     if hasattr(L, "qk_tag_relative_gradient"):
         L.qk_tag_relative_gradient.argtypes = [vp, vp, T, vp, vp, ci, C.c_double, C.c_double, ci]
         L.qk_tag_centered_gradient.argtypes = [vp, vp, vp, vp, ci, ci, C.c_double, C.c_double, C.c_double, ci]
@@ -278,6 +283,7 @@
     "qk_ghost_plan_create", "qk_ghost_plan_destroy", "qk_ghost_plan_num_peers", "qk_ghost_plan_peer", "qk_ghost_plan_num_items", "qk_ghost_plan_item",
     "qk_FillBoundary_local", "qk_FillBoundary_local_int", "qk_FillBoundary_pack", "qk_FillBoundary_unpack", "qk_FillBoundary_pack_int", "qk_FillBoundary_unpack_int", "qk_SumBoundary_local", "qk_SumBoundary_pack", "qk_SumBoundary_unpack", "qk_FillPhysicalBoundary",
     "qk_FillPhysicalBoundary_subset", "qk_ghost_plan_set_components", "qk_ghost_plan_box_is_remote", "qk_ghost_plan_set_box_remote",
+    "qk_ghost_source_plan", "qk_ghost_source_lookup",
     "qk_tag_relative_gradient", "qk_tag_centered_gradient", "qk_avgdown_plan_create", "qk_avgdown_plan_destroy", "qk_avgdown_plan_num_items", "qk_average_down", "qk_PreInterpState", "qk_PostInterpState",
     "qk_interp_plan_create", "qk_interp_plan_destroy", "qk_interp_plan_num_items", "qk_interp_plan_item", "qk_InterpFromCoarse",
     "qk_fluxreg_create", "qk_fluxreg_destroy", "qk_fluxreg_num_items", "qk_fluxreg_item", "qk_fluxreg_reset", "qk_fluxreg_save", "qk_fluxreg_restore", "qk_fluxreg_CrseAdd", "qk_fluxreg_FineAdd",
diff --git a/quokka_amd/csrc/qk_boundary.hip b/quokka_amd/csrc/qk_boundary.hip
--- a/quokka_amd/csrc/qk_boundary.hip
+++ b/quokka_amd/csrc/qk_boundary.hip
@@ -439,6 +439,143 @@
 	return QK_OK;
 }
 
+int qk_ghost_source_plan(qk_level *lev, const qk_geometry *geom, int nghost, int ncomp, const qk_bcrec *bcs, int n_all, int *qualifies)
+{
+	if (lev == nullptr) {
+		return QK_ERR_INVALID;
+	}
+	qk_ctx *ctx = lev->ctx;
+	QK_REQUIRE(ctx, geom && bcs && qualifies && ncomp >= 1 && nghost >= 0, "qk_ghost_source_plan: bad argument");
+	*qualifies = 0;
+	lev->gs_qualifies = 0;
+	if (geom->ndim != 3 || lev->ndim != 3 || lev->nboxes == 0 || n_all != lev->nboxes || ncomp < NVAR) {
+		return QK_OK;
+	}
+	int dlo[3], dhi[3], blen[3], nlat[3];
+	int64_t nsites = 1;
+	for (int d = 0; d < 3; ++d) {
+		dlo[d] = geom->domain.lo[d];
+		dhi[d] = geom->domain.hi[d];
+		blen[d] = lev->boxes[0].hi[d] - lev->boxes[0].lo[d] + 1;
+		const int width = dhi[d] - dlo[d] + 1;
+		if (blen[d] < std::max(nghost, 1) || width % blen[d] != 0) {
+			return QK_OK;
+		}
+		nlat[d] = width / blen[d];
+		nsites *= nlat[d];
+	}
+	if (nsites != lev->nboxes || blen[0] % 64 != 0) {
+		return QK_OK;
+	}
+	auto site = [&](const int l[3]) { return static_cast<size_t>(l[0] + nlat[0] * (l[1] + nlat[1] * l[2])); };
+	std::vector<int> lat2box(static_cast<size_t>(nsites), -1);
+	std::vector<std::array<int, 3>> latOf(static_cast<size_t>(lev->nboxes));
+	for (int b = 0; b < lev->nboxes; ++b) {
+		int l[3];
+		for (int d = 0; d < 3; ++d) {
+			const int len = lev->boxes[b].hi[d] - lev->boxes[b].lo[d] + 1;
+			const int rel = lev->boxes[b].lo[d] - dlo[d];
+			if (len != blen[d] || rel < 0 || rel % blen[d] != 0 || rel / blen[d] >= nlat[d]) {
+				return QK_OK;
+			}
+			l[d] = rel / blen[d];
+		}
+		if (lat2box[site(l)] != -1) {
+			return QK_OK;
+		}
+		lat2box[site(l)] = b;
+		latOf[static_cast<size_t>(b)] = {l[0], l[1], l[2]};
+	}
+	enum { WRAP, REFLECT, CLAMP };
+	int rule[3][2];
+	for (int d = 0; d < 3; ++d) {
+		for (int side = 0; side < 2; ++side) {
+			rule[d][side] = -1;
+			for (int n = 0; n < ncomp; ++n) {
+				const int type = (side == 0) ? bcs[n].lo[d] : bcs[n].hi[d];
+				int r;
+				if (geom->periodic[d] != 0) {
+					r = WRAP;
+				} else if (type == QK_BC_REFLECT_EVEN || type == QK_BC_REFLECT_ODD) {
+					r = REFLECT;
+					if ((type == QK_BC_REFLECT_ODD) != (n == MX + d)) {
+						return QK_OK;
+					}
+				} else if (type == QK_BC_FOEXTRAP) {
+					r = CLAMP;
+				} else {
+					return QK_OK;
+				}
+				if (rule[d][side] != -1 && rule[d][side] != r) {
+					return QK_OK;
+				}
+				rule[d][side] = r;
+			}
+		}
+	}
+	std::vector<GhostFace> faces(static_cast<size_t>(lev->nboxes) * 6);
+	for (int b = 0; b < lev->nboxes; ++b) {
+		for (int d = 0; d < 3; ++d) {
+			for (int side = 0; side < 2; ++side) {
+				GhostFace f{b, 0, 1, 0};
+				int l[3] = {latOf[static_cast<size_t>(b)][0], latOf[static_cast<size_t>(b)][1], latOf[static_cast<size_t>(b)][2]};
+				const bool wall = (side == 0) ? (l[d] == 0) : (l[d] == nlat[d] - 1);
+				const int r = wall ? rule[d][side] : WRAP;
+				if (r == REFLECT) {
+					f.a = (side == 0) ? 2 * dlo[d] - 1 : 2 * dhi[d] + 1;
+					f.b = -1;
+					f.flip = 1;
+				} else if (r == CLAMP) {
+					f.a = (side == 0) ? dlo[d] : dhi[d];
+					f.b = 0;
+				} else {
+					const int width = dhi[d] - dlo[d] + 1;
+					f.a = wall ? ((side == 0) ? width : -width) : 0;
+					l[d] = wall ? ((side == 0) ? nlat[d] - 1 : 0) : l[d] + ((side == 0) ? -1 : 1);
+					f.box = lat2box[site(l)];
+				}
+				faces[static_cast<size_t>(ghostFaceSlot(b, d, side))] = f;
+			}
+		}
+	}
+	lev->gs_faces = faces;
+	lev->gs_ncomp = ncomp;
+	if (ctx->device >= 0) {
+		(void)hipFree(lev->d_gs_faces);
+		lev->d_gs_faces = nullptr;
+		QK_HIP_CHECK(ctx, hipMalloc(reinterpret_cast<void **>(&lev->d_gs_faces), sizeof(GhostFace) * faces.size()));
+		QK_HIP_CHECK(ctx, hipMemcpy(lev->d_gs_faces, faces.data(), sizeof(GhostFace) * faces.size(), hipMemcpyHostToDevice));
+	}
+	lev->gs_qualifies = 1;
+	*qualifies = 1;
+	return QK_OK;
+}
+
+int qk_ghost_source_lookup(qk_level *lev, int box, const int idx[3], int *src_box, int src_idx[3], int flip[3])
+{
+	if (lev == nullptr) {
+		return QK_ERR_INVALID;
+	}
+	qk_ctx *ctx = lev->ctx;
+	QK_REQUIRE(ctx, lev->gs_qualifies != 0, "qk_ghost_source_lookup: the level has no source map (qk_ghost_source_plan)");
+	QK_REQUIRE(ctx, box >= 0 && box < lev->nboxes && idx && src_box && src_idx && flip, "qk_ghost_source_lookup: bad argument");
+	int bb = box;
+	for (int d = 0; d < 3; ++d) {
+		const int lo = lev->boxes[box].lo[d], hi = lev->boxes[box].hi[d];
+		QK_REQUIRE(ctx, idx[d] >= lo - (hi - lo + 1) && idx[d] <= hi + (hi - lo + 1), "qk_ghost_source_lookup: more than a box length outside");
+		src_idx[d] = idx[d];
+		flip[d] = 0;
+		if (idx[d] < lo || idx[d] > hi) {
+			GhostFace const &f = lev->gs_faces[static_cast<size_t>(ghostFaceSlot(bb, d, idx[d] > hi ? 1 : 0))];
+			src_idx[d] = f.a + f.b * idx[d];
+			flip[d] = f.flip;
+			bb = f.box;
+		}
+	}
+	*src_box = bb;
+	return QK_OK;
+}
+
 int qk_ghost_plan_destroy(qk_ghost_plan *plan)
 {
 	if (plan == nullptr) {
diff --git a/quokka_amd/csrc/qk_core.hip b/quokka_amd/csrc/qk_core.hip
--- a/quokka_amd/csrc/qk_core.hip
+++ b/quokka_amd/csrc/qk_core.hip
@@ -126,6 +126,7 @@
 	(void)hipFree(lev->d_boxes);
 	(void)hipFree(lev->d_sgeom);
 	(void)hipFree(lev->d_tile_flags);
+	(void)hipFree(lev->d_gs_faces);
 	(void)hipFree(lev->d_cooling_queue);
 	delete lev;
 	return QK_OK;
diff --git a/quokka_amd/csrc/qk_ghost_source.hpp b/quokka_amd/csrc/qk_ghost_source.hpp
--- /dev/null
+++ b/quokka_amd/csrc/qk_ghost_source.hpp
@@ -0,0 +1,20 @@
+#ifndef QK_GHOST_SOURCE_HPP_
+#define QK_GHOST_SOURCE_HPP_
+
+#include <hip/hip_runtime.h>
+
+#include "quokka_amd.h"
+
+namespace qk
+{
+
+struct GhostFace {
+	int box;
+	int a, b;
+	int flip;
+};
+__host__ __device__ __forceinline__ auto ghostFaceSlot(int box, int d, int side) -> int { return 6 * box + 2 * d + side; }
+
+}
+
+#endif
diff --git a/quokka_amd/csrc/qk_hydro_fused.hip b/quokka_amd/csrc/qk_hydro_fused.hip
--- a/quokka_amd/csrc/qk_hydro_fused.hip
+++ b/quokka_amd/csrc/qk_hydro_fused.hip
@@ -61,6 +61,7 @@
 	bool prim_in, prim_out;
 	bool store_vel;
 	qk_array4 *rk2Vel;
+	const GhostFace *gface;
 };
 
 QK_DEV auto sarr(SweepArgs const &a, int comp) -> double * { return a.scratch + static_cast<int64_t>(comp) * a.total_cells; }
@@ -130,9 +131,9 @@
 	return smax(chi_min, smin1((Zmax - Z) / (Zmax - Zmin)));
 }
 
-template <bool PRIM>
+template <bool PRIM, bool GFS = false>
 __global__ void __launch_bounds__(PT_THREADS, 4) k_pre3(const qk_box *boxes, const SGeom *geom, const qk_array4 *U_t, double *scratch, int64_t T, Eos eos, bool re, int nseg,
-							    int xt, int yt, int ndim)
+							    int xt, int yt, int ndim, const GhostFace *gface = nullptr)
 {
 	constexpr bool prim_in = PRIM;
 	const unsigned nblk = gridDim.x, lin = blockIdx.x;
@@ -198,11 +199,69 @@
 	auto cellOf = [&](PlaneRaw const &r) -> PlaneCell { return prim_in ? PlaneCell{r.rho, r.mx, r.my, r.mz, r.E} : planeCell(eos, re, r); };
 	int64_t uo = ownIn ? U.idx(oi, oj, zfirst - 3) : 0;
 	int64_t uh = haloIn ? U.idx(hi_, hj, zfirst - 3) : 0;
+	RA4::GT *po = nullptr, *ph = nullptr;
+	unsigned flips = 0;
+	int64_t kstep = 0;
+	bool flipz = false;
 
 	for (int k = zfirst - 3; k <= zlast + 3; ++k, uo += U.ks, uh += U.ks) {
 		const bool inPlane = (k >= zfirst) && (k <= zlast);
 		const bool kIn = (k >= fzlo) && (k <= fzhi);
-		const PlaneCell c = cellOf((ownIn && kIn) ? planeLoad(U, uo) : neutral);
+		if constexpr (GFS) {
+			po += kstep;
+			ph += kstep;
+			if (kIn && (k == max(zfirst - 3, fzlo) || k == bx.lo[2] || k == bx.hi[2] + 1)) {
+				const bool zout = (k < bx.lo[2]) || (k > bx.hi[2]);
+				const int zside = (k > bx.hi[2]) ? 1 : 0;
+				GhostFace fz{b, 0, 1, 0};
+				if (zout) {
+					fz = gface[ghostFaceSlot(b, 2, zside)];
+				}
+				const int ksrc = fz.a + fz.b * k;
+				kstep = fz.b * U.ks;
+				flipz = (fz.flip != 0);
+				auto column = [&](int ci, int cj, unsigned &fl) -> RA4::GT * {
+					int bb = b, is = ci, js = cj;
+					fl = 0;
+					if (ci < bx.lo[0] || ci > bx.hi[0]) {
+						const GhostFace f = gface[ghostFaceSlot(bb, 0, (ci > bx.hi[0]) ? 1 : 0)];
+						is = f.a + f.b * ci;
+						fl |= (f.flip != 0) ? 1u : 0u;
+						bb = f.box;
+					}
+					if (cj < bx.lo[1] || cj > bx.hi[1]) {
+						const GhostFace f = gface[ghostFaceSlot(bb, 1, (cj > bx.hi[1]) ? 1 : 0)];
+						js = f.a + f.b * cj;
+						fl |= (f.flip != 0) ? 2u : 0u;
+						bb = f.box;
+					}
+					if (zout) {
+						bb = gface[ghostFaceSlot(bb, 2, zside)].box;
+					}
+					RA4 Us(U_t[bb]);
+					return Us.p + Us.idx(is, js, ksrc);
+				};
+				unsigned fo = 0, fh = 0;
+				po = ownIn ? column(oi, oj, fo) : nullptr;
+				ph = haloIn ? column(hi_, hj, fh) : nullptr;
+				flips = fo | (fh << 2);
+			}
+		}
+		auto ownLoad = [&]() -> PlaneRaw {
+			if constexpr (GFS) {
+				PlaneRaw r;
+				const double mx = po[U.ns * MX], my = po[U.ns * MY], mz = po[U.ns * MZ];
+				r.rho = po[U.ns * RHO];
+				r.mx = (flips & 1u) ? -mx : mx;
+				r.my = (flips & 2u) ? -my : my;
+				r.mz = flipz ? -mz : mz;
+				r.E = po[U.ns * ENE];
+				return r;
+			} else {
+				return planeLoad(U, uo);
+			}
+		};
+		const PlaneCell c = cellOf((ownIn && kIn) ? ownLoad() : neutral);
 #pragma unroll
 		for (int m = 0; m < 4; ++m) {
 			Pz[m] = Pz[m + 1];
@@ -229,17 +288,43 @@
 			if (h >= 0) {
 				if constexpr (PRIM) {
 					if (haloIn && kIn) {
-						hc.P = U.p[uh + U.ns * ENE];
-						if (hy >= 0 && hy < PT_Y && hx >= -2 && hx < PT_X + 2) {
-							hc.vx = U.p[uh + U.ns * MX];
-						}
-						if (hx >= 0 && hx < PT_X && hy >= -2 && hy < PT_Y + 2) {
-							hc.vy = U.p[uh + U.ns * MY];
-						}
-						if (rimX || rimY) {
-							hc.rho = U.p[uh + U.ns * RHO];
+						if constexpr (GFS) {
+							hc.P = ph[U.ns * ENE];
+							if (hy >= 0 && hy < PT_Y && hx >= -2 && hx < PT_X + 2) {
+								const double v = ph[U.ns * MX];
+								hc.vx = (flips & 4u) ? -v : v;
+							}
+							if (hx >= 0 && hx < PT_X && hy >= -2 && hy < PT_Y + 2) {
+								const double v = ph[U.ns * MY];
+								hc.vy = (flips & 8u) ? -v : v;
+							}
+							if (rimX || rimY) {
+								hc.rho = ph[U.ns * RHO];
+							}
+						} else {
+							hc.P = U.p[uh + U.ns * ENE];
+							if (hy >= 0 && hy < PT_Y && hx >= -2 && hx < PT_X + 2) {
+								hc.vx = U.p[uh + U.ns * MX];
+							}
+							if (hx >= 0 && hx < PT_X && hy >= -2 && hy < PT_Y + 2) {
+								hc.vy = U.p[uh + U.ns * MY];
+							}
+							if (rimX || rimY) {
+								hc.rho = U.p[uh + U.ns * RHO];
+							}
 						}
 					}
+				} else if constexpr (GFS) {
+					PlaneRaw r = neutral;
+					if (haloIn && kIn) {
+						const double mx = ph[U.ns * MX], my = ph[U.ns * MY], mz = ph[U.ns * MZ];
+						r.rho = ph[U.ns * RHO];
+						r.mx = (flips & 4u) ? -mx : mx;
+						r.my = (flips & 8u) ? -my : my;
+						r.mz = flipz ? -mz : mz;
+						r.E = ph[U.ns * ENE];
+					}
+					hc = cellOf(r);
 				} else {
 					hc = cellOf((haloIn && kIn) ? planeLoad(U, uh) : neutral);
 				}
@@ -852,8 +937,24 @@
 		}
 	}
 }
-template <int ORDER, int NS>
-QK_DEV void fusexEdgeBatch(SweepArgs const &a, Eos const &eos, RA4 const &Uin, SGeom const &g, const int64_t (&st)[3], const double *S, int x0, int row0, int hi, int ot, EdgeRow<NVAR + NS> *edge)
+QK_DEV auto xorSign(double v, unsigned sign) -> double { return __hiloint2double(__double2hiint(v) ^ static_cast<int>(sign), __double2loint(v)); }
+template <bool GFS, int DIR> QK_DEV auto marchBase(SweepArgs const &a, RA4 const &Uin, int b, qk_box const &bx, int p, unsigned &sign) -> RA4::GT *
+{
+	RA4::GT *sp = Uin.p;
+	sign = 0u;
+	if constexpr (GFS) {
+		if (p < bx.lo[DIR] || p > bx.hi[DIR]) {
+			const GhostFace f = a.gface[ghostFaceSlot(b, DIR, (p > bx.hi[DIR]) ? 1 : 0)];
+			const qk_array4 &sd = a.U_in[f.box];
+			sp = (RA4::GT *)sd.p + ((DIR == 1) ? Uin.js : Uin.ks) * ((f.a + f.b * p - sd.begin[DIR]) - (p - ((DIR == 1) ? Uin.by : Uin.bz)));
+			sign = (f.flip != 0) ? 0x80000000u : 0u;
+		}
+	}
+	return sp;
+}
+template <int ORDER, int NS, bool GFS>
+QK_DEV void fusexEdgeBatch(SweepArgs const &a, Eos const &eos, RA4 const &Uin, SGeom const &g, int b, qk_box const &bx, const int64_t (&st)[3], const double *S, int x0, int row0, int hi, int ot,
+			   EdgeRow<NVAR + NS> *edge)
 {
 	constexpr int NV = NVAR + NS;
 	const int64_t T = a.total_cells;
@@ -864,9 +965,50 @@
 	const int f = x0 + 64 * side;
 	int64_t ub = Uin.idx(f - 3, mrow, ot);
 	double qb[6][NV], Uc[NVAR];
-#pragma unroll
-	for (int m = 0; m < 6; ++m, ++ub) {
-		loadPrims<NS>(Uin, ub, eos, a.reconstruct_eint, a.prim_in, qb[m], Uc);
+	if constexpr (GFS) {
+		const bool lowChunk = (x0 == bx.lo[0]), highChunk = (x0 + 63 == bx.hi[0]);
+		RA4::GT *bL = Uin.p, *bR = Uin.p;
+		int gL = 1, gR = 1;
+		if (lowChunk) {
+			const GhostFace gf = a.gface[ghostFaceSlot(b, 0, 0)];
+			const qk_array4 &sd = a.U_in[gf.box];
+			bL = (RA4::GT *)sd.p + ((gf.a + gf.b * (x0 - 3) - sd.begin[0]) - (x0 - 3 - Uin.bx));
+			gL = gf.b;
+		}
+		if (highChunk) {
+			const GhostFace gf = a.gface[ghostFaceSlot(b, 0, 1)];
+			const qk_array4 &sd = a.U_in[gf.box];
+			bR = (RA4::GT *)sd.p + ((gf.a + gf.b * (x0 + 64) - sd.begin[0]) - (x0 + 64 - Uin.bx));
+			gR = gf.b;
+		}
+#pragma unroll
+		for (int m = 0; m < 6; ++m) {
+#pragma unroll
+			for (int n = 0; n < NVAR; ++n) {
+				Uc[n] = Uin.p[ub + m + Uin.ns * n];
+			}
+			if (m < 3) {
+				if (lowChunk && side == 0) {
+#pragma unroll
+					for (int n = 0; n < NVAR; ++n) {
+						Uc[n] = bL[ub + m * gL + Uin.ns * n];
+					}
+					Uc[MX] = xorSign(Uc[MX], static_cast<unsigned>(gL) & 0x80000000u);
+				}
+			} else if (highChunk && side != 0) {
+#pragma unroll
+				for (int n = 0; n < NVAR; ++n) {
+					Uc[n] = bR[ub + 3 + (m - 3) * gR + Uin.ns * n];
+				}
+				Uc[MX] = xorSign(Uc[MX], static_cast<unsigned>(gR) & 0x80000000u);
+			}
+			primsOf<NS>(Uin, ub, eos, a.reconstruct_eint, a.prim_in, Uc, qb[m]);
+		}
+	} else {
+#pragma unroll
+		for (int m = 0; m < 6; ++m, ++ub) {
+			loadPrims<NS>(Uin, ub, eos, a.reconstruct_eint, a.prim_in, qb[m], Uc);
+		}
 	}
 	const int64_t cb = (f - 1 - g.glo[0]) + (mrow - g.glo[1]) * st[1] + (ot - g.glo[2]) * st[2];
 	const double chiL = S[cb], chiR = S[cb + 1];
@@ -893,10 +1035,11 @@
 		ed[2 * side + 1][n] = (side != 0) ? qb[4][n] : qb[2][n];
 	}
 }
-template <int DIR, int ORDER, int STAGE, bool LAST, int NS, bool CARRY, bool TWOD = false, bool FOFC = false, bool FUSEX = false>
+template <int DIR, int ORDER, int STAGE, bool LAST, int NS, bool CARRY, bool TWOD = false, bool FOFC = false, bool FUSEX = false, bool GFS = false>
 __global__ void __launch_bounds__(64 * MARCH_BY) k_sweep_march(SweepArgs a, Eos eos)
 {
 	static_assert(!FUSEX || (DIR == 1 && !LAST && !TWOD && !FOFC && CARRY), "the X sweep rides on the Y sweep of a 3-D level in the carried form");
+	static_assert(!GFS || (CARRY && NS == 0 && !TWOD && !FOFC && (FUSEX || DIR == 2)), "ghost_from_source: the fused XY march and the Z march of the carried form");
 	static_assert(!(FOFC && CARRY), "the first-order flux correction pass exists for the reference's form of the RK2 average");
 	static_assert(!TWOD || (DIR == 1 && LAST), "the 2-D build has one marching sweep: y, carrying the epilogue");
 	constexpr int NV = NVAR + NS;
@@ -978,9 +1121,14 @@
 	constexpr bool PFQ = !FUSEX && NS == 0;
 	double Un[NVAR];
 	if constexpr (PFQ) {
+		unsigned sign;
+		RA4::GT *sp = marchBase<GFS, DIR>(a, Uin, b, bx, lo - 3, sign);
 #pragma unroll
 		for (int n = 0; n < NVAR; ++n) {
-			Un[n] = Uin.p[u + Uin.ns * n];
+			Un[n] = sp[u + Uin.ns * n];
+		}
+		if constexpr (GFS) {
+			Un[MX + DIR] = xorSign(Un[MX + DIR], sign);
 		}
 	}
 	for (int step = 0; step < nvalid + 6; ++step, c += ms, u += ums) {
@@ -994,11 +1142,25 @@
 		{
 			double Uc[NVAR];
 			if constexpr (PFQ) {
+				unsigned sign;
+				RA4::GT *sp = marchBase<GFS, DIR>(a, Uin, b, bx, lo - 2 + step, sign);
 #pragma unroll
 				for (int n = 0; n < NVAR; ++n) {
 					Uc[n] = Un[n];
-					Un[n] = Uin.p[u + ums + Uin.ns * n];
-				}
+					Un[n] = sp[u + ums + Uin.ns * n];
+				}
+				if constexpr (GFS) {
+					Un[MX + DIR] = xorSign(Un[MX + DIR], sign);
+				}
+				primsOf<NS>(Uin, u, eos, a.reconstruct_eint, a.prim_in, Uc, q[4]);
+			} else if constexpr (GFS) {
+				unsigned sign;
+				RA4::GT *sp = marchBase<GFS, DIR>(a, Uin, b, bx, lo - 3 + step, sign);
+#pragma unroll
+				for (int n = 0; n < NVAR; ++n) {
+					Uc[n] = sp[u + Uin.ns * n];
+				}
+				Uc[MX + DIR] = xorSign(Uc[MX + DIR], sign);
 				primsOf<NS>(Uin, u, eos, a.reconstruct_eint, a.prim_in, Uc, q[4]);
 			} else {
 				loadPrims<NS>(Uin, u, eos, a.reconstruct_eint, a.prim_in, q[4], Uc);
@@ -1034,7 +1196,7 @@
 				EdgeRow<NV> *edge = s_edge[threadIdx.y];
 				const int rr = (step - 6) & (XROWS - 1);
 				if (rr == 0) {
-					fusexEdgeBatch<ORDER, NS>(a, eos, Uin, g, st, S, bx.lo[0] + bix * 64, cidx[DIR], hi, ot, edge);
+					fusexEdgeBatch<ORDER, NS, GFS>(a, eos, Uin, g, b, bx, st, S, bx.lo[0] + bix * 64, cidx[DIR], hi, ot, edge);
 					waveFence();
 					stageEdgeRow<NV>(sx, edge[0]);
 				}
@@ -1310,7 +1472,9 @@
 			return;
 		}
 		if constexpr (CARRY && !FOFC && NS == 0) {
-			if (fusex) {
+			if (fusex && a.gface != nullptr) {
+				hipLaunchKernelGGL((k_sweep_march<1, ORDER, STAGE, false, NS, CARRY, false, FOFC, true, true>), grid, dim3(64, MARCH_BY), 0, s, ay, eos);
+			} else if (fusex) {
 				hipLaunchKernelGGL((k_sweep_march<1, ORDER, STAGE, false, NS, CARRY, false, FOFC, true>), grid, dim3(64, MARCH_BY), 0, s, ay, eos);
 			}
 		}
@@ -1324,6 +1488,12 @@
 		az.nseg = marchSegments(lev, 2, 1);
 		const dim3 grid((lev->maxlen[0] + 63) / 64, (lev->maxlen[1] + MARCH_BY - 1) / MARCH_BY, lev->nboxes * az.nseg);
 		ProfScope ps(lev->ctx, s, "k_sweep_z");
+		if constexpr (CARRY && !FOFC && NS == 0) {
+			if (a.gface != nullptr) {
+				hipLaunchKernelGGL((k_sweep_march<2, ORDER, STAGE, true, NS, CARRY, false, FOFC, false, true>), grid, dim3(64, MARCH_BY), 0, s, az, eos);
+				return;
+			}
+		}
 		hipLaunchKernelGGL((k_sweep_march<2, ORDER, STAGE, true, NS, CARRY, false, FOFC>), grid, dim3(64, MARCH_BY), 0, s, az, eos);
 	}
 }
@@ -1437,6 +1607,17 @@
 			   "qk_hydro_stage_fused: prim_out belongs to stage 1, prim_in to stage 2 (whose old state is a different array)");
 	}
 
+	const bool gfs = (args->ghost_from_source == QK_GHOST_FROM_SOURCE_ON);
+	if (gfs) {
+		QK_REQUIRE(ctx, lev->gs_qualifies != 0 && lev->d_gs_faces != nullptr, "qk_hydro_stage_fused: ghost_from_source needs the level's source map (qk_ghost_source_plan found it qualifying)");
+		QK_REQUIRE(ctx, args->rk2_carry_rhs != 0 && args->fofc_pass == 0 && args->flux_mask == nullptr && t->nscalars == 0 && t->ndim == 3,
+			   "qk_hydro_stage_fused: ghost_from_source is the carried form of a 3-D level without flux mask and passive scalars");
+		QK_REQUIRE(ctx, args->U_in != args->U_out, "qk_hydro_stage_fused: ghost_from_source needs U_in and U_out to be different arrays");
+		if (!fusexApplies(lev, SweepArgs{}, true, 0)) {
+			return setError(ctx, QK_ERR_UNSUPPORTED, "qk_hydro_stage_fused: ghost_from_source needs the fused XY sweep");
+		}
+	}
+
 	if (int rc = buildGeom(lev); rc != QK_OK) {
 		return rc;
 	}
@@ -1453,7 +1634,12 @@
 		const int xt = (lev->maxlen[0] + 2 + PT_X - 1) / PT_X, yt = (lev->maxlen[1] + 2 + PT_Y - 1) / PT_Y;
 		const int nseg = prePassSegments(lev, xt, yt);
 		const dim3 grid(static_cast<unsigned>(xt) * yt * lev->nboxes * nseg);
-		if (args->prim_in != 0) {
+		const GhostFace *gface = lev->d_gs_faces;
+		if (gfs && args->prim_in != 0) {
+			hipLaunchKernelGGL((k_pre3<true, true>), grid, dim3(PT_THREADS), 0, s, boxes, geom, args->U_in, scratch, T, eos, re, nseg, xt, yt, t->ndim, gface);
+		} else if (gfs) {
+			hipLaunchKernelGGL((k_pre3<false, true>), grid, dim3(PT_THREADS), 0, s, boxes, geom, args->U_in, scratch, T, eos, re, nseg, xt, yt, t->ndim, gface);
+		} else if (args->prim_in != 0) {
 			hipLaunchKernelGGL(k_pre3<true>, grid, dim3(PT_THREADS), 0, s, boxes, geom, args->U_in, scratch, T, eos, re, nseg, xt, yt, t->ndim);
 		} else {
 			hipLaunchKernelGGL(k_pre3<false>, grid, dim3(PT_THREADS), 0, s, boxes, geom, args->U_in, scratch, T, eos, re, nseg, xt, yt, t->ndim);
@@ -1484,6 +1670,7 @@
 	a.fluxMask = (args->rk2_carry_rhs != 0) ? args->flux_mask : nullptr;
 	a.prim_in = (args->prim_in != 0);
 	a.prim_out = (args->prim_out != 0);
+	a.gface = gfs ? lev->d_gs_faces : nullptr;
 	for (int d = 0; d < 3; ++d) {
 		a.dx3[d] = args->dx[d];
 	}
diff --git a/quokka_amd/csrc/qk_internal.hpp b/quokka_amd/csrc/qk_internal.hpp
--- a/quokka_amd/csrc/qk_internal.hpp
+++ b/quokka_amd/csrc/qk_internal.hpp
@@ -9,6 +9,7 @@
 #include <vector>
 
 #include "quokka_amd.h"
+#include "qk_ghost_source.hpp"
 
 struct qk_prof_pending {
 	int slot;
@@ -46,6 +47,10 @@
 	int *d_tile_flags = nullptr;
 	size_t tile_flags_bytes = 0;
 	unsigned long long *d_cooling_queue = nullptr;
+	int gs_qualifies = 0;
+	int gs_ncomp = 0;
+	std::vector<qk::GhostFace> gs_faces;
+	qk::GhostFace *d_gs_faces = nullptr;
 };
 
 namespace qk
diff --git a/quokka_amd/host/quokka_host.hpp b/quokka_amd/host/quokka_host.hpp
--- a/quokka_amd/host/quokka_host.hpp
+++ b/quokka_amd/host/quokka_host.hpp
@@ -470,6 +470,7 @@
 	int lastPlotFileStep_ = 0, lastChkFileStep_ = 0;
 	void outputAfterInitialConditions()
 	{
+		ensureGhostsFilled();
 		if (this->restart_chkfile.empty() && this->checkpointInterval_ > 0) {
 			WriteCheckpointFile();
 		}
@@ -481,16 +482,19 @@
 	void outputAfterStep(int step)
 	{
 		if (this->plotfileInterval_ > 0 && (step + 1) % this->plotfileInterval_ == 0) {
+			ensureGhostsFilled();
 			lastPlotFileStep_ = step + 1;
 			WritePlotFile();
 		}
 		if (this->checkpointInterval_ > 0 && (step + 1) % this->checkpointInterval_ == 0) {
+			ensureGhostsFilled();
 			lastChkFileStep_ = step + 1;
 			WriteCheckpointFile();
 		}
 	}
 	void outputAfterEvolve()
 	{
+		ensureGhostsFilled();
 		if (this->plotfileInterval_ > 0 && istep[0] > lastPlotFileStep_) {
 			WritePlotFile();
 		}
@@ -1195,6 +1199,50 @@
 	[[nodiscard]] auto carryActive() const -> bool { return AMREX_SPACEDIM == 3 && rk2CarryRhs_ != 0 && integratorOrder_ == 2 && !storeFluxRk2_ && !forceExactForm_; }
 	bool forceExactForm_ = false;
 
+	int gfsState_ = 0;
+	bool ghostsStale_ = false;
+	[[nodiscard]] auto ghostFromSourceApplies() -> bool
+	{
+		if constexpr (!fusedEligible() || AMREX_SPACEDIM != 3 || HydroSystem<problem_t>::nscalars_ != 0 || is_radiation_enabled_) {
+			return false;
+		} else {
+			if (!carryActive() || fluxMask_.size() > 0 || this->beforePhysBC_ || this->amrLevel_ != 0 || this->customBcIsDefault_ != 1 ||
+			    qkhost::Comm::get().size > 1 || overlapActive()) {
+				return false;
+			}
+			if (gfsState_ == 0) {
+				gfsState_ = 2;
+				char const *e = std::getenv("QK_GHOST_FROM_SOURCE");
+				char const *fx = std::getenv("QK_FUSEX");
+				int maxLevel = 0;
+				amrex::ParmParse("amr").query("max_level", maxLevel);
+				if ((e == nullptr || std::atoi(e) != 0) && (fx == nullptr || std::atoi(fx) != 0) && maxLevel == 0) {
+					auto const bcs = this->boundaryRecords();
+					int q = 0;
+					qkhost::check(qk_ghost_source_plan(this->levelHandle(), &this->qgeom_, nghost_cc_, static_cast<int>(bcs.size()), bcs.data(),
+									   static_cast<int>(this->allBoxes_.size()), &q),
+						      "qk_ghost_source_plan");
+					gfsState_ = (q != 0) ? 1 : 2;
+				}
+			}
+			return gfsState_ == 1;
+		}
+	}
+	void ensureGhostsFilled(std::initializer_list<amrex::MultiFab const *> more = {})
+	{
+		if (ghostsStale_) {
+			ghostsStale_ = false;
+			this->fillBoundaryConditions(state_old_cc_[0]);
+			this->fillBoundaryConditions(state_inter_cc_);
+			this->fillBoundaryConditions(state_new_cc_[0]);
+			for (auto const *mf : more) {
+				if (mf != &state_old_cc_[0] && mf != &state_inter_cc_ && mf != &state_new_cc_[0]) {
+					this->fillBoundaryConditions(*const_cast<amrex::MultiFab *>(mf));
+				}
+			}
+		}
+	}
+
 	struct OverlapGroup {
 		std::vector<int> idx;
 		qk_level *lev = nullptr;
@@ -1302,7 +1350,7 @@
 		}
 	}
 	void fusedLaunch(int stageNo, amrex::MultiFab const &U_in, amrex::MultiFab const &U_old, amrex::MultiFab &U_out, double dt, int group = -1, bool fofc = false,
-			 int slot = 0, OverlapGroup *grp = nullptr, void *scratch = nullptr, int64_t scratchBytes = 0, hipStream_t stream = nullptr)
+			 int slot = 0, OverlapGroup *grp = nullptr, void *scratch = nullptr, int64_t scratchBytes = 0, hipStream_t stream = nullptr, bool ghostFromSource = false)
 	{
 		auto t = qkhost::traits<problem_t>();
 		if (grp == nullptr && group >= 0) {
@@ -1354,6 +1402,7 @@
 			a.prim_out = (stageNo == 1) ? 1 : 0;
 			a.prim_in = (stageNo == 2) ? 1 : 0;
 		}
+		a.ghost_from_source = ghostFromSource ? QK_GHOST_FROM_SOURCE_ON : 0;
 		qkhost::check(qk_hydro_stage_fused(grp == nullptr ? qkhost::Runtime::get().lev : grp->lev, stream != nullptr ? stream : qkhost::Runtime::get().computeStream(), &t, &a),
 			      "qk_hydro_stage_fused");
 	}
@@ -1395,6 +1444,7 @@
 
 	auto correctStage(int stageNo, amrex::MultiFab const &U_in, amrex::MultiFab const &U_old, amrex::MultiFab &U_out, double dt) -> bool
 	{
+		ensureGhostsFilled({&U_in, &U_old});
 		if (stageNo == 1) {
 			stage1LeftF1_ = !carryActive();
 		}
@@ -1460,6 +1510,12 @@
 		if (overlapActive()) {
 			this->fillBoundaryConditions(U_in, [&]() { fusedLaunch(stageNo, U_in, U_old, U_out, dt, 0, false, slot); });
 			fusedLaunch(stageNo, U_in, U_old, U_out, dt, 1, false, slot);
+			return;
+		}
+		if (ghostFromSourceApplies()) {
+			this->activate();
+			ghostsStale_ = true;
+			fusedLaunch(stageNo, U_in, U_old, U_out, dt, -1, false, slot, nullptr, nullptr, 0, nullptr, true);
 			return;
 		}
 		this->fillBoundaryConditions(U_in);
diff --git a/quokka_amd/simulation.py b/quokka_amd/simulation.py
--- a/quokka_amd/simulation.py
+++ b/quokka_amd/simulation.py
@@ -274,6 +274,8 @@
         self.strang_sources = []
         self.ghost = GhostExchange(lev, geom, self.ncomp_cc, NGHOST_CC, self.all_boxes, self.owner, rank, bcs, dirichlet)
         self.flag_ghost = None
+        self.ghost_from_source = os.environ.get("QK_GHOST_FROM_SOURCE", "1") != "0"
+        self._gfs_qualifies = None
         nd = geom.ndim
         self.halfFlux = [MultiFab(lev, self.hydro.nvar_, 0, facedir=d) for d in range(nd)]
         self.halfVel = [MultiFab(lev, 1, 0, facedir=d) for d in range(nd)]
@@ -305,6 +307,25 @@
 
     def fillBoundaryConditions(self, state: MultiFab):
         self.ghost.fill(state)
+        state.ghost_stale = False
+
+    def ensure_ghosts_filled(self, *states: MultiFab):
+        for st in states:
+            if getattr(st, "ghost_stale", False):
+                self.fillBoundaryConditions(st)
+
+    def _ghost_from_source_applies(self) -> bool:
+        if not (self.ghost_from_source and type(self) is HydroSimulation and self.nranks == 1 and self.use_fused and self._carry_active()
+                and getattr(self, "flux_mask", None) is None and self.traits.nscalars == 0 and not self._has_dirichlet
+                and os.environ.get("QK_FUSEX", "1").strip() not in ("0", "")):
+            return False
+        if self._gfs_qualifies is None:
+            L, q = self.ctx.L, C.c_int(0)
+            if hasattr(L, "qk_ghost_source_plan"):
+                self.ctx.check(L.qk_ghost_source_plan(self.lev.h, C.byref(self.ghost._geom_c), NGHOST_CC, self.ncomp_cc, self.ghost.bcs, len(self.all_boxes),
+                                                      C.byref(q)), "qk_ghost_source_plan")
+            self._gfs_qualifies = bool(q.value)
+        return self._gfs_qualifies
 
     def set_initial_conditions(self, fn: Callable[[np.ndarray, np.ndarray, np.ndarray], np.ndarray]):
         for b, (lo, hi) in enumerate(self.my_boxes):
@@ -603,7 +624,7 @@
         c = self.ctx
         c.check(c.L.qk_clear_bytes(c.h, c.stream(), C.c_void_p(self._dev_words.data_ptr() + (0 if both else 32 * slot)), 64 if both else 32), "qk_clear_bytes")
 
-    def _fused_launch(self, stage: int, U_in, U_old, U_out, dt, group=None, fofc: bool = False, slot: int = 0, scratch=None):
+    def _fused_launch(self, stage: int, U_in, U_old, U_out, dt, group=None, fofc: bool = False, slot: int = 0, scratch=None, ghost_from_source: bool = False):
         lev, idx = (self.lev, None) if group is None else group
         tab = (lambda mf: mf.ptr) if idx is None else (lambda mf: mf.subset_ptr(idx))
         a = capi.StageArgs()
@@ -642,6 +663,7 @@
         a.fofc_pass = int(fofc)
         if self._prim_now and not fofc:
             a.prim_out, a.prim_in = int(stage == 1), int(stage == 2)
+        a.ghost_from_source = capi.GHOST_FROM_SOURCE_ON if ghost_from_source else 0
         c = self.ctx
         c.check(c.L.qk_hydro_stage_fused(lev.h, c.stream(), C.byref(self.traits), C.byref(a)), "qk_hydro_stage_fused")
 
@@ -691,6 +713,10 @@
         """hook: a refined level sets the time its coarse-fine ghost cells are interpolated to"""
 
     def _launch_stage(self, stage, U_in, U_old, U_out, dt, slot: int = 0):
+        if self._ghost_from_source_applies():
+            U_in.ghost_stale = True
+            self._fused_launch(stage, U_in, U_old, U_out, dt, slot=slot, ghost_from_source=True)
+            return
         self._before_fill(stage, dt)
         groups = self.overlap_groups()
         if groups is None:
@@ -699,6 +725,7 @@
             return
         early, late = groups
         self.ghost.fill(U_in, between=lambda: self._fused_launch(stage, U_in, U_old, U_out, dt, early, slot=slot))
+        U_in.ghost_stale = False
         self._fused_launch(stage, U_in, U_old, U_out, dt, late, slot=slot)
 
     def _finish_stage(self, stage, U_in, U_old, U_out, dt, nbad: int) -> bool:
@@ -729,6 +756,7 @@
         return self._redo_stage_unfused(stage, U_in, U_old, U_out, dt)
 
     def _correct_stage(self, stage, U_in, U_old, U_out, dt) -> bool:
+        self.ensure_ghosts_filled(U_in, U_old)
         if stage == 1:
             self._stage1_left_F1 = not self._carry_active()
         ok = self._fofc_fused(stage, U_in, U_old, U_out, dt)
```

New measurement: 3488 Mcell-updates/s (median of 6 runs). 1.06x the previous value.
